# aclike/dynamic_multiview_3d

Hardware: AMD Instinct MI355X
Metric: train images/sec, appearance-flow encoder-decoder 128x128x3 (fwd+bwd+Adam) (higher is better)
Workload: dtype bf16x3; 1 GPU; appflow_offset: AppearanceFlowModel 128x128x3, batch 64 per GPU, Adam lr 1e-4, random-init weights (reference initialisers); global_batch=64, parallelism=dp1

## Files before the change

### dynamic_multiview_3d_amd/_lib.py

```python
import ctypes as C
import os

HERE = os.path.dirname(os.path.abspath(__file__))
LIB_PATH = os.environ.get("MV3D_LIB") or os.path.join(HERE, "libmv3d_hip.so")

ACT_NONE, ACT_LRELU, ACT_RELU, ACT_TANH = 0, 1, 2, 3
ACT_BY_NAME = {None: ACT_NONE, 'none': ACT_NONE, 'lrelu': ACT_LRELU, 'relu': ACT_RELU, 'tanh': ACT_TANH}
F32 = 0


class ConvGeom(C.Structure):
    _fields_ = [(n, C.c_int32) for n in
                ("N", "H", "W", "C", "Ho", "Wo", "K", "kh", "kw", "sh", "sw", "img_ld", "feat_ld", "dtype")]


class Epilogue(C.Structure):
    _fields_ = [("bias", C.c_void_p), ("act", C.c_int32), ("leak", C.c_float), ("gmask_act", C.c_int32),
                ("gmask_leak", C.c_float), ("gmask_ref", C.c_void_p), ("gmask_ld", C.c_int32)]


class FcChainLayer(C.Structure):
    _fields_ = [("M", C.c_void_p), ("bias", C.c_void_p), ("y", C.c_void_p), ("y_ld", C.c_int32), ("out", C.c_int32),
                ("act", C.c_int32), ("leak", C.c_float)]


class FcChain(C.Structure):
    _fields_ = [("B", C.c_int32), ("nlayers", C.c_int32), ("in_", C.c_int32), ("x_ld", C.c_int32), ("x", C.c_void_p),
                ("l", FcChainLayer * 4)]


class Mv3dError(RuntimeError):
    pass


_vp, _i, _i64, _f, _sz = C.c_void_p, C.c_int, C.c_int64, C.c_float, C.c_size_t
_G, _E = C.POINTER(ConvGeom), C.POINTER(Epilogue)

STATUS_FUNCS = {
    "mv3d_conv2d_fwd": [_G, _vp, _vp, _vp, _E, _vp, _sz, _vp],
    "mv3d_conv2d_dgrad": [_G, _vp, _vp, _vp, _E, _vp, _sz, _vp],
    "mv3d_conv2d_wgrad": [_G, _vp, _vp, _vp, _vp, _vp, _sz, _vp],
    "mv3d_deconv2d_fwd": [_G, _vp, _vp, _vp, _E, _vp, _sz, _vp],
    "mv3d_deconv2d_dgrad": [_G, _vp, _vp, _vp, _E, _vp, _sz, _vp],
    "mv3d_deconv2d_wgrad": [_G, _vp, _vp, _vp, _vp, _sz, _vp],
    "mv3d_fc_fwd": [_i, _i, _i, _vp, _i, _vp, _vp, _i, _E, _vp, _sz, _vp],
    "mv3d_fc_dgrad": [_i, _i, _i, _vp, _i, _vp, _vp, _i, _E, _vp, _sz, _vp],
    "mv3d_fc_wgrad": [_i, _i, _i, _vp, _i, _vp, _i, _vp, _vp, _vp, _sz, _vp],
    "mv3d_fc_wgrad_dgrad": [_i, _i, _i, _vp, _i, _vp, _i, _vp, _vp, _vp, _vp, _i, _E, _vp, _sz, _vp],
    "mv3d_fc_chain_fwd": [C.POINTER(FcChain), _vp],
    "mv3d_act_fwd": [_i64, _i, _vp, _i, _vp, _i, _i, _f, _vp],
    "mv3d_act_bwd": [_i64, _i, _vp, _i, _vp, _i, _vp, _i, _i, _f, _vp],
    "mv3d_copy2d": [_i64, _i, _vp, _i64, _i64, _vp, _i64, _i, _vp],
    "mv3d_group_sum": [_i64, _i, _i, _vp, _i64, _vp, _i64, _vp],
    "mv3d_warp_resample_fwd": [_i, _i, _i, _i, _i, _i, _vp, _vp, _i, _vp, _vp, _vp],
    "mv3d_warp_resample_bwd": [_i, _i, _i, _i, _i, _i, _vp, _vp, _i, _vp, _vp, _i, _vp],
    "mv3d_warp_resample_loss": [_i, _i, _i, _i, _i, _i, _vp, _vp, _i, _vp, _i, _i, _f, _vp, _vp, _vp, _i, _vp, _vp],
    "mv3d_resampler_fwd": [_i, _i, _i, _i, _i, _vp, _i, _vp, _i, _vp, _i, _vp],
    "mv3d_resampler_bwd": [_i, _i, _i, _i, _i, _vp, _i, _vp, _i, _vp, _i, _vp, _i, _vp, _i, _vp, _sz, _vp],
    "mv3d_image_metrics": [_i, _i, _i, _i, _vp, _i, _vp, _i, _f, _vp, _vp, _sz, _vp],
    "mv3d_ssim_loss": [_i, _i, _i, _i, _vp, _i, _vp, _i, _f, _f, _vp, _vp, _i, _i, _vp, _sz, _vp],
    "mv3d_flow_smoothness": [_i, _i, _i, _vp, _i, _vp, _i, _i, _f, _f, _f, _vp, _vp, _i, _i, _vp, _sz, _vp],
    "mv3d_pixel_loss": [_i64, _i, _vp, _vp, _vp, _i, _f, _vp, _vp, _vp],
    "mv3d_loss_overwrite_next": [],
    "mv3d_pixel_loss_strided": [_i64, _i, _vp, _i, _vp, _i, _f, _vp, _i, _i, _f, _vp, _vp, _i, _vp],
    "mv3d_tfrecord_open": [C.c_char_p, _i, C.POINTER(_vp)],
    "mv3d_tfrecord_read": [_vp, _i, _i, _i, C.POINTER(C.c_char_p), C.POINTER(C.c_int), C.POINTER(C.c_size_t), C.POINTER(_vp), C.POINTER(C.c_int)],
    "mv3d_u8_to_unit_f32": [_i64, _vp, _vp, _vp],
    "mv3d_u8_process_image": [_vp, _i, _i, _i, _i, _vp, _i, _i, _vp],
    "mv3d_fill": [_vp, _i64, _f, _vp],
    "mv3d_adam_step": [_i64, _vp, _vp, _vp, _vp, _f, _f, _f, _f, _f, _f, _f, _vp],
    "mv3d_adam_step_dev": [_i64, _vp, _vp, _vp, _vp, _vp, _i, C.POINTER(_i64), C.POINTER(_i64), _vp],
    "mv3d_adam_advance": [_vp, _vp],
    "mv3d_fc_wgrad_adam": [_i, _i, _i, _vp, _i, _vp, _i, _vp, _vp, _vp, _vp, _vp, _vp],
    "mv3d_sgd_step": [_i64, _vp, _vp, _vp, _f, _f, _i, _f, _vp],
    "mv3d_sgd_step_dev": [_i64, _vp, _vp, _vp, _vp, _i, C.POINTER(_i64), C.POINTER(_i64), _vp],
    "mv3d_fc_wgrad_sgd": [_i, _i, _i, _vp, _i, _vp, _i, _vp, _vp, _vp, _vp, _vp],
    "mv3d_grad_finalize_begin": [],
    "mv3d_grad_finalize_add": [_vp, _i64],
    "mv3d_grad_finalize_commit": [_vp, _sz, _vp, _vp, _vp, _vp, _vp, _vp],
    "mv3d_grad_finalize_commit_sgd": [_vp, _sz, _vp, _vp, _vp, _vp, _vp],
    "mv3d_grad_finalize_abort": [],
    "mv3d_comm_unique_id": [_vp],
    "mv3d_comm_init": [C.POINTER(_vp), _i, _i, _vp],
    "mv3d_comm_destroy": [_vp],
    "mv3d_comm_allreduce_sum": [_vp, _vp, _i64, _vp],
    "mv3d_comm_reduce_scatter_sum": [_vp, _vp, _vp, _i64, _vp],
    "mv3d_comm_allgather": [_vp, _vp, _vp, _i64, _vp],
    "mv3d_ipc_export": [_vp, _vp, C.POINTER(_i64)],
    "mv3d_ipc_open": [_vp, C.POINTER(_vp)],
    "mv3d_ipc_close": [_vp],
    "mv3d_mesh_reduce_sum": [C.POINTER(_vp), _i, _vp, _i64, _vp],
    "mv3d_mesh_copy": [_vp, _vp, _i64, _vp],
    "mv3d_filter_cache_bind": [_G, _i, _vp, _vp, _sz],
    "mv3d_filter_cache_commit": [_vp, _sz, _vp],
    "mv3d_filter_cache_refresh": [_vp],
    "mv3d_filter_cache_clear": [],
    "mv3d_plan_begin": [_vp],
    "mv3d_plan_end": [],
    "mv3d_plan_run": [_vp, _vp],
    "mv3d_plan_run_range": [_vp, _i, _i, _vp],
    "mv3d_plan_run_range_multi": [_vp, _i, _i, _vp, C.POINTER(_vp), _i, _i],
    "mv3d_plan_side": [_i],
    "mv3d_plan_profile": [_vp, _i],
    "mv3d_plan_profile_collect": [_vp],
    "mv3d_plan_profile_select": [_vp, C.c_char_p],
    "mv3d_plan_profile_reset": [_vp],
    "mv3d_plan_op_info": [_vp, _i, C.POINTER(C.c_char_p), C.POINTER(C.c_double), C.POINTER(C.c_double),
                          C.POINTER(C.c_double), C.POINTER(C.c_int)],
}
OTHER_FUNCS = {
    "mv3d_version": (C.c_char_p, []),
    "mv3d_last_error": (C.c_char_p, []),
    "mv3d_conv_workspace_bytes": (_sz, [_G]),
    "mv3d_conv_wgrad_workspace_bytes": (_sz, [_G]),
    "mv3d_fc_workspace_bytes": (_sz, [_i, _i, _i]),
    "mv3d_resampler_bwd_workspace_bytes": (_sz, [_i, _i, _i, _i, _i]),
    "mv3d_image_metrics_workspace_bytes": (_sz, [_i, _i, _i, _i]),
    "mv3d_ssim_loss_workspace_bytes": (_sz, [_i, _i, _i, _i]),
    "mv3d_flow_smoothness_workspace_bytes": (_sz, [_i, _i, _i]),
    "mv3d_crc32c": (C.c_uint32, [_vp, _sz]),
    "mv3d_set_diagnostics": (C.c_int, [_i]),
    "mv3d_set_wgrad_cus": (C.c_int, [_i]),
    "mv3d_tfrecord_close": (None, [_vp]),
    "mv3d_filter_prepared_bytes": (_sz, [_G, _i]),
    "mv3d_filter_cache_table_bytes": (_sz, []),
    "mv3d_grad_finalize_table_bytes": (_sz, []),
    "mv3d_plan_create": (_vp, []),
    "mv3d_plan_destroy": (None, [_vp]),
    "mv3d_plan_size": (_i, [_vp]),
    "mv3d_comm_available": (_i, []),
    "mv3d_fc_wgrad_adam_supported": (_i, [_i, _i, _i, _i, _i]),
    "mv3d_debug_cconv_stamps": (_i, [_vp, _sz]),
    "mv3d_debug_cwgrad_stamps": (_i, [_vp, _sz]),
    "mv3d_debug_band_stamps": (_i, [_vp, _sz]),
}
EXPORTS = sorted(list(STATUS_FUNCS) + list(OTHER_FUNCS))

_lib = None


class _Checked:

    def __init__(self, name, fn, dll):
        self.name, self.fn, self.dll = name, fn, dll

    def __call__(self, *args):
        rc = self.fn(*args)
        if rc != 0:
            raise Mv3dError("%s failed (%d): %s" % (self.name, rc, self.dll.mv3d_last_error().decode()))
        return rc


class _Lib:
    def __init__(self, path):
        if not os.path.exists(path):
            raise Mv3dError("%s not found: build it with `python -m dynamic_multiview_3d_amd.build` "
                            "(hipcc --offload-arch=gfx950); there is no fallback path" % path)
        import torch
        self.dll = C.CDLL(path)
        for name, (res, args) in OTHER_FUNCS.items():
            fn = getattr(self.dll, name)
            fn.restype, fn.argtypes = res, args
            if name[5:] != 'last_error':
                setattr(self, name[5:], fn)
        for name, args in STATUS_FUNCS.items():
            fn = getattr(self.dll, name)
            fn.restype, fn.argtypes = C.c_int, args
            setattr(self, name[5:], _Checked(name, fn, self.dll))
            setattr(self, "raw_" + name[5:], fn)

    def last_error(self):
        return self.dll.mv3d_last_error().decode()


def lib():
    global _lib
    if _lib is None:
        _lib = _Lib(LIB_PATH)
    return _lib


def plan_ops(plan):
    l = lib()
    out = []
    for i in range(l.plan_size(plan)):
        name, fl, by, ms, runs = C.c_char_p(), C.c_double(), C.c_double(), C.c_double(), C.c_int()
        l.plan_op_info(plan, i, C.byref(name), C.byref(fl), C.byref(by), C.byref(ms), C.byref(runs))
        out.append((name.value.decode(), fl.value, by.value, ms.value, runs.value))
    return out


def epilogue(bias=None, act=ACT_NONE, leak=0.2, gmask_act=ACT_NONE, gmask_leak=0.2, gmask_ref=None, gmask_ld=0):
    return Epilogue(bias, act, leak, gmask_act, gmask_leak, gmask_ref, gmask_ld)


def conv_geom(N, H, W, Cc, K, kh, kw, sh, sw, img_ld=None, feat_ld=None):
    Ho, Wo = -(-H // sh), -(-W // sw)
    return ConvGeom(N, H, W, Cc, Ho, Wo, K, kh, kw, sh, sw, Cc if img_ld is None else img_ld,
                    K if feat_ld is None else feat_ld, F32)
```

### dynamic_multiview_3d_amd/build.py

```python
import os
import shutil
import subprocess
import sys

HERE = os.path.dirname(os.path.abspath(__file__))
CSRC = os.path.join(HERE, "csrc")
LIB = os.path.join(HERE, "libmv3d_hip.so")

UNITS = {
    "core.hip": [],
    "conv.hip": [],
    "hconv.hip": [],
    "bconv.hip": [],
    "cconv.hip": (["-DCC_TAP_STAMPS"] if os.environ.get("MV3D_CC_TAP_STAMPS") else []),
    "sconv.hip": [],
    "thin.hip": [],
    "wgrad_tile.hip": [],
    "fc.hip": [],
    "elem.hip": ["-ffp-contract=off"],
    "resampler.hip": ["-ffp-contract=off"],
    "process_image.hip": ["-ffp-contract=off"],
    "metrics.hip": ["-ffp-contract=off"],
    "ssim_loss.hip": ["-ffp-contract=off"],
    "flow_smooth.hip": ["-ffp-contract=off"],
    "comm.hip": [],
    "tfrecord.hip": ["-msse4.2"],
}
COMMON = ["-O3", "-std=c++17", "--offload-arch=gfx950", "-fPIC", "-Wall", "-Wno-unused-function"]


def _hipcc():
    exe = shutil.which("hipcc") or "/opt/rocm/bin/hipcc"
    if not os.path.exists(exe):
        raise RuntimeError("hipcc not found: libmv3d_hip.so cannot be built")
    return exe


def _stale(target, deps):
    if not os.path.exists(target):
        return True
    t = os.path.getmtime(target)
    return any(os.path.getmtime(d) > t for d in deps)


def build(force=False, verbose=False):
    hipcc = _hipcc()
    objdir = os.path.join(HERE, "build")
    os.makedirs(objdir, exist_ok=True)
    headers = [os.path.join(CSRC, "common.h"), os.path.join(CSRC, "conv_common.h"), os.path.join(HERE, "..", "include", "mv3d_hip.h")]
    objs = []
    for src, extra in UNITS.items():
        s = os.path.join(CSRC, src)
        o = os.path.join(objdir, src.replace(".hip", ".o"))
        objs.append(o)
        if force or _stale(o, [s] + headers):
            cmd = [hipcc] + COMMON + extra + ["-c", s, "-o", o]
            if verbose:
                print(" ".join(cmd), flush=True)
            subprocess.run(cmd, check=True)
    if force or _stale(LIB, objs):
        cmd = [hipcc, "-shared", "-fPIC", "--offload-arch=gfx950", "-o", LIB] + objs + ["-ldl"]
        if verbose:
            print(" ".join(cmd), flush=True)
        subprocess.run(cmd, check=True)
    return LIB


if __name__ == "__main__":
    print(build(force="--force" in sys.argv, verbose=True))
```

### dynamic_multiview_3d_amd/csrc/bconv.hip

```cpp
#include "conv_common.h"
#include <algorithm>
#include <mutex>
#include <string.h>
#include <vector>

namespace mv3d {

typedef __bf16 bf16x8 __attribute__((ext_vector_type(8)));
typedef __bf16 bf16x4 __attribute__((ext_vector_type(4)));

constexpr int BC_PIXB = 144;

__device__ __forceinline__ void split4(const float4& v, uint2& hi, uint2& lo) {
    bf16x4 h, l;
    h[0] = (__bf16)v.x; h[1] = (__bf16)v.y; h[2] = (__bf16)v.z; h[3] = (__bf16)v.w;
    l[0] = (__bf16)(v.x - (float)h[0]); l[1] = (__bf16)(v.y - (float)h[1]);
    l[2] = (__bf16)(v.z - (float)h[2]); l[3] = (__bf16)(v.w - (float)h[3]);
    hi = __builtin_bit_cast(uint2, h);
    lo = __builtin_bit_cast(uint2, l);
}


template <int NTHR>
__device__ __forceinline__ void bconv_stage_halo(const IgemmParams& p, const HconvExtra& x, unsigned char* halo, int cc, int n,
                                                 int ih0, int iw0, int tid) {
    constexpr int PS = NTHR / 8;
    const int c4 = tid & 7;
    const int halo_pix = x.HR * x.HC;
    const int ch = cc * 32 + c4 * 4;
    const bool ch_ok = ch < p.Ka && !(x.dbg & 1);
    const int dq = PS / x.HC, dr = PS - dq * x.HC;
    int pix = tid >> 3;
    int hrv = (int)(((unsigned)pix * (unsigned)x.inv_hc) >> 20), hc = pix - hrv * x.HC;
    for (; pix < halo_pix;) {
        float4 v[8];
        int lofs[8];
#pragma unroll
        for (int u = 0; u < 8; ++u) {
            const int g = x.G > 1 ? (int)(((unsigned)hrv * (unsigned)x.inv_hri) >> 20) : 0;
            const int hr = hrv - g * x.HRi;
            const int ih = ih0 + hr, iw = iw0 + hc;
            const bool ok = ch_ok && pix < halo_pix && n + g < p.N && (unsigned)ih < (unsigned)p.Ha && (unsigned)iw < (unsigned)p.Wa;
            const float* src = ok ? p.A + (int64_t)(((n + g) * p.Ha + ih) * p.Wa + iw) * p.a_ld + ch : p.A;
            const float4 t4 = *reinterpret_cast<const float4*>(src);
            v[u] = ok ? t4 : make_float4(0.f, 0.f, 0.f, 0.f);
            lofs[u] = pix < halo_pix ? hrv * x.row_bytes + hc * BC_PIXB + c4 * 8 : -1;
            pix += PS; hc += dr; hrv += dq;
            if (hc >= x.HC) { hc -= x.HC; ++hrv; }
        }
#pragma unroll
        for (int u = 0; u < 8; ++u) {
            if (lofs[u] >= 0) {
                uint2 hi, lo;
                split4(v[u], hi, lo);
                *reinterpret_cast<uint2*>(halo + lofs[u]) = hi;
                *reinterpret_cast<uint2*>(halo + lofs[u] + 64) = lo;
            }
        }
    }
}

template <int MT, int NT>
__device__ __forceinline__ void bconv_store_tile(const IgemmParams& p, const HconvExtra& x, const f32x16 (&acc)[MT][NT], int wave, int lane,
                                                 int n, int oh0, int ow0, int n0, int phh, int phw, int zks) {
    const int li = lane & 31, lh = lane >> 5;
    const int Hp = p.Hp[0], Wp = p.Wp[0];
    const int64_t npix_total = (int64_t)p.N * p.Hc * p.Wc;
    const bool interior = n + x.G <= p.N && oh0 + x.TH <= Hp && ow0 + x.TW <= Wp && n0 + 32 * NT <= p.Cc && !(x.dbg & 16);
#pragma unroll
    for (int m = 0; m < MT; ++m)
#pragma unroll
        for (int y = 0; y < NT; ++y) {
            const int col = n0 + y * 32 + li;
            const float bias = (p.bias && col < p.Cc) ? p.bias[col] : 0.f;
#pragma unroll
            for (int grp = 0; grp < 4; ++grp) {
                const int q = (wave * MT + m) * 32 + 8 * grp + 4 * lh;
                const int g = q >> x.img_shift, qr = q & ((1 << x.img_shift) - 1);
                const int ohp = oh0 + (qr >> x.tw_shift), owp = ow0 + (qr & (x.TW - 1));
                const int64_t pix0 = (int64_t)((n + g) * p.Hc + ohp * p.so_h + phh) * p.Wc + owp * p.so_w + phw;
#pragma unroll
                for (int j = 0; j < 4; ++j) {
                    const float a = acc[m][y][4 * grp + j];
                    const int64_t pix = pix0 + j * p.so_w;
                    if (interior || (n + g < p.N && ohp < Hp && owp + j < Wp && col < p.Cc && !(x.dbg & 16))) {
                        if (x.ksplit > 1) p.Part[((int64_t)zks * npix_total + pix) * p.Cc + col] = a;
                        else {
                            float v = act_apply(a + bias, p.act, p.leak);
                            if (p.gact != MV3D_ACT_NONE) v *= act_grad_from_out(p.gref[pix * p.g_ld + col], p.gact, p.gleak);
                            p.Out[pix * p.c_ld + col] = v;
                        }
                    }
                }
            }
        }
}

__global__ __launch_bounds__(256) void bconv_split_filter_kernel(const IgemmParams p, uint4* __restrict__ Wf, int ntaps, int chunks, int ntiles) {
    const int64_t gid = (int64_t)blockIdx.x * 256 + threadIdx.x;
    const int lane = (int)(gid & 63);
    int64_t r = gid >> 6;
    const int s = (int)(r & 1); r >>= 1;
    const int nt = (int)(r % ntiles); r /= ntiles;
    const int cc = (int)(r % chunks); r /= chunks;
    const int t = (int)r;
    if (t >= ntaps) return;
    const int li = lane & 31, lh = lane >> 5;
    const int col = nt * 32 + li;
    const int ch0 = cc * 32 + s * 16 + lh * 8;
    const float* wt = p.Wt + (int64_t)p.taps[t].widx * p.w_tap_stride;
    float v[8];
#pragma unroll
    for (int j = 0; j < 8; ++j) {
        const int ch = ch0 + j;
        v[j] = (col < p.Cc && ch < p.Ka) ? wt[(int64_t)ch * p.w_ks + (int64_t)col * p.w_ns] : 0.f;
    }
    uint2 h0, l0, h1, l1;
    split4(make_float4(v[0], v[1], v[2], v[3]), h0, l0);
    split4(make_float4(v[4], v[5], v[6], v[7]), h1, l1);
    uint4* dst = Wf + ((((int64_t)t * chunks + cc) * ntiles + nt) * 4 + s * 2) * 64 + lane;
    dst[0] = make_uint4(h0.x, h0.y, h1.x, h1.y);
    dst[64] = make_uint4(l0.x, l0.y, l1.x, l1.y);
}

template <int MT, int NT>
struct BFrags {
    uint4 a[MT][2][2];
    uint4 b[NT][2][2];
};

template <int NPH, int MT, int NT, int WAVES>
__global__ __launch_bounds__(WAVES * 64) void bconv_kernel(const IgemmParams p, const HconvExtra x, const uint4* __restrict__ Wf, int ntiles) {
    extern __shared__ __attribute__((aligned(16))) unsigned char halo[];
    constexpr int NTHR = WAVES * 64;
    const int tid = threadIdx.x;
    const int lane = tid & 63, wave = tid >> 6;
    const int li = lane & 31, lh = lane >> 5;

    int b = blockIdx.x;
    const int tw_i = b % x.tiles_w; b /= x.tiles_w;
    const int th_i = b % x.tiles_h;
    const int n = (b / x.tiles_h) * x.G;
    const int oh0 = th_i * x.TH, ow0 = tw_i * x.TW;
    const int n0 = blockIdx.y * 32 * NT;
    const int zks = (int)blockIdx.z % x.ksplit;

    int lane_base[MT];
#pragma unroll
    for (int m = 0; m < MT; ++m) {
        const int pidx = (wave * MT + m) * 32 + li;
        const int g = pidx >> x.img_shift, pr = pidx & ((1 << x.img_shift) - 1);
        const int tr = pr >> x.tw_shift, tc = pr & (x.TW - 1);
        lane_base[m] = (g * x.HRi + tr * p.sa_h) * x.row_bytes + tc * p.sa_w * BC_PIXB + lh * 16;
    }

    f32x16 acc[NPH][MT][NT];
#pragma unroll
    for (int a = 0; a < NPH; ++a)
#pragma unroll
        for (int m = 0; m < MT; ++m)
#pragma unroll
            for (int y = 0; y < NT; ++y)
#pragma unroll
                for (int r = 0; r < 16; ++r) acc[a][m][y][r] = 0.f;

    const int ph_z = x.phase_split ? (int)blockIdx.z / x.ksplit : 0;
    const int tap_lo = x.phase_split ? p.tap_begin[ph_z] : 0;
    const int ntaps_here = x.phase_split ? p.tap_begin[ph_z + 1] - tap_lo : x.ntaps_total;
    const int tap_hi = tap_lo + ntaps_here;
    const int cc_begin = (x.chunks * zks) / x.ksplit, cc_end = (x.chunks * (zks + 1)) / x.ksplit;
    const int total_seq = (cc_end - cc_begin) * ntaps_here;

    const uint4* wf_lane = Wf + (int64_t)(blockIdx.y * NT) * 256 + lane;
// ... 296 lines not shown
        pg.x = std::min<int>((int)grid.x, cap);
    }
    return dispatch(stream, OpInfo{name, flops, bytes}, [=](hipStream_t s) {
        bconvu_kernel<NTAPS, U, MT, NT, WAVES><<<pg, WAVES * 64, lds, s>>>(p, xp, wf, ntiles);
        return launched(who);
    });
}

static int launch_bconv_cfg(const IgemmParams& p, const HconvExtra& x, int nph_fused, int MT, int NT, int WAVES, dim3 grid, size_t lds,
                            const uint4* wf, int ntiles, void* stream, const char* name, const char* who, double flops, double bytes) {
#define MV3D_BC(NPH_, MT_, NT_, W_) launch_bconv_t<NPH_, MT_, NT_, W_>(p, x, grid, lds, wf, ntiles, stream, name, who, flops, bytes)
    const int ntaps_all = p.tap_begin[p.so_h * p.so_w];
    if (WAVES == 8) return launch_cconv(p, x, wf, ntiles, stream, who, flops, bytes);
    if (nph_fused == 1 && !x.phase_split && p.so_h == 1 && p.so_w == 1 && (ntaps_all == 25 || ntaps_all == 9) && !(disabled_paths() & 8192)) {
#define MV3D_BCU(MT_, NT_, W_) (ntaps_all == 25 ? launch_bconvu_t<25, 5, MT_, NT_, W_>(p, x, grid, lds, wf, ntiles, stream, name, who, flops, bytes) \
                                                : launch_bconvu_t<9, 3, MT_, NT_, W_>(p, x, grid, lds, wf, ntiles, stream, name, who, flops, bytes))
        if (MT == 2 && NT == 1 && WAVES == 4) return MV3D_BCU(2, 1, 4);
        if (MT == 2 && NT == 2 && WAVES == 4) return MV3D_BCU(2, 2, 4);
        if (MT == 1 && NT == 2 && WAVES == 4) return MV3D_BCU(1, 2, 4);
        if (MT == 1 && NT == 1 && WAVES == 4) return MV3D_BCU(1, 1, 4);
        if (MT == 1 && NT == 1 && WAVES == 2) return MV3D_BCU(1, 1, 2);
        if (MT == 1 && NT == 2 && WAVES == 2) return MV3D_BCU(1, 2, 2);
#undef MV3D_BCU
    }
    if (nph_fused == 4) {
        if (MT == 1 && NT == 1 && WAVES == 4) return MV3D_BC(4, 1, 1, 4);
        if (MT == 1 && NT == 1 && WAVES == 2) return MV3D_BC(4, 1, 1, 2);
    } else {
        if (MT == 2 && NT == 1 && WAVES == 4) return MV3D_BC(1, 2, 1, 4);
        if (MT == 2 && NT == 2 && WAVES == 4) return MV3D_BC(1, 2, 2, 4);
        if (MT == 1 && NT == 2 && WAVES == 4) return MV3D_BC(1, 1, 2, 4);
        if (MT == 1 && NT == 1 && WAVES == 4) return MV3D_BC(1, 1, 1, 4);
        if (MT == 1 && NT == 1 && WAVES == 2) return MV3D_BC(1, 1, 1, 2);
        if (MT == 1 && NT == 2 && WAVES == 2) return MV3D_BC(1, 1, 2, 2);
    }
#undef MV3D_BC
    return fail(MV3D_E_UNSUPPORTED, "%s: no split-bf16 kernel for nph=%d MT=%d NT=%d waves=%d", who, nph_fused, MT, NT, WAVES);
}

const void* bconv_cache_lookup(const IgemmParams& p, int* ntiles_out);

int launch_bconv(const IgemmParams& p, const HconvExtra& x, int nph_fused, int MT, int NT, int WAVES, dim3 grid,
                 void* wfrag, void* stream, const char* name, const char* who, double flops, double bytes) {
    const int nph = p.so_h * p.so_w;
    const int ntaps = p.tap_begin[nph];
    const int chunks = x.chunks, ntiles = cdiv(p.Cc, 32 * NT) * NT;
    uint4* wf = reinterpret_cast<uint4*>(wfrag);
    int cached_tiles = 0;
    const void* cached = bconv_cache_lookup(p, &cached_tiles);
    if (cached && cached_tiles >= ntiles) {
        wf = reinterpret_cast<uint4*>(const_cast<void*>(cached));
        const size_t lds0 = (size_t)bconv_lds_bytes(x);
        return launch_bconv_cfg(p, x, nph_fused, MT, NT, WAVES, grid, lds0, wf, cached_tiles, stream, name, who, flops, bytes);
    }
    {
        const int64_t threads = (int64_t)ntaps * chunks * ntiles * 2 * 64;
        const int blocks = (int)cdiv64(threads, 256);
        const IgemmParams pc = p;
        int rc = dispatch(stream, OpInfo{"bconv_split_filter", 0.0, 2.0 * (double)ntaps * p.Ka * p.Cc * 4.0}, [=](hipStream_t s) {
            bconv_split_filter_kernel<<<blocks, 256, 0, s>>>(pc, wf, ntaps, chunks, ntiles);
            return launched("bconv_split_filter_kernel");
        });
        if (rc != MV3D_OK) return rc;
    }
    return launch_bconv_cfg(p, x, nph_fused, MT, NT, WAVES, grid, (size_t)bconv_lds_bytes(x), wf, ntiles, stream, name, who, flops, bytes);
}


const uint4* bconv_get_filter(const IgemmParams& p, void* ws, size_t ws_bytes, void* stream, int* ntiles_out, int* rc) {
    const int nph = p.so_h * p.so_w;
    const int ntaps = p.tap_begin[nph];
    const int chunks = cdiv(p.Ka, 32), ntiles = cdiv(p.Cc, 32);
    int cached_tiles = 0;
    const void* cached = bconv_cache_lookup(p, &cached_tiles);
    if (cached && cached_tiles >= ntiles) { *ntiles_out = cached_tiles; *rc = MV3D_OK; return reinterpret_cast<const uint4*>(cached); }
    const size_t need = bconv_filter_bytes(p, 1);
    if (!ws || ws_bytes < need || (reinterpret_cast<uintptr_t>(ws) & 15)) { *rc = 1; return nullptr; }
    uint4* wf = reinterpret_cast<uint4*>(ws);
    const int64_t threads = (int64_t)ntaps * chunks * ntiles * 2 * 64;
    const int blocks = (int)cdiv64(threads, 256);
    const IgemmParams pc = p;
    *rc = dispatch(stream, OpInfo{"bconv_split_filter", 0.0, 2.0 * (double)ntaps * p.Ka * p.Cc * 4.0}, [=](hipStream_t s) {
        bconv_split_filter_kernel<<<blocks, 256, 0, s>>>(pc, wf, ntaps, chunks, ntiles);
        return launched("bconv_split_filter_kernel");
    });
    if (*rc != MV3D_OK) return nullptr;
    *ntiles_out = ntiles;
    return wf;
}

struct SplitJob {
    const float* Wt; uint4* Wf;
    int ntaps, chunks, ntiles, Ka, Cc, w_tap_stride, w_ks, w_ns;
    int first_block, nblocks;
    int16_t widx[36];
};

static std::mutex g_cache_mu;
static std::vector<SplitJob> g_jobs;
static const SplitJob* g_table_dev = nullptr;
static int g_table_jobs = 0, g_total_blocks = 0;

__global__ __launch_bounds__(256) void bconv_split_all_kernel(const SplitJob* __restrict__ jobs, int njobs) {
    const int* block_job = reinterpret_cast<const int*>(jobs + njobs);
    const SplitJob& jb = jobs[block_job[blockIdx.x]];
    const int64_t gid = (int64_t)(blockIdx.x - jb.first_block) * 256 + threadIdx.x;
    const int lane = (int)(gid & 63);
    int64_t r = gid >> 6;
    const int s = (int)(r & 1); r >>= 1;
    const int nt = (int)(r % jb.ntiles); r /= jb.ntiles;
    const int cc = (int)(r % jb.chunks); r /= jb.chunks;
    const int t = (int)r;
    if (t >= jb.ntaps) return;
    const int li = lane & 31, lh = lane >> 5;
    const int col = nt * 32 + li;
    const int ch0 = cc * 32 + s * 16 + lh * 8;
    const float* wt = jb.Wt + (int64_t)jb.widx[t] * jb.w_tap_stride;
    float v[8];
    if (jb.w_ks == 1 && (jb.w_ns & 3) == 0 && ch0 + 8 <= jb.Ka && col < jb.Cc && ((reinterpret_cast<uintptr_t>(wt) & 15) == 0)) {
        const float4* src = reinterpret_cast<const float4*>(wt + (int64_t)col * jb.w_ns + ch0);
        const float4 u0 = src[0], u1 = src[1];
        v[0] = u0.x; v[1] = u0.y; v[2] = u0.z; v[3] = u0.w; v[4] = u1.x; v[5] = u1.y; v[6] = u1.z; v[7] = u1.w;
    } else {
#pragma unroll
        for (int e = 0; e < 8; ++e) {
            const int ch = ch0 + e;
            v[e] = (col < jb.Cc && ch < jb.Ka) ? wt[(int64_t)ch * jb.w_ks + (int64_t)col * jb.w_ns] : 0.f;
        }
    }
    uint2 h0, l0, h1, l1;
    split4(make_float4(v[0], v[1], v[2], v[3]), h0, l0);
    split4(make_float4(v[4], v[5], v[6], v[7]), h1, l1);
    uint4* dst = jb.Wf + ((((int64_t)t * jb.chunks + cc) * jb.ntiles + nt) * 4 + s * 2) * 64 + lane;
    dst[0] = make_uint4(h0.x, h0.y, h1.x, h1.y);
    dst[64] = make_uint4(l0.x, l0.y, l1.x, l1.y);
}

static bool job_matches(const SplitJob& j, const IgemmParams& p, int ntaps) {
    if (j.Wt != p.Wt || j.ntaps != ntaps || j.Ka != p.Ka || j.Cc != p.Cc || j.w_ks != p.w_ks || j.w_ns != p.w_ns ||
        j.w_tap_stride != p.w_tap_stride) return false;
    for (int t = 0; t < ntaps; ++t) if (j.widx[t] != p.taps[t].widx) return false;
    return true;
}

const void* bconv_cache_lookup(const IgemmParams& p, int* ntiles_out) {
    const int ntaps = p.tap_begin[p.so_h * p.so_w];
    std::lock_guard<std::mutex> lk(g_cache_mu);
    if (!g_table_dev) return nullptr;
    for (int i = 0; i < g_table_jobs && i < (int)g_jobs.size(); ++i)
        if (job_matches(g_jobs[i], p, ntaps)) { *ntiles_out = g_jobs[i].ntiles; return g_jobs[i].Wf; }
    return nullptr;
}

size_t bconv_prepared_bytes(const IgemmParams& p) {
    if (p.fold || p.Ka % 16 != 0 || p.Cc < 16) return 0;
    const int ntaps = p.tap_begin[p.so_h * p.so_w];
    if (ntaps < 2 || ntaps > 36) return 0;
    return bconv_filter_bytes(p, 2);
}

int bconv_cache_bind(const IgemmParams& p, void* prepared, size_t bytes) {
    const size_t need = bconv_prepared_bytes(p);
    if (need == 0) return 1;
    if (!prepared || bytes < need || (reinterpret_cast<uintptr_t>(prepared) & 15))
        return fail(MV3D_E_INVAL, "mv3d_filter_cache_bind: prepared buffer null, misaligned or %zu < %zu bytes", bytes, need);
    const int ntaps = p.tap_begin[p.so_h * p.so_w];
    SplitJob j = {};
    j.Wt = p.Wt; j.Wf = reinterpret_cast<uint4*>(prepared);
    j.ntaps = ntaps; j.chunks = cdiv(p.Ka, 32); j.ntiles = cdiv(p.Cc, 64) * 2; j.Ka = p.Ka; j.Cc = p.Cc;
    j.w_tap_stride = p.w_tap_stride; j.w_ks = p.w_ks; j.w_ns = p.w_ns;
    for (int t = 0; t < ntaps; ++t) j.widx[t] = p.taps[t].widx;
    j.nblocks = (int)cdiv64((int64_t)ntaps * j.chunks * j.ntiles * 2 * 64, 256);
    std::lock_guard<std::mutex> lk(g_cache_mu);
    for (auto& e : g_jobs)
        if (job_matches(e, p, ntaps)) { e.Wf = j.Wf; g_table_dev = nullptr; return MV3D_OK; }
    g_jobs.push_back(j);
    g_table_dev = nullptr;
    return MV3D_OK;
}

}

using namespace mv3d;

extern "C" {

static size_t cache_table_bytes_locked() {
    size_t blocks = 0;
    for (const auto& j : g_jobs) blocks += (size_t)j.nblocks;
    return g_jobs.size() * sizeof(SplitJob) + blocks * sizeof(int);
}

size_t mv3d_filter_cache_table_bytes(void) {
    std::lock_guard<std::mutex> lk(g_cache_mu);
    return cache_table_bytes_locked();
}

int mv3d_filter_cache_commit(void* table_dev, size_t table_bytes, void* stream) {
    std::lock_guard<std::mutex> lk(g_cache_mu);
    const size_t need = cache_table_bytes_locked();
    if (g_jobs.empty()) { g_table_dev = nullptr; g_table_jobs = 0; g_total_blocks = 0; return MV3D_OK; }
    if (!table_dev || table_bytes < need) return fail(MV3D_E_INVAL, "mv3d_filter_cache_commit: table %zu < %zu bytes", table_bytes, need);
    int first = 0;
    for (auto& j : g_jobs) { j.first_block = first; first += j.nblocks; }
    std::vector<unsigned char> host(need);
    memcpy(host.data(), g_jobs.data(), g_jobs.size() * sizeof(SplitJob));
    int* bj = reinterpret_cast<int*>(host.data() + g_jobs.size() * sizeof(SplitJob));
    for (size_t i = 0; i < g_jobs.size(); ++i)
        for (int b = 0; b < g_jobs[i].nblocks; ++b) bj[g_jobs[i].first_block + b] = (int)i;
    hipError_t e = hipMemcpyAsync(table_dev, host.data(), need, hipMemcpyHostToDevice, reinterpret_cast<hipStream_t>(stream));
    if (e == hipSuccess) e = hipStreamSynchronize(reinterpret_cast<hipStream_t>(stream));
    if (e != hipSuccess) return fail(MV3D_E_HIP, "mv3d_filter_cache_commit: %s", hipGetErrorString(e));
    g_table_dev = reinterpret_cast<const SplitJob*>(table_dev);
    g_table_jobs = (int)g_jobs.size();
    g_total_blocks = first;
    return MV3D_OK;
}

int mv3d_filter_cache_refresh(void* stream) {
    const SplitJob* table; int njobs, blocks; double bytes = 0.0;
    {
        std::lock_guard<std::mutex> lk(g_cache_mu);
        table = g_table_dev; njobs = g_table_jobs; blocks = g_total_blocks;
        for (int i = 0; i < njobs; ++i) bytes += 8.0 * g_jobs[i].ntaps * (double)g_jobs[i].Ka * g_jobs[i].Cc;
    }
    if (!table || njobs == 0) return MV3D_OK;
    return dispatch(stream, OpInfo{"bconv_split_all", 0.0, bytes}, [=](hipStream_t s) {
        bconv_split_all_kernel<<<blocks, 256, 0, s>>>(table, njobs);
        return launched("bconv_split_all_kernel");
    });
}

int mv3d_filter_cache_clear(void) {
    std::lock_guard<std::mutex> lk(g_cache_mu);
    g_jobs.clear(); g_table_dev = nullptr; g_table_jobs = 0; g_total_blocks = 0;
    return MV3D_OK;
}

}
```

### dynamic_multiview_3d_amd/csrc/common.h

```cpp
#pragma once
#include <hip/hip_runtime.h>
#include <stdint.h>
#include <stdlib.h>
#include <functional>
#include "../../include/mv3d_hip.h"

namespace mv3d {

int fail(int code, const char* fmt, ...) __attribute__((format(printf, 2, 3)));
struct OpInfo {
    const char* name;
    double flops;
    double bytes;
};

const char* intern_label(const char* fmt, ...) __attribute__((format(printf, 1, 2)));

bool recording();
bool take_loss_overwrite();
void record(std::function<int(hipStream_t)> fn, const OpInfo& info);

enum OptKind { OPT_NONE = 0, OPT_ADAM = 1, OPT_MOMENTUM = 2, OPT_GD = 3 };

__device__ __forceinline__ void momentum_elem(float g, float& p, float& a, float lr, float mu, bool nesterov) {
#pragma clang fp contract(off)
    a = a * mu + g;
    if (nesterov) p = p - (g * lr + (a * mu) * lr);
    else p = p - a * lr;
}
__device__ __forceinline__ void gd_elem(float g, float& p, float lr) {
#pragma clang fp contract(off)
    p = p - g * lr;
}

template <class F>
inline int dispatch(void* stream, const OpInfo& info, F fn) {
    if (recording()) { record(std::function<int(hipStream_t)>(fn), info); return MV3D_OK; }
    return fn(reinterpret_cast<hipStream_t>(stream));
}

inline int launched(const char* what) {
    hipError_t e = hipGetLastError();
    if (e != hipSuccess) return fail(MV3D_E_HIP, "%s: %s", what, hipGetErrorString(e));
    return MV3D_OK;
}

struct FinSegHost { const float* part; int nslab; int64_t count; float* out; };
bool finalize_collecting();
void finalize_push(const float* part, int nslab, int64_t count, float* out);
void finalize_open();
}
#include <vector>
namespace mv3d {
const std::vector<FinSegHost>* finalize_peek();
void finalize_take(std::vector<FinSegHost>* out);

int disabled_paths();

static inline int cdiv(int a, int b) { return (a + b - 1) / b; }
static inline int64_t cdiv64(int64_t a, int64_t b) { return (a + b - 1) / b; }

static inline void same_pad(int size, int k, int s, int* out, int* before) {
    int o = (size + s - 1) / s;
    int total = (o - 1) * s + k - size;
    if (total < 0) total = 0;
    *out = o;
    *before = total / 2;
}

__device__ __forceinline__ float act_apply(float x, int act, float leak) {
    if (act == MV3D_ACT_LRELU) {
        float f1 = 0.5f * (1.0f + leak), f2 = 0.5f * (1.0f - leak);
        return __fadd_rn(__fmul_rn(f1, x), __fmul_rn(f2, fabsf(x)));
    }
    if (act == MV3D_ACT_RELU) {
        float y = __fadd_rn(__fmul_rn(0.5f, x), __fmul_rn(0.5f, fabsf(x)));
        return x < 0.0f ? -0.0f : y;
    }
    if (act == MV3D_ACT_TANH) return tanhf(x);
    return x;
}

__device__ __forceinline__ float act_grad_from_out(float y, int act, float leak) {
    if (act == MV3D_ACT_LRELU) {
        float f1 = 0.5f * (1.0f + leak), f2 = 0.5f * (1.0f - leak);
        float s = (y > 0.0f) ? 1.0f : ((y < 0.0f) ? -1.0f : 0.0f);
        return f1 + f2 * s;
    }
    if (act == MV3D_ACT_RELU) {
        if (y > 0.0f) return 1.0f;
        return (__float_as_uint(y) >> 31) ? 0.0f : 0.5f;
    }
    if (act == MV3D_ACT_TANH) return 1.0f - y * y;
    return 1.0f;
}

typedef float f32x16 __attribute__((ext_vector_type(16)));
typedef float f32x4 __attribute__((ext_vector_type(4)));

}
```

### dynamic_multiview_3d_amd/csrc/core.hip

```cpp
#include "common.h"
#include <atomic>
#include <cstdlib>
#include <stdarg.h>
#include <stdio.h>
#include <string.h>
#include <vector>
#include <mutex>
#include <set>
#include <string>

struct PlanOp {
    std::function<int(hipStream_t)> fn;
    mv3d::OpInfo info;
    double total_ms;
    int runs;
    bool selected = true;
    int side = 0;
};

struct mv3d_plan {
    std::vector<PlanOp> ops;
    bool profile = false;
    std::vector<hipEvent_t> pool;
    size_t used = 0;
    hipEvent_t fork[MV3D_MAX_SIDE] = {}, join[MV3D_MAX_SIDE] = {};
    bool pass_open = false;
};

namespace mv3d {

static std::atomic<int> g_disabled{-1};
int disabled_paths() {
    int v = g_disabled.load(std::memory_order_relaxed);
    if (v < 0) {
        const char* e = getenv("MV3D_DISABLE");
        v = e ? atoi(e) : 0;
        g_disabled.store(v, std::memory_order_relaxed);
    }
    return v;
}

static thread_local char g_err[512] = "";
static thread_local mv3d_plan* g_rec = nullptr;
static thread_local int g_side = 0;

int fail(int code, const char* fmt, ...) {
    va_list ap;
    va_start(ap, fmt);
    vsnprintf(g_err, sizeof(g_err), fmt, ap);
    va_end(ap);
    return code;
}
const char* intern_label(const char* fmt, ...) {
    char buf[128];
    va_list ap;
    va_start(ap, fmt);
    vsnprintf(buf, sizeof(buf), fmt, ap);
    va_end(ap);
    static std::mutex mu;
    static std::set<std::string>* labels = new std::set<std::string>();
    std::lock_guard<std::mutex> lk(mu);
    return labels->insert(buf).first->c_str();
}
static thread_local std::vector<FinSegHost>* g_fin = nullptr;
bool finalize_collecting() { return g_fin != nullptr; }
void finalize_open() { if (!g_fin) g_fin = new std::vector<FinSegHost>(); }
void finalize_push(const float* part, int nslab, int64_t count, float* out) { if (g_fin) g_fin->push_back(FinSegHost{part, nslab, count, out}); }
const std::vector<FinSegHost>* finalize_peek() { return g_fin; }
void finalize_take(std::vector<FinSegHost>* out) {
    if (!g_fin) return;
    if (out) out->swap(*g_fin);
    delete g_fin;
    g_fin = nullptr;
}
bool recording() { return g_rec != nullptr; }
void record(std::function<int(hipStream_t)> fn, const OpInfo& info) { g_rec->ops.push_back(PlanOp{std::move(fn), info, 0.0, 0, true, g_side}); }
}

extern "C" {

const char* mv3d_version(void) { return "mv3d_hip 0.3 (gfx950, split-bf16 / fp32 MFMA)"; }
const char* mv3d_last_error(void) { return mv3d::g_err; }

mv3d_plan* mv3d_plan_create(void) { return new mv3d_plan(); }
void mv3d_plan_destroy(mv3d_plan* p) {
    if (!p) return;
    if (mv3d::g_rec == p) mv3d::g_rec = nullptr;
    for (hipEvent_t e : p->pool) (void)hipEventDestroy(e);
    for (int k = 0; k < MV3D_MAX_SIDE; ++k) {
        if (p->fork[k]) (void)hipEventDestroy(p->fork[k]);
        if (p->join[k]) (void)hipEventDestroy(p->join[k]);
    }
    delete p;
}
int mv3d_plan_begin(mv3d_plan* p) {
    if (!p) return mv3d::fail(MV3D_E_INVAL, "mv3d_plan_begin: null plan");
    if (mv3d::g_rec) return mv3d::fail(MV3D_E_INVAL, "mv3d_plan_begin: a plan is already recording on this thread");
    p->ops.clear();
    p->used = 0;
    mv3d::g_rec = p;
    mv3d::g_side = 0;
    return MV3D_OK;
}
int mv3d_plan_side(int side) {
    if (side < 0 || side > MV3D_MAX_SIDE) return mv3d::fail(MV3D_E_INVAL, "mv3d_plan_side: side %d not in [0, %d]", side, MV3D_MAX_SIDE);
    mv3d::g_side = side;
    return MV3D_OK;
}
int mv3d_plan_end(void) {
    if (!mv3d::g_rec) return mv3d::fail(MV3D_E_INVAL, "mv3d_plan_end: nothing is recording");
    mv3d::g_rec = nullptr;
    return MV3D_OK;
}
int mv3d_plan_size(const mv3d_plan* p) { return p ? (int)p->ops.size() : 0; }

int mv3d_plan_run_range(mv3d_plan* p, int begin, int end, void* stream) {
    return mv3d_plan_run_range_multi(p, begin, end, stream, nullptr, 0, 0);
}

int mv3d_plan_run_range_multi(mv3d_plan* p, int begin, int end, void* stream, void* const* side_streams, int nside, int flags) {
    if (!p) return mv3d::fail(MV3D_E_INVAL, "mv3d_plan_run_range: null plan");
    if (mv3d::g_rec) return mv3d::fail(MV3D_E_INVAL, "mv3d_plan_run_range: cannot run while recording");
    const int n = (int)p->ops.size();
    if (begin < 0 || end > n || begin > end) return mv3d::fail(MV3D_E_INVAL, "mv3d_plan_run_range: bad range [%d, %d) of %d", begin, end, n);
    if (nside < 0 || nside > MV3D_MAX_SIDE || (nside > 0 && !side_streams)) return mv3d::fail(MV3D_E_INVAL, "mv3d_plan_run_range_multi: bad side stream list");
    hipStream_t s = reinterpret_cast<hipStream_t>(stream);
    for (int k = 0; k < nside; ++k)
        if (!p->fork[k]) {
            if (hipEventCreateWithFlags(&p->fork[k], hipEventDisableTiming) != hipSuccess ||
                hipEventCreateWithFlags(&p->join[k], hipEventDisableTiming) != hipSuccess)
                return mv3d::fail(MV3D_E_HIP, "mv3d_plan_run_range_multi: hipEventCreate failed");
        }
    int prev_side = 0;
    bool used[MV3D_MAX_SIDE] = {};
    auto stream_of = [&](int i) -> hipStream_t {
        const int tag = p->ops[i].side;
        const int sd = (nside > 0 && tag > 0) ? 1 + (tag - 1) % nside : 0;
        hipStream_t so = sd ? reinterpret_cast<hipStream_t>(side_streams[sd - 1]) : s;
        if (sd && so == s) { prev_side = 0; return s; }
        if (sd && sd != prev_side) {
            (void)hipEventRecord(p->fork[sd - 1], s);
            (void)hipStreamWaitEvent(so, p->fork[sd - 1], 0);
            used[sd - 1] = true;
        }
        prev_side = sd;
        return so;
    };
    auto join = [&]() {
        if (flags & MV3D_RUN_NO_JOIN) return;
        for (int k = 0; k < nside; ++k)
            if (used[k]) {
                (void)hipEventRecord(p->join[k], reinterpret_cast<hipStream_t>(side_streams[k]));
                (void)hipStreamWaitEvent(s, p->join[k], 0);
            }
    };
    if (!p->profile) {
        for (int i = begin; i < end; ++i) {
            int rc = p->ops[i].fn(stream_of(i));
            if (rc != MV3D_OK) return rc;
        }
        join();
        return MV3D_OK;
    }
    const size_t need = p->used + 2 * (size_t)n;
    while (p->pool.size() < need) {
        hipEvent_t e;
        if (hipEventCreate(&e) != hipSuccess) return mv3d::fail(MV3D_E_HIP, "mv3d_plan_run: hipEventCreate failed");
        p->pool.push_back(e);
    }
    if (!p->pass_open) {
        for (int i = 0; i < begin; ++i)
            if (p->ops[i].selected) { (void)hipEventRecord(p->pool[p->used + 2 * i], s); (void)hipEventRecord(p->pool[p->used + 2 * i + 1], s); }
        p->pass_open = true;
    }
    for (int i = begin; i < end; ++i) {
        const bool sel = p->ops[i].selected;
        hipStream_t so = stream_of(i);
        if (sel) (void)hipEventRecord(p->pool[p->used + 2 * i], so);
        int rc = p->ops[i].fn(so);
        if (sel) (void)hipEventRecord(p->pool[p->used + 2 * i + 1], so);
        if (rc != MV3D_OK) return rc;
    }
    join();
    if (end == n) { p->used = need; p->pass_open = false; }
    return MV3D_OK;
}

int mv3d_plan_run(mv3d_plan* p, void* stream) {
    if (!p) return mv3d::fail(MV3D_E_INVAL, "mv3d_plan_run: null plan");
    return mv3d_plan_run_range(p, 0, (int)p->ops.size(), stream);
}

int mv3d_plan_profile(mv3d_plan* p, int enable) {
    if (!p) return mv3d::fail(MV3D_E_INVAL, "mv3d_plan_profile: null plan");
    p->profile = enable != 0;
    return MV3D_OK;
}

int mv3d_plan_profile_collect(mv3d_plan* p) {
    if (!p) return mv3d::fail(MV3D_E_INVAL, "mv3d_plan_profile_collect: null plan");
    const size_t n = p->ops.size();
    if (n == 0 || p->used == 0) return MV3D_OK;
    size_t last = n;
    for (size_t i = 0; i < n; ++i) if (p->ops[i].selected) last = i;
    if (last == n) { p->used = 0; return MV3D_OK; }
    if (hipEventSynchronize(p->pool[p->used - 2 * n + 2 * last + 1]) != hipSuccess)
        return mv3d::fail(MV3D_E_HIP, "mv3d_plan_profile_collect: hipEventSynchronize failed");
    for (size_t base = 0; base + 2 * n <= p->used; base += 2 * n)
        for (size_t i = 0; i < n; ++i) {
            if (!p->ops[i].selected) continue;
            float ms = 0.f;
            if (hipEventElapsedTime(&ms, p->pool[base + 2 * i], p->pool[base + 2 * i + 1]) == hipSuccess) {
                p->ops[i].total_ms += ms;
                p->ops[i].runs += 1;
            }
        }
    p->used = 0;
    (void)hipGetLastError();
    return MV3D_OK;
}

static bool label_matches(const char* label, const char* pats) {
    const size_t ll = strlen(label);
    for (const char* p = pats; *p;) {
        const char* e = strchr(p, '|');
        size_t n = e ? (size_t)(e - p) : strlen(p);
// ... 67 lines not shown
```

### dynamic_multiview_3d_amd/csrc/elem.hip

```cpp
#include "common.h"
#include "reduce_common.h"
#include <vector>
#include <algorithm>
#include <cstdlib>
#include <atomic>

namespace mv3d {

constexpr int LOSS_ROWS = 32, LOSS_MAXB = 1024;
__device__ unsigned g_loss_part[LOSS_ROWS][LOSS_MAXB];
__device__ unsigned g_loss_ticket[LOSS_ROWS];

static thread_local bool g_loss_overwrite = false;
bool take_loss_overwrite() {
    const bool v = g_loss_overwrite;
    g_loss_overwrite = false;
    return v;
}
static int next_loss_row() {
    static std::atomic<unsigned> n{0};
    const int flag = take_loss_overwrite() ? 256 : 0;
    return (int)(n.fetch_add(1) % LOSS_ROWS) | flag;
}

__device__ __forceinline__ void loss_combine(float term, float* loss, int row_flag) {
    const int row = row_flag & 255;
    __shared__ unsigned s_last;
    __shared__ float s_w[4];
    if (threadIdx.x == 0) {
        (void)__hip_atomic_exchange(&g_loss_part[row][blockIdx.x], __float_as_uint(term), __ATOMIC_RELAXED, __HIP_MEMORY_SCOPE_AGENT);
        asm volatile("s_waitcnt vmcnt(0)" ::: "memory");
        const unsigned t = __hip_atomic_fetch_add(&g_loss_ticket[row], 1u, __ATOMIC_RELAXED, __HIP_MEMORY_SCOPE_AGENT);
        s_last = t == gridDim.x - 1;
    }
    __syncthreads();
    if (!s_last) return;
    float sum = 0.f;
    for (unsigned i = threadIdx.x; i < gridDim.x; i += 256)
        sum += __uint_as_float(__hip_atomic_fetch_or(&g_loss_part[row][i], 0u, __ATOMIC_RELAXED, __HIP_MEMORY_SCOPE_AGENT));
    for (int off = 32; off > 0; off >>= 1) sum += __shfl_down(sum, off);
    if ((threadIdx.x & 63) == 0) s_w[threadIdx.x >> 6] = sum;
    __syncthreads();
    if (threadIdx.x == 0) {
        const float total = (s_w[0] + s_w[1]) + (s_w[2] + s_w[3]);
        if (row_flag & 256) *loss = total; else atomicAdd(loss, total);
        __hip_atomic_store(&g_loss_ticket[row], 0u, __ATOMIC_RELAXED, __HIP_MEMORY_SCOPE_AGENT);
    }
}

struct ResampleParams {
    const float* src; const float* flow; const float* dgen;
    float* warp; float* gen; float* dflow;
    int N, H, W, Hs, Ws, C, flow_ld, dflow_ld;
};

__device__ __forceinline__ float tap(const float* img, int Ws, int Hs, int C, int y, int x, int c) {
    const bool ok = (unsigned)x < (unsigned)Ws && (unsigned)y < (unsigned)Hs;
    const int xc = min(max(x, 0), Ws - 1), yc = min(max(y, 0), Hs - 1);
    const float v = img[((int64_t)yc * Ws + xc) * C + c];
    return ok ? v : 0.f;
}

template <bool BWD>
__global__ __launch_bounds__(256) void resample_kernel(const ResampleParams p) {
    const int tj = threadIdx.x & 31, ti = threadIdx.x >> 5;
    const int j = blockIdx.x * 32 + tj, i = blockIdx.y * 8 + ti, n = blockIdx.z;
    if (i >= p.H || j >= p.W) return;
    const int64_t pix = ((int64_t)n * p.H + i) * p.W + j;
    const float* fl = p.flow + pix * p.flow_ld;
    const float x = fl[0] + (float)i;
    const float y = fl[1] + (float)j;
    if (!BWD && p.warp) { p.warp[pix * 2] = x; p.warp[pix * 2 + 1] = y; }
    const bool valid = x > -1.0f && y > -1.0f && x < (float)p.Ws && y < (float)p.Hs;
    const float fxf = floorf(x), fyf = floorf(y);
    const int fx = (int)fxf, fy = (int)fyf, cx = fx + 1, cy = fy + 1;
    const float dx = (fxf + 1.0f) - x, dy = (fyf + 1.0f) - y;
    const float* img = p.src + (int64_t)n * p.Hs * p.Ws * p.C;
    if (!BWD) {
        float* out = p.gen + pix * p.C;
        for (int c = 0; c < p.C; ++c) {
            float v = 0.f;
            if (valid) {
                const float iff = tap(img, p.Ws, p.Hs, p.C, fy, fx, c), icc = tap(img, p.Ws, p.Hs, p.C, cy, cx, c);
                const float ifc = tap(img, p.Ws, p.Hs, p.C, cy, fx, c), icf = tap(img, p.Ws, p.Hs, p.C, fy, cx, c);
                v = ((dx * dy * iff + (1.0f - dx) * (1.0f - dy) * icc) + dx * (1.0f - dy) * ifc) + (1.0f - dx) * dy * icf;
            }
            out[c] = v;
        }
    } else {
        float gx = 0.f, gy = 0.f;
        if (valid) {
            const float* g = p.dgen + pix * p.C;
            for (int c = 0; c < p.C; ++c) {
                const float iff = tap(img, p.Ws, p.Hs, p.C, fy, fx, c), icc = tap(img, p.Ws, p.Hs, p.C, cy, cx, c);
                const float ifc = tap(img, p.Ws, p.Hs, p.C, cy, fx, c), icf = tap(img, p.Ws, p.Hs, p.C, fy, cx, c);
                gx += g[c] * (dy * (icf - iff) + (1.0f - dy) * (icc - ifc));
                gy += g[c] * (dx * (ifc - iff) + (1.0f - dx) * (icc - icf));
            }
        }
        float* d = p.dflow + pix * p.dflow_ld;
        d[0] = gx; d[1] = gy;
    }
}

struct ResampleTileParams {
    const float* src; const float* flow; const float* aux;
    float* warp; float* gen; float* dflow; float* loss; int loss_row;
    int N, H, W, Hs, Ws, flow_ld, aux_ld, dflow_ld, kind;
    float weight;
    int tiles_i, tiles_j, n_tiles;
};

template <int MODE, int C>
__global__ __launch_bounds__(256) void resample_tile_kernel(const ResampleTileParams p) {
    constexpr int P = 33;
    __shared__ float s_xy[2][32 * P];
    __shared__ float s_c[C][32 * P];
    const int lo = threadIdx.x & 31, hi = threadIdx.x >> 5;
    const float inv_pix = 1.0f / (float)((int64_t)p.N * p.H * p.W);
    const float gscale = (p.kind == 2 ? 2.0f : 1.0f) * p.weight / (float)((int64_t)p.N * p.H * p.W);
    float sum = 0.f;
    for (int tile = blockIdx.x; tile < p.n_tiles; tile += gridDim.x) {
        int b = tile;
        const int tj = b % p.tiles_j; b /= p.tiles_j;
        const int ti = b % p.tiles_i;
        const int n = b / p.tiles_i;
        const int i0 = ti * 32, j0 = tj * 32;
        const float* img = p.src + (int64_t)n * p.Hs * p.Ws * C;
        {
            float fx_[4], fy_[4], av[4][C];
#pragma unroll
            for (int k = 0; k < 4; ++k) {
                const int i = min(i0 + hi + 8 * k, p.H - 1), j = min(j0 + lo, p.W - 1);
                const int64_t pix = ((int64_t)n * p.H + i) * p.W + j;
                const float* fl = p.flow + pix * p.flow_ld;
                fx_[k] = fl[0]; fy_[k] = fl[1];
                if (MODE != 0) {
#pragma unroll
                    for (int c = 0; c < C; ++c) av[k][c] = p.aux[pix * p.aux_ld + c];
                }
            }
#pragma unroll
            for (int k = 0; k < 4; ++k) {
                const int r = hi + 8 * k, i = i0 + r, j = j0 + lo;
                const float x = fx_[k] + (float)min(i, p.H - 1), y = fy_[k] + (float)min(j, p.W - 1);
                s_xy[0][r * P + lo] = x; s_xy[1][r * P + lo] = y;
                if (MODE != 0) {
#pragma unroll
                    for (int c = 0; c < C; ++c) s_c[c][r * P + lo] = av[k][c];
                }
                if (MODE != 1 && p.warp && i < p.H && j < p.W) {
                    const int64_t pix = ((int64_t)n * p.H + i) * p.W + j;
                    p.warp[pix * 2] = x; p.warp[pix * 2 + 1] = y;
                }
// ... 115 lines not shown
        else { sum += fabsf(d); g = ((d > 0.f) ? 1.f : ((d < 0.f) ? -1.f : 0.f)) * m * gscale; }
        if (p.grad) p.grad[pix * p.grad_ld + c] = g;
    }
    for (int off = 32; off > 0; off >>= 1) sum += __shfl_down(sum, off);
    __shared__ float s_part[4];
    if ((threadIdx.x & 63) == 0) s_part[threadIdx.x >> 6] = sum;
    __syncthreads();
    loss_combine((s_part[0] + s_part[1] + s_part[2] + s_part[3]) * (p.weight / (float)p.pixels), p.loss, p.loss_row);
}

__global__ __launch_bounds__(256) void pixel_loss_dense_kernel(int64_t total4, int64_t pixels, const float4* __restrict__ a,
                                                              const float4* __restrict__ b, int kind, float weight, float* loss,
                                                              float4* __restrict__ grad, int loss_row) {
    const float gscale = (kind == 2 ? 2.0f : 1.0f) * weight / (float)pixels;
    float sum = 0.f;
    for (int64_t i = (int64_t)blockIdx.x * 256 + threadIdx.x; i < total4; i += (int64_t)gridDim.x * 256) {
        const float4 x = a[i], y = b[i];
        const float d[4] = {x.x - y.x, x.y - y.y, x.z - y.z, x.w - y.w};
        float g[4];
#pragma unroll
        for (int e = 0; e < 4; ++e) {
            if (kind == 2) { sum += d[e] * d[e]; g[e] = d[e] * gscale; }
            else { sum += fabsf(d[e]); g[e] = ((d[e] > 0.f) ? 1.f : ((d[e] < 0.f) ? -1.f : 0.f)) * gscale; }
        }
        if (grad) grad[i] = make_float4(g[0], g[1], g[2], g[3]);
    }
    for (int off = 32; off > 0; off >>= 1) sum += __shfl_down(sum, off);
    __shared__ float s_part[4];
    if ((threadIdx.x & 63) == 0) s_part[threadIdx.x >> 6] = sum;
    __syncthreads();
    loss_combine((s_part[0] + s_part[1] + s_part[2] + s_part[3]) * (weight / (float)pixels), loss, loss_row);
}

__global__ __launch_bounds__(256) void u8_to_unit_f32_kernel(int64_t count, const unsigned char* __restrict__ src, float* __restrict__ dst) {
    const int64_t nvec = count >> 2;
    for (int64_t i = (int64_t)blockIdx.x * 256 + threadIdx.x; i < nvec; i += (int64_t)gridDim.x * 256) {
        const uchar4 b = reinterpret_cast<const uchar4*>(src)[i];
        reinterpret_cast<float4*>(dst)[i] = make_float4((float)b.x / 255.0f, (float)b.y / 255.0f, (float)b.z / 255.0f, (float)b.w / 255.0f);
    }
    if (blockIdx.x == 0 && threadIdx.x < (count & 3)) { const int64_t i = (nvec << 2) + threadIdx.x; dst[i] = (float)src[i] / 255.0f; }
}

__global__ __launch_bounds__(256) void fill_kernel(float* dst, int64_t count, float v) {
    for (int64_t i = (int64_t)blockIdx.x * 256 + threadIdx.x; i < count; i += (int64_t)gridDim.x * 256) dst[i] = v;
}

__global__ __launch_bounds__(256) void adam_kernel(int64_t count, float* __restrict__ p, const float* __restrict__ g,
                                                  float* __restrict__ m, float* __restrict__ v, float alpha,
                                                  float omb1, float omb2, float eps, float gscale) {
    const int64_t nvec = count >> 2;
    for (int64_t i = (int64_t)blockIdx.x * 256 + threadIdx.x; i < nvec; i += (int64_t)gridDim.x * 256) {
        float4 pp = reinterpret_cast<float4*>(p)[i], gg = reinterpret_cast<const float4*>(g)[i];
        float4 mm = reinterpret_cast<float4*>(m)[i], vv = reinterpret_cast<float4*>(v)[i];
        float* pe = &pp.x; float* ge = &gg.x; float* me = &mm.x; float* ve = &vv.x;
#pragma unroll
        for (int k = 0; k < 4; ++k) {
            const float gk = ge[k] * gscale;
            me[k] += (gk - me[k]) * omb1;
            ve[k] += (gk * gk - ve[k]) * omb2;
            pe[k] -= (me[k] * alpha) / (sqrtf(ve[k]) + eps);
        }
        reinterpret_cast<float4*>(p)[i] = pp;
        reinterpret_cast<float4*>(m)[i] = mm;
        reinterpret_cast<float4*>(v)[i] = vv;
    }
    if (blockIdx.x == 0 && threadIdx.x < (count & 3)) {
        const int64_t i = (nvec << 2) + threadIdx.x;
        const float gk = g[i] * gscale;
        m[i] += (gk - m[i]) * omb1;
        v[i] += (gk * gk - v[i]) * omb2;
        p[i] -= (m[i] * alpha) / (sqrtf(v[i]) + eps);
    }
}

struct AdamSkips { int n; int64_t lo[8], hi[8]; };
__global__ __launch_bounds__(256) void adam_dev_kernel(int64_t count, float* __restrict__ p, const float* __restrict__ g,
                                                      float* __restrict__ m, float* __restrict__ v, const float* __restrict__ st, const AdamSkips sk) {
    const float lr = st[0], b1 = st[1], b2 = st[2], eps = st[3], b1p = st[4], b2p = st[5], gscale = st[6];
    const float alpha = lr * sqrtf(1.0f - b2p) / (1.0f - b1p);
    const float omb1 = 1.0f - b1, omb2 = 1.0f - b2;
    int64_t kept = count >> 2;
    for (int r = 0; r < sk.n; ++r) kept -= (sk.hi[r] - sk.lo[r]) >> 2;
    for (int64_t j = (int64_t)blockIdx.x * 256 + threadIdx.x; j < kept; j += (int64_t)gridDim.x * 256) {
        int64_t i = j;
        for (int r = 0; r < sk.n; ++r)
            if (i >= (sk.lo[r] >> 2)) i += (sk.hi[r] - sk.lo[r]) >> 2;
        float4 pp = reinterpret_cast<float4*>(p)[i], gg = reinterpret_cast<const float4*>(g)[i];
        float4 mm = reinterpret_cast<float4*>(m)[i], vv = reinterpret_cast<float4*>(v)[i];
        float* pe = &pp.x; float* ge = &gg.x; float* me = &mm.x; float* ve = &vv.x;
#pragma unroll
        for (int k = 0; k < 4; ++k) {
            const float gk = ge[k] * gscale;
            me[k] += (gk - me[k]) * omb1;
            ve[k] += (gk * gk - ve[k]) * omb2;
            pe[k] -= (me[k] * alpha) / (sqrtf(ve[k]) + eps);
        }
        reinterpret_cast<float4*>(p)[i] = pp;
        reinterpret_cast<float4*>(m)[i] = mm;
        reinterpret_cast<float4*>(v)[i] = vv;
    }
}
__global__ void adam_advance_kernel(float* st) {
    if (threadIdx.x == 0 && blockIdx.x == 0) { st[4] = st[4] * st[1]; st[5] = st[5] * st[2]; }
}

template <bool MOM>
__device__ __forceinline__ void sgd4(float* p, const float* g, float* a, int64_t i, float lr, float mu, bool nesterov, float gscale) {
    float4 pp = reinterpret_cast<float4*>(p)[i], gg = reinterpret_cast<const float4*>(g)[i];
    float4 aa = MOM ? reinterpret_cast<float4*>(a)[i] : make_float4(0.f, 0.f, 0.f, 0.f);
    float* pe = &pp.x; float* ge = &gg.x; float* ae = &aa.x;
#pragma unroll
    for (int k = 0; k < 4; ++k) {
        const float gk = ge[k] * gscale;
        if (MOM) momentum_elem(gk, pe[k], ae[k], lr, mu, nesterov);
        else gd_elem(gk, pe[k], lr);
    }
    reinterpret_cast<float4*>(p)[i] = pp;
    if (MOM) reinterpret_cast<float4*>(a)[i] = aa;
}

template <bool MOM>
__global__ __launch_bounds__(256) void sgd_kernel(int64_t count, float* __restrict__ p, const float* __restrict__ g,
                                                 float* __restrict__ a, float lr, float mu, int nesterov, float gscale) {
    const int64_t nvec = count >> 2;
    for (int64_t i = (int64_t)blockIdx.x * 256 + threadIdx.x; i < nvec; i += (int64_t)gridDim.x * 256)
        sgd4<MOM>(p, g, a, i, lr, mu, nesterov != 0, gscale);
    if (blockIdx.x == 0 && threadIdx.x < (count & 3)) {
        const int64_t i = (nvec << 2) + threadIdx.x;
        const float gk = g[i] * gscale;
        if (MOM) { float pv = p[i], av = a[i]; momentum_elem(gk, pv, av, lr, mu, nesterov != 0); p[i] = pv; a[i] = av; }
        else { float pv = p[i]; gd_elem(gk, pv, lr); p[i] = pv; }
    }
}

template <bool MOM>
__global__ __launch_bounds__(256) void sgd_dev_kernel(int64_t count, float* __restrict__ p, const float* __restrict__ g,
                                                     float* __restrict__ a, const float* __restrict__ st, const AdamSkips sk) {
    const float lr = st[MV3D_SGD_LR], mu = st[MV3D_SGD_MOMENTUM], gscale = st[MV3D_SGD_GSCALE];
    const bool nesterov = st[MV3D_SGD_NESTEROV] != 0.f;
    int64_t kept = count >> 2;
    for (int r = 0; r < sk.n; ++r) kept -= (sk.hi[r] - sk.lo[r]) >> 2;
    for (int64_t j = (int64_t)blockIdx.x * 256 + threadIdx.x; j < kept; j += (int64_t)gridDim.x * 256) {
        int64_t i = j;
        for (int r = 0; r < sk.n; ++r)
            if (i >= (sk.lo[r] >> 2)) i += (sk.hi[r] - sk.lo[r]) >> 2;
        sgd4<MOM>(p, g, a, i, lr, mu, nesterov, gscale);
    }
}

struct FinSeg {
    const float* part; float* out;
    int64_t off;
    int64_t count;
    int nslab, vec, blk0, pad;
};

template <int OPT>
__global__ __launch_bounds__(256) void grad_finalize_kernel(const FinSeg* __restrict__ segs, const int* __restrict__ seg_of_blk,
                                                           const float* __restrict__ G, float* __restrict__ P, float* __restrict__ M,
                                                           float* __restrict__ V, const float* __restrict__ st) {
    constexpr bool ADAM = OPT == OPT_ADAM, SGD = OPT == OPT_MOMENTUM || OPT == OPT_GD;
    __shared__ float s_sum[4][16][17];
    const FinSeg sg = segs[seg_of_blk[blockIdx.x]];
    const int blk = (int)blockIdx.x - sg.blk0;
    float alpha = 0.f, omb1 = 0.f, omb2 = 0.f, eps = 0.f, gscale = 1.f;
    if (ADAM) {
        const float lr = st[0], b1 = st[1], b2 = st[2], b1p = st[4], b2p = st[5];
        eps = st[3]; gscale = st[6];
        alpha = lr * sqrtf(1.0f - b2p) / (1.0f - b1p);
        omb1 = 1.0f - b1; omb2 = 1.0f - b2;
    }
    float lr = 0.f, mu = 0.f;
    bool nesterov = false;
    if (SGD) {
        lr = st[MV3D_SGD_LR]; mu = st[MV3D_SGD_MOMENTUM]; nesterov = st[MV3D_SGD_NESTEROV] != 0.f; gscale = st[MV3D_SGD_GSCALE];
    }
    auto adam1 = [&](int64_t i, float g) {
        const float gk = g * gscale;
        float m = M[i], v = V[i], pp = P[i];
        m += (gk - m) * omb1;
        v += (gk * gk - v) * omb2;
        pp -= (m * alpha) / (sqrtf(v) + eps);
        P[i] = pp; M[i] = m; V[i] = v;
    };
    auto sgd1 = [&](int64_t i, float g) {
        const float gk = g * gscale;
        float pp = P[i];
        if (OPT == OPT_MOMENTUM) { float a = M[i]; momentum_elem(gk, pp, a, lr, mu, nesterov); M[i] = a; }
        else gd_elem(gk, pp, lr);
        P[i] = pp;
    };
    if (sg.nslab == 0) {
        if (!ADAM && !SGD) return;
        const int64_t i4 = (int64_t)blk * 256 + threadIdx.x;
        if (i4 * 4 >= sg.count) return;
        const int64_t i = (sg.off >> 2) + i4;
        if constexpr (SGD) {
            sgd4<OPT == OPT_MOMENTUM>(P, G, M, i, lr, mu, nesterov, gscale);
            return;
        }
        float4 pp = reinterpret_cast<float4*>(P)[i], gg = reinterpret_cast<const float4*>(G)[i];
        float4 mm = reinterpret_cast<float4*>(M)[i], vv = reinterpret_cast<float4*>(V)[i];
        float* pe = &pp.x; float* ge = &gg.x; float* me = &mm.x; float* ve = &vv.x;
#pragma unroll
        for (int k = 0; k < 4; ++k) {
            const float gk = ge[k] * gscale;
            me[k] += (gk - me[k]) * omb1;
            ve[k] += (gk * gk - ve[k]) * omb2;
            pe[k] -= (me[k] * alpha) / (sqrtf(ve[k]) + eps);
        }
        reinterpret_cast<float4*>(P)[i] = pp;
        reinterpret_cast<float4*>(M)[i] = mm;
        reinterpret_cast<float4*>(V)[i] = vv;
        return;
    }
    auto fin = [&](int64_t i, float t) {
        if (ADAM) adam1(sg.off + i, t);
        else if (SGD) sgd1(sg.off + i, t);
        else sg.out[i] = t;
    };
    if (sg.vec) reduce_slabs_body<4>(sg.part, sg.nslab, sg.count, blk, s_sum, fin);
    else reduce_slabs_body<1>(sg.part, sg.nslab, sg.count, blk, s_sum, fin);
}

__global__ __launch_bounds__(256) void act_fwd_kernel(int64_t rows, int ch, const float* x, int x_ld, float* y, int y_ld,
                                                     int act, float leak) {
    const int64_t total = rows * ch;
    for (int64_t i = (int64_t)blockIdx.x * 256 + threadIdx.x; i < total; i += (int64_t)gridDim.x * 256) {
        const int64_t r = i / ch; const int c = (int)(i - r * ch);
        y[r * y_ld + c] = act_apply(x[r * x_ld + c], act, leak);
    }
}
__global__ __launch_bounds__(256) void act_bwd_kernel(int64_t rows, int ch, const float* dy, int dy_ld, const float* ref,
                                                     int ref_ld, float* dx, int dx_ld, int act, float leak) {
    const int64_t total = rows * ch;
    for (int64_t i = (int64_t)blockIdx.x * 256 + threadIdx.x; i < total; i += (int64_t)gridDim.x * 256) {
        const int64_t r = i / ch; const int c = (int)(i - r * ch);
        dx[r * dx_ld + c] = dy[r * dy_ld + c] * act_grad_from_out(ref[r * ref_ld + c], act, leak);
    }
}
__global__ __launch_bounds__(256) void copy2d_kernel(int64_t rows, int ch, const float* src, int64_t src_ld, int64_t src_row_div,
                                                    float* dst, int64_t dst_ld, int accumulate) {
    const int64_t total = rows * ch;
    for (int64_t i = (int64_t)blockIdx.x * 256 + threadIdx.x; i < total; i += (int64_t)gridDim.x * 256) {
        const int64_t r = i / ch; const int c = (int)(i - r * ch);
        const float v = src[(r / src_row_div) * src_ld + c];
        float* d = dst + r * dst_ld + c;
        *d = accumulate ? (*d + v) : v;
    }
}
__global__ __launch_bounds__(256) void group_sum_kernel(int64_t groups, int group, int ch, const float* src, int64_t src_ld,
                                                       float* dst, int64_t dst_ld) {
    const int64_t total = groups * ch;
    for (int64_t i = (int64_t)blockIdx.x * 256 + threadIdx.x; i < total; i += (int64_t)gridDim.x * 256) {
        const int64_t gidx = i / ch; const int c = (int)(i - gidx * ch);
        float s = 0.f;
        for (int r = 0; r < group; ++r) s += src[(gidx * group + r) * src_ld + c];
        dst[gidx * dst_ld + c] = s;
    }
}

static inline int grid_for(int64_t total) { return (int)std::min<int64_t>(cdiv64(total, 256), 8192); }

}

using namespace mv3d;

extern "C" {

int mv3d_warp_resample_fwd(int N, int H, int W, int Hs, int Ws, int C, const void* src, const void* flow, int flow_ld,
                           void* warp_out, void* gen, void* stream) {
    if (N <= 0 || H <= 0 || W <= 0 || Hs <= 0 || Ws <= 0 || C <= 0 || flow_ld < 2) return fail(MV3D_E_INVAL, "mv3d_warp_resample_fwd: bad shape");
    if (!src || !flow || !gen) return fail(MV3D_E_INVAL, "mv3d_warp_resample_fwd: null pointer");
    if (N > 65535) return fail(MV3D_E_UNSUPPORTED, "mv3d_warp_resample_fwd: batch > 65535");
    if (C <= 4 && !(disabled_paths() & 65536)) {
        ResampleTileParams t = {};
        t.src = (const float*)src; t.flow = (const float*)flow; t.warp = (float*)warp_out; t.gen = (float*)gen;
        t.N = N; t.H = H; t.W = W; t.Hs = Hs; t.Ws = Ws; t.flow_ld = flow_ld;
        const int blocks = resample_tile_blocks(t);
        return dispatch(stream, OpInfo{"resample_fwd", 0.0, (double)N * H * W * (8.0 + 8.0 * C)}, [=](hipStream_t s) {
            launch_resample_tile<0>(t, C, blocks, s);
            return launched("resample_tile_kernel<fwd>");
        });
    }
    ResampleParams p = {(const float*)src, (const float*)flow, nullptr, (float*)warp_out, (float*)gen, nullptr, N, H, W, Hs, Ws, C, flow_ld, 0};
    dim3 grid(cdiv(W, 32), cdiv(H, 8), N);
    return dispatch(stream, OpInfo{"resample_fwd", 0.0, (double)N * H * W * (8.0 + 8.0 * C)}, [=](hipStream_t s) {
        resample_kernel<false><<<grid, 256, 0, s>>>(p);
        return launched("resample_kernel<fwd>");
    });
}

int mv3d_warp_resample_bwd(int N, int H, int W, int Hs, int Ws, int C, const void* src, const void* flow, int flow_ld,
                           const void* dgen, void* dflow, int dflow_ld, void* stream) {
    if (N <= 0 || H <= 0 || W <= 0 || Hs <= 0 || Ws <= 0 || C <= 0 || flow_ld < 2 || dflow_ld < 2) return fail(MV3D_E_INVAL, "mv3d_warp_resample_bwd: bad shape");
    if (!src || !flow || !dgen || !dflow) return fail(MV3D_E_INVAL, "mv3d_warp_resample_bwd: null pointer");
    if (N > 65535) return fail(MV3D_E_UNSUPPORTED, "mv3d_warp_resample_bwd: batch > 65535");
    if (C <= 4 && !(disabled_paths() & 65536)) {
        ResampleTileParams t = {};
        t.src = (const float*)src; t.flow = (const float*)flow; t.aux = (const float*)dgen; t.aux_ld = C; t.dflow = (float*)dflow;
        t.N = N; t.H = H; t.W = W; t.Hs = Hs; t.Ws = Ws; t.flow_ld = flow_ld; t.dflow_ld = dflow_ld;
        const int blocks = resample_tile_blocks(t);
        return dispatch(stream, OpInfo{"resample_bwd", 0.0, (double)N * H * W * (16.0 + 8.0 * C)}, [=](hipStream_t s) {
            launch_resample_tile<1>(t, C, blocks, s);
            return launched("resample_tile_kernel<bwd>");
        });
    }
    ResampleParams p = {(const float*)src, (const float*)flow, (const float*)dgen, nullptr, nullptr, (float*)dflow, N, H, W, Hs, Ws, C, flow_ld, dflow_ld};
    dim3 grid(cdiv(W, 32), cdiv(H, 8), N);
    return dispatch(stream, OpInfo{"resample_bwd", 0.0, (double)N * H * W * (16.0 + 8.0 * C)}, [=](hipStream_t s) {
        resample_kernel<true><<<grid, 256, 0, s>>>(p);
        return launched("resample_kernel<bwd>");
    });
}

int mv3d_warp_resample_loss(int N, int H, int W, int Hs, int Ws, int C, const void* src, const void* flow, int flow_ld,
                            const void* target, int target_ld, int kind, float weight, void* warp_out, void* gen,
                            void* dflow, int dflow_ld, void* loss_accum, void* stream) {
    if (N <= 0 || H <= 0 || W <= 0 || Hs <= 0 || Ws <= 0 || C <= 0 || flow_ld < 2 || target_ld < C || (dflow && dflow_ld < 2))
        return fail(MV3D_E_INVAL, "mv3d_warp_resample_loss: bad shape");
    if (kind != 1 && kind != 2) return fail(MV3D_E_INVAL, "mv3d_warp_resample_loss: kind must be 1 (l1) or 2 (euclidean)");
    if (!src || !flow || !target || !gen || !loss_accum) return fail(MV3D_E_INVAL, "mv3d_warp_resample_loss: null pointer");
    if (C > 4) return fail(MV3D_E_UNSUPPORTED, "mv3d_warp_resample_loss: more than 4 channels");
    ResampleTileParams t = {};
    t.src = (const float*)src; t.flow = (const float*)flow; t.aux = (const float*)target; t.aux_ld = target_ld;
    t.warp = (float*)warp_out; t.gen = (float*)gen; t.dflow = (float*)dflow; t.loss = (float*)loss_accum;
    t.N = N; t.H = H; t.W = W; t.Hs = Hs; t.Ws = Ws; t.flow_ld = flow_ld; t.dflow_ld = dflow_ld; t.kind = kind; t.weight = weight;
    t.loss_row = next_loss_row();
    static const int max_blocks = getenv("MV3D_RL_BLOCKS") ? atoi(getenv("MV3D_RL_BLOCKS")) : 512;
    const int blocks = std::min(resample_tile_blocks(t), max_blocks);
    return dispatch(stream, OpInfo{"resample_loss", 0.0, (double)N * H * W * (8.0 + 8.0 + 8.0 + 12.0 * C)}, [=](hipStream_t s) {
        launch_resample_tile<2>(t, C, blocks, s);
        return launched("resample_tile_kernel<fused>");
    });
}

int mv3d_pixel_loss_strided(int64_t pixels, int ch, const void* a, int a_ld, const void* b, int b_ld, float b_scale,
                            const void* mask, int mask_ld, int kind, float weight, void* loss_accum, void* grad, int grad_ld,
                            void* stream) {
    if (pixels <= 0 || ch <= 0 || (kind != 1 && kind != 2)) return fail(MV3D_E_INVAL, "mv3d_pixel_loss: bad arguments");
    if (!a || !b || !loss_accum) return fail(MV3D_E_INVAL, "mv3d_pixel_loss: null pointer");
    if (a_ld < ch || b_ld < ch || (grad && grad_ld < ch) || (mask && mask_ld < 1)) return fail(MV3D_E_INVAL, "mv3d_pixel_loss: pixel stride smaller than the channel count");
    PixelLossParams p = {pixels, ch, (const float*)a, a_ld, (const float*)b, b_ld, b_scale, (const float*)mask, mask_ld, kind, weight,
                         (float*)loss_accum, (float*)grad, grad_ld, next_loss_row()};
    const int64_t total = pixels * ch;
    const bool dense = a_ld == ch && b_ld == ch && (!grad || grad_ld == ch) && !mask && b_scale == 1.0f && (total & 3) == 0 &&
                       ((((uintptr_t)a) | ((uintptr_t)b) | ((uintptr_t)grad)) & 15) == 0;
    if (dense) {
        const int64_t total4 = total >> 2;
        const int blocks4 = (int)std::min<int64_t>(cdiv64(total4, 256 * 2), 256);
        return dispatch(stream, OpInfo{"pixel_loss", 0.0, (double)total * (grad ? 12.0 : 8.0)}, [=](hipStream_t s) {
            pixel_loss_dense_kernel<<<blocks4, 256, 0, s>>>(total4, pixels, (const float4*)a, (const float4*)b, kind, weight,
                                                           (float*)loss_accum, (float4*)grad, p.loss_row);
            return launched("pixel_loss_dense_kernel");
        });
    }
    const int blocks = (int)std::min<int64_t>(cdiv64(total, 256 * 8), 256);
    return dispatch(stream, OpInfo{"pixel_loss", 0.0, (double)total * (grad ? 12.0 : 8.0)}, [=](hipStream_t s) {
        pixel_loss_kernel<<<blocks, 256, 0, s>>>(p);
        return launched("pixel_loss_kernel");
    });
}

int mv3d_pixel_loss(int64_t pixels, int ch, const void* a, const void* b, const void* mask, int kind, float weight,
                    void* loss_accum, void* grad, void* stream) {
    return mv3d_pixel_loss_strided(pixels, ch, a, ch, b, ch, 1.0f, mask, 1, kind, weight, loss_accum, grad, ch, stream);
}

int mv3d_fill(void* dst, int64_t count, float value, void* stream) {
    if (!dst || count < 0) return fail(MV3D_E_INVAL, "mv3d_fill: bad arguments");
    if (count == 0) return MV3D_OK;
    return dispatch(stream, OpInfo{"fill", 0.0, 4.0 * count}, [=](hipStream_t s) {
        fill_kernel<<<grid_for(count), 256, 0, s>>>((float*)dst, count, value);
        return launched("fill_kernel");
    });
}

int mv3d_u8_to_unit_f32(int64_t count, const void* src, void* dst, void* stream) {
    if (count <= 0 || !src || !dst) return fail(MV3D_E_INVAL, "mv3d_u8_to_unit_f32: bad arguments");
    if (((uintptr_t)src & 3) || ((uintptr_t)dst & 15)) return fail(MV3D_E_INVAL, "mv3d_u8_to_unit_f32: src must be 4-byte and dst 16-byte aligned");
    return dispatch(stream, OpInfo{"u8_to_unit_f32", 0.0, 5.0 * count}, [=](hipStream_t s) {
        u8_to_unit_f32_kernel<<<grid_for(count / 4 + 1), 256, 0, s>>>(count, (const unsigned char*)src, (float*)dst);
        return launched("u8_to_unit_f32_kernel");
    });
}

static int parse_skips(const char* who, int64_t count, int nskip, const int64_t* skip_lo, const int64_t* skip_hi, AdamSkips& sk,
                       int64_t& skipped) {
    if (nskip < 0 || nskip > 8 || (nskip > 0 && (!skip_lo || !skip_hi))) return fail(MV3D_E_INVAL, "%s: at most 8 skipped ranges", who);
    sk = {};
    sk.n = nskip;
    skipped = 0;
    for (int r = 0; r < nskip; ++r) {
        if ((skip_lo[r] & 3) || (skip_hi[r] & 3) || skip_lo[r] < 0 || skip_hi[r] > count || skip_lo[r] > skip_hi[r])
            return fail(MV3D_E_INVAL, "%s: skipped range %d is not a multiple-of-4 sub-range", who, r);
        if (r > 0 && skip_lo[r] < skip_hi[r - 1]) return fail(MV3D_E_INVAL, "%s: skipped ranges must be sorted and disjoint", who);
        sk.lo[r] = skip_lo[r]; sk.hi[r] = skip_hi[r];
        skipped += skip_hi[r] - skip_lo[r];
    }
    return MV3D_OK;
}

int mv3d_adam_step(int64_t count, void* p, const void* g, void* m, void* v, float lr, float beta1, float beta2,
                   float eps, float beta1_power, float beta2_power, float grad_scale, void* stream) {
    if (count <= 0 || !p || !g || !m || !v) return fail(MV3D_E_INVAL, "mv3d_adam_step: bad arguments");
    if (((uintptr_t)p | (uintptr_t)g | (uintptr_t)m | (uintptr_t)v) & 15) return fail(MV3D_E_INVAL, "mv3d_adam_step: buffers must be 16-byte aligned");
    const float alpha = lr * sqrtf(1.0f - beta2_power) / (1.0f - beta1_power);
    const float omb1 = 1.0f - beta1, omb2 = 1.0f - beta2;
    const int blocks = (int)std::min<int64_t>(cdiv64(count / 4 + 1, 256), 4096);
    return dispatch(stream, OpInfo{"adam", 0.0, 28.0 * count}, [=](hipStream_t s) {
        adam_kernel<<<blocks, 256, 0, s>>>(count, (float*)p, (const float*)g, (float*)m, (float*)v, alpha, omb1, omb2, eps, grad_scale);
        return launched("adam_kernel");
    });
}

int mv3d_adam_step_dev(int64_t count, void* p, const void* g, void* m, void* v, const void* state, int nskip, const int64_t* skip_lo,
                       const int64_t* skip_hi, void* stream) {
    if (count <= 0 || (count & 3) || !p || !g || !m || !v || !state) return fail(MV3D_E_INVAL, "mv3d_adam_step_dev: bad arguments (count must be a multiple of 4)");
    if (((uintptr_t)p | (uintptr_t)g | (uintptr_t)m | (uintptr_t)v) & 15) return fail(MV3D_E_INVAL, "mv3d_adam_step_dev: buffers must be 16-byte aligned");
    AdamSkips sk;
    int64_t skipped;
    if (int rc = parse_skips("mv3d_adam_step_dev", count, nskip, skip_lo, skip_hi, sk, skipped)) return rc;
    const int blocks = (int)std::min<int64_t>(cdiv64((count - skipped) / 4 + 1, 256), 4096);
    return dispatch(stream, OpInfo{"adam", 0.0, 28.0 * (count - skipped)}, [=](hipStream_t s) {
        adam_dev_kernel<<<blocks, 256, 0, s>>>(count, (float*)p, (const float*)g, (float*)m, (float*)v, (const float*)state, sk);
        return launched("adam_dev_kernel");
    });
}

int mv3d_adam_advance(void* state, void* stream) {
    if (!state) return fail(MV3D_E_INVAL, "mv3d_adam_advance: null state");
    return dispatch(stream, OpInfo{"adam_advance", 0.0, 16.0}, [=](hipStream_t s) {
        adam_advance_kernel<<<1, 64, 0, s>>>((float*)state);
        return launched("adam_advance_kernel");
    });
}

int mv3d_sgd_step(int64_t count, void* p, const void* g, void* accum, float lr, float momentum, int use_nesterov, float grad_scale,
                  void* stream) {
    if (count <= 0 || !p || !g) return fail(MV3D_E_INVAL, "mv3d_sgd_step: bad arguments");
    if (((uintptr_t)p | (uintptr_t)g | (uintptr_t)accum) & 15) return fail(MV3D_E_INVAL, "mv3d_sgd_step: buffers must be 16-byte aligned");
    if (!accum && (momentum != 0.0f || use_nesterov))
        return fail(MV3D_E_INVAL, "mv3d_sgd_step: momentum / use_nesterov need the accumulator (accum == NULL is gradient descent)");
    const bool mom = accum != nullptr;
    const int nest = use_nesterov ? 1 : 0;
    const int blocks = (int)std::min<int64_t>(cdiv64(count / 4 + 1, 256), 4096);
    return dispatch(stream, OpInfo{mom ? "momentum" : "sgd", 0.0, (mom ? 20.0 : 12.0) * count}, [=](hipStream_t s) {
        if (mom) sgd_kernel<true><<<blocks, 256, 0, s>>>(count, (float*)p, (const float*)g, (float*)accum, lr, momentum, nest, grad_scale);
        else sgd_kernel<false><<<blocks, 256, 0, s>>>(count, (float*)p, (const float*)g, nullptr, lr, 0.0f, 0, grad_scale);
        return launched("sgd_kernel");
    });
}

int mv3d_sgd_step_dev(int64_t count, void* p, const void* g, void* accum, const void* sgd_state, int nskip, const int64_t* skip_lo,
                      const int64_t* skip_hi, void* stream) {
    if (count <= 0 || (count & 3) || !p || !g || !sgd_state) return fail(MV3D_E_INVAL, "mv3d_sgd_step_dev: bad arguments (count must be a multiple of 4)");
    if (((uintptr_t)p | (uintptr_t)g | (uintptr_t)accum) & 15) return fail(MV3D_E_INVAL, "mv3d_sgd_step_dev: buffers must be 16-byte aligned");
    AdamSkips sk;
    int64_t skipped;
    if (int rc = parse_skips("mv3d_sgd_step_dev", count, nskip, skip_lo, skip_hi, sk, skipped)) return rc;
    const bool mom = accum != nullptr;
    const int blocks = (int)std::min<int64_t>(cdiv64((count - skipped) / 4 + 1, 256), 4096);
    return dispatch(stream, OpInfo{mom ? "momentum" : "sgd", 0.0, (mom ? 20.0 : 12.0) * (count - skipped)}, [=](hipStream_t s) {
        if (mom) sgd_dev_kernel<true><<<blocks, 256, 0, s>>>(count, (float*)p, (const float*)g, (float*)accum, (const float*)sgd_state, sk);
        else sgd_dev_kernel<false><<<blocks, 256, 0, s>>>(count, (float*)p, (const float*)g, nullptr, (const float*)sgd_state, sk);
        return launched("sgd_dev_kernel");
    });
}

int mv3d_act_fwd(int64_t rows, int ch, const void* x, int x_ld, void* y, int y_ld, int act, float leak, void* stream) {
    if (rows <= 0 || ch <= 0 || !x || !y || x_ld < ch || y_ld < ch) return fail(MV3D_E_INVAL, "mv3d_act_fwd: bad arguments");
    return dispatch(stream, OpInfo{"act_fwd", 0.0, 8.0 * rows * ch}, [=](hipStream_t s) {
        act_fwd_kernel<<<grid_for(rows * ch), 256, 0, s>>>(rows, ch, (const float*)x, x_ld, (float*)y, y_ld, act, leak);
        return launched("act_fwd_kernel");
    });
}

int mv3d_act_bwd(int64_t rows, int ch, const void* dy, int dy_ld, const void* ref, int ref_ld, void* dx, int dx_ld,
                 int act, float leak, void* stream) {
    if (rows <= 0 || ch <= 0 || !dy || !ref || !dx || dy_ld < ch || ref_ld < ch || dx_ld < ch) return fail(MV3D_E_INVAL, "mv3d_act_bwd: bad arguments");
    return dispatch(stream, OpInfo{"act_bwd", 0.0, 12.0 * rows * ch}, [=](hipStream_t s) {
        act_bwd_kernel<<<grid_for(rows * ch), 256, 0, s>>>(rows, ch, (const float*)dy, dy_ld, (const float*)ref, ref_ld, (float*)dx, dx_ld, act, leak);
        return launched("act_bwd_kernel");
    });
}

int mv3d_copy2d(int64_t rows, int ch, const void* src, int64_t src_ld, int64_t src_row_div, void* dst, int64_t dst_ld,
                int accumulate, void* stream) {
    if (rows <= 0 || ch <= 0 || !src || !dst || src_row_div < 1) return fail(MV3D_E_INVAL, "mv3d_copy2d: bad arguments");
    return dispatch(stream, OpInfo{"copy2d", 0.0, 8.0 * rows * ch}, [=](hipStream_t s) {
        copy2d_kernel<<<grid_for(rows * ch), 256, 0, s>>>(rows, ch, (const float*)src, src_ld, src_row_div, (float*)dst, dst_ld, accumulate);
        return launched("copy2d_kernel");
    });
}

int mv3d_group_sum(int64_t groups, int group, int ch, const void* src, int64_t src_ld, void* dst, int64_t dst_ld, void* stream) {
    if (groups <= 0 || group <= 0 || ch <= 0 || !src || !dst) return fail(MV3D_E_INVAL, "mv3d_group_sum: bad arguments");
    return dispatch(stream, OpInfo{"group_sum", 0.0, 4.0 * groups * ch * (group + 1)}, [=](hipStream_t s) {
        group_sum_kernel<<<grid_for(groups * ch), 256, 0, s>>>(groups, group, ch, (const float*)src, src_ld, (float*)dst, dst_ld);
        return launched("group_sum_kernel");
    });
}

int mv3d_loss_overwrite_next(void) { g_loss_overwrite = true; return MV3D_OK; }

int mv3d_grad_finalize_begin(void) {
    if (finalize_collecting()) return fail(MV3D_E_INVAL, "mv3d_grad_finalize_begin: a collection is already open on this thread");
    finalize_open();
    return MV3D_OK;
}
int mv3d_grad_finalize_add(void* grad, int64_t count) {
    if (!finalize_collecting()) return fail(MV3D_E_INVAL, "mv3d_grad_finalize_add: no open collection");
    if (!grad || count <= 0 || ((uintptr_t)grad & 15)) return fail(MV3D_E_INVAL, "mv3d_grad_finalize_add: bad range (16-byte aligned, count > 0)");
    finalize_push(nullptr, 0, count, (float*)grad);
    return MV3D_OK;
}
int mv3d_grad_finalize_abort(void) { finalize_take(nullptr); return MV3D_OK; }

static int fin_blocks(const FinSegHost& h) {
    if (h.nslab == 0) return (int)cdiv64(cdiv64(h.count, 4), 256);
    const bool vec = h.count % 4 == 0 && ((uintptr_t)h.part & 15) == 0;
    return (int)cdiv64(h.count, vec ? 64 : 16);
}
size_t mv3d_grad_finalize_table_bytes(void) {
    const std::vector<FinSegHost>* v = finalize_peek();
    if (!v) return 0;
    size_t blocks = 0;
    for (const FinSegHost& h : *v) blocks += fin_blocks(h);
    return ((v->size() * sizeof(FinSeg) + 255) & ~(size_t)255) + blocks * sizeof(int);
}
static int grad_finalize_launch(std::vector<FinSegHost>& segs, size_t need, void* table, size_t table_bytes, void* grads, void* params,
                                void* slot1, void* slot2, const void* state, int opt, void* stream) {
    const bool upd = opt != OPT_NONE;
    std::vector<FinSegHost> keep;
    for (size_t a = 0; a < segs.size(); ++a) {
        const FinSegHost& h = segs[a];
        bool dup = false;
        for (size_t b = 0; b < segs.size(); ++b) {
            if (b == a || segs[b].out != h.out) continue;
            if (h.nslab == 0 && (segs[b].nslab > 0 || b < a)) dup = true;
            if (h.nslab > 0 && segs[b].nslab > 0 && b < a) return fail(MV3D_E_INVAL, "mv3d_grad_finalize_commit: two filter gradients write the same range");
        }
        if (!dup && (upd || h.nslab > 0)) keep.push_back(h);
    }
    if (keep.empty()) return MV3D_OK;
    const bool dry = !table && recording();
    if (!dry && (!table || table_bytes < need || ((uintptr_t)table & 15))) return fail(MV3D_E_WORKSPACE, "mv3d_grad_finalize_commit: table %zu < %zu bytes", table_bytes, need);
    std::vector<FinSeg> dev(keep.size());
    std::vector<int> seg_of;
    double bytes = 0.0;
    for (size_t j = 0; j < keep.size(); ++j) {
        const FinSegHost& h = keep[j];
        FinSeg& d = dev[j];
        d.part = h.part; d.out = h.out; d.count = h.count; d.nslab = h.nslab; d.pad = 0;
        d.vec = h.nslab > 0 && h.count % 4 == 0 && ((uintptr_t)h.part & 15) == 0;
        d.off = 0;
        if (upd) {
            const int64_t off = h.out - (float*)grads;
            if (off < 0 || (h.nslab == 0 && (off & 3))) return fail(MV3D_E_INVAL, "mv3d_grad_finalize_commit: segment %zu is not inside the flat gradient buffer", j);
            d.off = off;
        }
        d.blk0 = (int)seg_of.size();
        const int nb = fin_blocks(h);
        seg_of.insert(seg_of.end(), nb, (int)j);
        bytes += 4.0 * h.count * (h.nslab + (opt == OPT_ADAM ? 6 : opt == OPT_MOMENTUM ? 4 : opt == OPT_GD ? 2 : 1));
    }
    const size_t seg_bytes = (dev.size() * sizeof(FinSeg) + 255) & ~(size_t)255;
    if (!dry && (hipMemcpy(table, dev.data(), dev.size() * sizeof(FinSeg), hipMemcpyHostToDevice) != hipSuccess ||
                 hipMemcpy((char*)table + seg_bytes, seg_of.data(), seg_of.size() * sizeof(int), hipMemcpyHostToDevice) != hipSuccess))
        return fail(MV3D_E_HIP, "mv3d_grad_finalize_commit: table upload failed");
    const FinSeg* dsegs = (const FinSeg*)table;
    const int* dmap = (const int*)((char*)table + seg_bytes);
    const int blocks = (int)seg_of.size();
    const char* label = opt == OPT_ADAM ? "grad_finalize_adam" : opt == OPT_MOMENTUM ? "grad_finalize_momentum" : opt == OPT_GD ? "grad_finalize_sgd" : "grad_finalize";
    return dispatch(stream, OpInfo{label, 0.0, bytes}, [=](hipStream_t s) {
        const float* G = (const float*)grads; float* P = (float*)params; const float* st = (const float*)state;
        if (opt == OPT_ADAM) grad_finalize_kernel<OPT_ADAM><<<blocks, 256, 0, s>>>(dsegs, dmap, G, P, (float*)slot1, (float*)slot2, st);
        else if (opt == OPT_MOMENTUM) grad_finalize_kernel<OPT_MOMENTUM><<<blocks, 256, 0, s>>>(dsegs, dmap, G, P, (float*)slot1, nullptr, st);
        else if (opt == OPT_GD) grad_finalize_kernel<OPT_GD><<<blocks, 256, 0, s>>>(dsegs, dmap, G, P, nullptr, nullptr, st);
        else grad_finalize_kernel<OPT_NONE><<<blocks, 256, 0, s>>>(dsegs, dmap, nullptr, nullptr, nullptr, nullptr, nullptr);
        return launched("grad_finalize_kernel");
    });
}

int mv3d_grad_finalize_commit(void* table, size_t table_bytes, void* grads, void* params, void* adam_m, void* adam_v,
                              const void* adam_state, void* stream) {
    if (!finalize_collecting()) return fail(MV3D_E_INVAL, "mv3d_grad_finalize_commit: no open collection");
    const size_t need = mv3d_grad_finalize_table_bytes();
    std::vector<FinSegHost> segs;
    finalize_take(&segs);
    const bool adam = adam_state != nullptr;
    if (adam && (!grads || !params || !adam_m || !adam_v || (((uintptr_t)grads | (uintptr_t)params | (uintptr_t)adam_m | (uintptr_t)adam_v) & 15)))
        return fail(MV3D_E_INVAL, "mv3d_grad_finalize_commit: the optimiser needs the four flat buffers (16-byte aligned)");
    return grad_finalize_launch(segs, need, table, table_bytes, grads, params, adam_m, adam_v, adam_state, adam ? OPT_ADAM : OPT_NONE, stream);
}

int mv3d_grad_finalize_commit_sgd(void* table, size_t table_bytes, void* grads, void* params, void* accum, const void* sgd_state,
                                  void* stream) {
    if (!finalize_collecting()) return fail(MV3D_E_INVAL, "mv3d_grad_finalize_commit_sgd: no open collection");
    const size_t need = mv3d_grad_finalize_table_bytes();
    std::vector<FinSegHost> segs;
    finalize_take(&segs);
    if (!grads || !params || !sgd_state || (((uintptr_t)grads | (uintptr_t)params | (uintptr_t)accum) & 15))
        return fail(MV3D_E_INVAL, "mv3d_grad_finalize_commit_sgd: the optimiser needs the flat gradient, parameter (and momentum) buffers, 16-byte aligned, and the state");
    return grad_finalize_launch(segs, need, table, table_bytes, grads, params, accum, nullptr, sgd_state, accum ? OPT_MOMENTUM : OPT_GD, stream);
}

}
```

### dynamic_multiview_3d_amd/csrc/reduce_common.h

```cpp
#pragma once
#include "common.h"

namespace mv3d {

template <int VEC, class FIN>
__device__ __forceinline__ void reduce_slabs_body(const float* __restrict__ part, int nslab, int64_t count,
                                                  int blk, float (*s_sum)[16][17], FIN fin) {
    const int e = threadIdx.x & 15, sl = threadIdx.x >> 4;
    const int64_t i = ((int64_t)blk * 16 + e) * VEC;
    float acc[8][VEC];
#pragma unroll
    for (int u = 0; u < 8; ++u)
#pragma unroll
        for (int v = 0; v < VEC; ++v) acc[u][v] = 0.f;
    if (i < count) {
        const float* p = part + (int64_t)sl * count + i;
        const int64_t step = 16 * count;
        int k = sl;
        for (; k + 112 < nslab; k += 128, p += 8 * step) {
#pragma unroll
            for (int u = 0; u < 8; ++u) {
                if constexpr (VEC == 4) {
                    const float4 t = *reinterpret_cast<const float4*>(p + u * step);
                    acc[u][0] += t.x; acc[u][1] += t.y; acc[u][2] += t.z; acc[u][3] += t.w;
                } else {
                    acc[u][0] += p[u * step];
                }
            }
        }
        for (; k < nslab; k += 16, p += step) {
            if constexpr (VEC == 4) {
                const float4 t = *reinterpret_cast<const float4*>(p);
                acc[0][0] += t.x; acc[0][1] += t.y; acc[0][2] += t.z; acc[0][3] += t.w;
            } else {
                acc[0][0] += p[0];
            }
        }
    }
#pragma unroll
    for (int v = 0; v < VEC; ++v)
        s_sum[v][sl][e] = ((acc[0][v] + acc[1][v]) + (acc[2][v] + acc[3][v])) + ((acc[4][v] + acc[5][v]) + (acc[6][v] + acc[7][v]));
    __syncthreads();
    if (sl < VEC && i < count) {
        float t = 0.f;
#pragma unroll
        for (int j = 0; j < 16; ++j) t += s_sum[sl][j][e];
        fin(i + sl, t);
    }
}

}
```

### dynamic_multiview_3d_amd/graph.py

```python
import ctypes as C
import os
import math
from collections import OrderedDict

import numpy as np
import torch

from . import _lib
from ._lib import ACT_NONE, ACT_LRELU, ACT_RELU, ACT_TANH

_current = []


def current_graph():
    if not _current:
        raise RuntimeError("no Graph is active: build models inside `with Graph(...) as g:`")
    return _current[-1]


class Storage:

    def __init__(self, rows, ch, alias_of=None):
        self.rows, self.ch = rows, ch
        self.parent, self.ch_off = None, 0
        self.alias_of = alias_of
        self.has_alias = False
        self.data = None
        self.grad = None
        self.needs_grad = False
        self.external = False
        if alias_of is not None:
            alias_of.has_alias = True

    def resolve(self):
        s, off = self, 0
        while s.parent is not None:
            off += s.ch_off
            s = s.parent
        return s, off

    def can_be_adopted(self):
        return self.parent is None and self.alias_of is None and not self.has_alias and not self.external


class Tensor:
    def __init__(self, graph, shape, storage=None, ch_off=0, producer=None, act=ACT_NONE, leak=0.2,
                 requires_grad=False, name=None):
        self.graph = graph
        self.shape = tuple(int(s) for s in shape)
        self.C = self.shape[-1]
        self.rows = int(np.prod(self.shape[:-1])) if len(self.shape) > 1 else 1
        self.storage = storage if storage is not None else Storage(self.rows, self.C)
        self.ch_off = ch_off
        self.producer = producer
        self.act, self.leak = act, leak
        self.requires_grad = requires_grad
        self.name = name
        self.fused_into = None
        self.grad_consumers = 0
        self.grad_written = False
        self.grad_masked = False
        if requires_grad:
            self.storage.needs_grad = True

    def get_shape(self):
        return list(self.shape)

    def _root(self):
        s = self.storage
        if s.alias_of is not None:
            root, off = s.alias_of.resolve()
            assert off == 0 and root.ch == s.alias_of.ch
            return root, 0, s.ch
        root, off = s.resolve()
        return root, off, root.ch

    @property
    def ld(self):
        return self._root()[2]

    @property
    def ptr(self):
        root, off, _ = self._root()
        return root.data.data_ptr() + 4 * (off + self.ch_off)

    @property
    def grad_ptr(self):
        root, off, _ = self._root()
        return root.grad.data_ptr() + 4 * (off + self.ch_off)

    def _view(self, buf):
        root, off, ld = self._root()
        v = buf.view(-1, ld)[:, off + self.ch_off: off + self.ch_off + self.C]
        return v.reshape(self.shape) if v.is_contiguous() else v.unflatten(0, self.shape[:-1])

    def value(self):
        return self._view(self._root()[0].data)

    def grad_value(self):
        return self._view(self._root()[0].grad)

    def numpy(self):
        return self.value().detach().cpu().numpy().copy()

    def set(self, array):
        t = torch.as_tensor(np.ascontiguousarray(array, dtype=np.float32)) if not torch.is_tensor(array) else array
        self.value().copy_(t.reshape(self.shape), non_blocking=True)


class Variable:
    def __init__(self, name, shape, init):
        self.name, self.shape, self.init = name, tuple(shape), init
        self.size = int(np.prod(shape))
        self.offset = None
        self.graph = None
        self.has_grad = False

    @property
    def ptr(self):
        return self.graph.params.data_ptr() + 4 * self.offset

    @property
    def grad_ptr(self):
        return self.graph.grads.data_ptr() + 4 * self.offset

    def value(self):
        self.graph._settle()
        return self.graph.params[self.offset:self.offset + self.size].view(self.shape)

    def grad_value(self):
        self.graph._settle()
        return self.graph.grads[self.offset:self.offset + self.size].view(self.shape)


class ScalarExpr:

    def __init__(self, terms=()):
        self.terms = list(terms)

    def __add__(self, o):
        if isinstance(o, (int, float)):
            if o != 0:
                raise NotImplementedError("adding a non-zero constant to a loss")
            return ScalarExpr(self.terms)
        return ScalarExpr(self.terms + o.terms)

    __radd__ = __add__

    def __mul__(self, c):
        return ScalarExpr([(w * float(c), t) for w, t in self.terms])

    __rmul__ = __mul__


LOSS_L1, LOSS_L2, LOSS_SSIM, LOSS_SMOOTH = 1, 2, 3, 4


class LossTerm:

    def __init__(self, a, b, kind, mask=None, b_scale=1.0, max_val=1.0, edge_alpha=0.0, eps=1e-3):
        self.a, self.b, self.kind, self.mask, self.b_scale = a, b, kind, mask, float(b_scale)
        self.max_val = float(max_val)
        self.edge_alpha, self.eps = float(edge_alpha), float(eps)
        self.ws = None


class Node:
    def forward(self, g):
        raise NotImplementedError

    def backward(self, g):
        pass


def _epi(bias=None, act=ACT_NONE, leak=0.2, mask_of=None):
    if mask_of is not None and mask_of.act != ACT_NONE:
        return _lib.epilogue(bias, act, leak, mask_of.act, mask_of.leak, mask_of.ptr, mask_of.ld)
    return _lib.epilogue(bias, act, leak)


def _ensure_premasked(g, t):
    if t.act != ACT_NONE and not t.grad_masked:
        g.lib.act_bwd(t.rows, t.C, t.grad_ptr, t.ld, t.ptr, t.ld, t.grad_ptr, t.ld, t.act, t.leak, g.stream)
        t.grad_masked = True


def _note_grad_written(x, masked):
    x.grad_written = True
    x.grad_masked = masked


class ConvNode(Node):

    def __init__(self, x, y, w, b, kh, kw, sh, sw, transposed):
        self.x, self.y, self.w, self.b = x, y, w, b
        self.k = (kh, kw, sh, sw)
        self.transposed = transposed
        self.act, self.leak = ACT_NONE, 0.2

    def geom(self):
        kh, kw, sh, sw = self.k
        img, feat = (self.y, self.x) if self.transposed else (self.x, self.y)
        n, h, w, c = img.shape
        return _lib.conv_geom(n, h, w, c, feat.shape[3], kh, kw, sh, sw, img.ld, feat.ld)

    def workspace_bytes(self, g):
        return g.lib.conv_workspace_bytes(C.byref(self.geom()))

    def wgrad_partial_bytes(self, g):
        return int(g.lib.conv_wgrad_workspace_bytes(C.byref(self.geom())))

    def forward(self, g):
        geom = self.geom()
        epi = _epi(self.b.ptr if self.b is not None else None, self.act, self.leak)
        fn = g.lib.deconv2d_fwd if self.transposed else g.lib.conv2d_fwd
        fn(C.byref(geom), self.x.ptr, self.w.ptr, self.y.ptr, C.byref(epi), g.ws_ptr, g.ws_bytes, g.stream)

    def backward(self, g):
        y, x = self.y, self.x
        if not y.grad_written:
            return
        _ensure_premasked(g, y)
        geom = self.geom()
        ws_side = g.begin_side()
        ws_len = g.ws_bytes
        if g._finalizing:
            ws_side, ws_len = g._part_arena.data_ptr() + self._part_off, self._part_bytes
        if self.transposed:
            g.lib.deconv2d_wgrad(C.byref(geom), x.ptr, y.grad_ptr, self.w.grad_ptr, ws_side, ws_len, g.stream)
        else:
            g.lib.conv2d_wgrad(C.byref(geom), x.ptr, y.grad_ptr, self.w.grad_ptr,
                               self.b.grad_ptr if self.b is not None else None, ws_side, ws_len, g.stream)
        g.end_side()
        self.w.has_grad = True
        if self.b is not None:
            self.b.has_grad = True
        if x.requires_grad:
            epi = _epi(mask_of=x)
            fn = g.lib.deconv2d_dgrad if self.transposed else g.lib.conv2d_dgrad
            fn(C.byref(geom), y.grad_ptr, self.w.ptr, x.grad_ptr, C.byref(epi), g.ws_ptr, g.ws_bytes, g.stream)
            _note_grad_written(x, x.act != ACT_NONE)


class LinearNode(Node):

    def __init__(self, x, y, m, b):
        self.x, self.y, self.m, self.b = x, y, m, b
        self.act, self.leak = ACT_NONE, 0.2

    def workspace_bytes(self, g):
        return g.lib.fc_workspace_bytes(self.x.shape[0], self.x.C, self.y.C)

    chain = None

    def forward(self, g):
        x, y = self.x, self.y
        if self.chain is not None:
            if self is not self.chain[-1]:
                return
            c = _lib.FcChain()
# ... 100 lines not shown
                    _ensure_premasked(g, o)
        for i in self.ins:
            if i.requires_grad:
                if want_mask and i.act == ACT_NONE:
                    raise RuntimeError("view of mixed activation / linear tensors cannot carry a masked gradient")
                _note_grad_written(i, want_mask)


class CopyConcatNode(Node):

    def __init__(self, ins, out):
        self.ins, self.out = ins, out

    def forward(self, g):
        off = 0
        for t in self.ins:
            g.lib.copy2d(t.rows, t.C, t.ptr, t.ld, 1, self.out.ptr + 4 * off, self.out.ld, 0, g.stream)
            off += t.C

    def backward(self, g):
        o = self.out
        if not o.grad_written:
            return
        off = 0
        for t in self.ins:
            if t.requires_grad:
                g.lib.copy2d(t.rows, t.C, o.grad_ptr + 4 * off, o.ld, 1, t.grad_ptr, t.ld, 0, g.stream)
                _note_grad_written(t, o.grad_masked and t.act != ACT_NONE)
                if o.grad_masked and t.act == ACT_NONE:
                    raise RuntimeError("masked gradient reached a linear tensor through concat")
            off += t.C


class TileNode(Node):

    def __init__(self, x, y, reps):
        self.x, self.y, self.reps = x, y, reps

    def forward(self, g):
        x, y = self.x, self.y
        g.lib.copy2d(y.rows, y.C, x.ptr, x.ld, self.reps, y.ptr, y.ld, 0, g.stream)

    def backward(self, g):
        x, y = self.x, self.y
        if not y.grad_written or not x.requires_grad:
            return
        g.lib.group_sum(x.rows, self.reps, x.C, y.grad_ptr, y.ld, x.grad_ptr, x.ld, g.stream)
        _note_grad_written(x, y.grad_masked)


class ResampleNode(Node):

    def __init__(self, src, flow, warp, gen):
        self.src, self.flow, self.warp, self.gen = src, flow, warp, gen
        self.fused_loss = None

    def workspace_bytes(self, g):
        if not self.src.requires_grad:
            return 0
        n, h, w, _ = self.flow.shape
        _, hs, ws, c = self.src.shape
        return g.lib.resampler_bwd_workspace_bytes(n, h * w, hs, ws, c)

    def forward(self, g):
        n, h, w, _ = self.flow.shape
        _, hs, ws, c = self.src.shape
        if self.fused_loss is not None:
            wgt, term = self.fused_loss
            want_grad = self.flow.requires_grad
            g.lib.warp_resample_loss(n, h, w, hs, ws, c, self.src.ptr, self.flow.ptr, self.flow.ld, term.b.ptr, term.b.ld,
                                     term.kind, float(wgt), self.warp.ptr, self.gen.ptr,
                                     self.flow.grad_ptr if want_grad else None, self.flow.ld, g.loss_buf.data_ptr(), g.stream)
            if want_grad:
                _note_grad_written(self.flow, False)
            return
        g.lib.warp_resample_fwd(n, h, w, hs, ws, c, self.src.ptr, self.flow.ptr, self.flow.ld,
                                self.warp.ptr, self.gen.ptr, g.stream)

    def backward(self, g):
        if self.fused_loss is not None or not self.gen.grad_written:
            return
        n, h, w, _ = self.flow.shape
        _, hs, ws, c = self.src.shape
        if self.flow.requires_grad:
            g.lib.warp_resample_bwd(n, h, w, hs, ws, c, self.src.ptr, self.flow.ptr, self.flow.ld,
                                    self.gen.grad_ptr, self.flow.grad_ptr, self.flow.ld, g.stream)
            _note_grad_written(self.flow, False)
        if self.src.requires_grad:
            g.lib.resampler_bwd(n, h * w, hs, ws, c, self.src.ptr, self.src.ld, self.warp.ptr, 2, self.gen.grad_ptr, self.gen.ld,
                                None, 0, self.src.grad_ptr, self.src.ld, g.ws_ptr, g.ws_bytes, g.stream)
            _note_grad_written(self.src, False)


class ResamplerNode(Node):

    def __init__(self, src, warp, out):
        self.src, self.warp, self.out = src, warp, out

    def _dims(self):
        n, hs, ws, c = self.src.shape
        return n, self.warp.rows // n, hs, ws, c

    def workspace_bytes(self, g):
        return g.lib.resampler_bwd_workspace_bytes(*self._dims()) if self.src.requires_grad else 0

    def forward(self, g):
        src, warp, out = self.src, self.warp, self.out
        g.lib.resampler_fwd(*self._dims(), src.ptr, src.ld, warp.ptr, warp.ld, out.ptr, out.ld, g.stream)

    def backward(self, g):
        src, warp, out = self.src, self.warp, self.out
        if not out.grad_written or not (warp.requires_grad or src.requires_grad):
            return
        g.lib.resampler_bwd(*self._dims(), src.ptr, src.ld, warp.ptr, warp.ld, out.grad_ptr, out.ld,
                            warp.grad_ptr if warp.requires_grad else None, warp.ld,
                            src.grad_ptr if src.requires_grad else None, src.ld, g.ws_ptr, g.ws_bytes, g.stream)
        for t in (warp, src):
            if t.requires_grad:
                _note_grad_written(t, False)


class Graph:

    ALIGN = 64

    def __init__(self, device=None, seed=1234):
        self.device = torch.device(device if device is not None else 'cuda')
        self.rng = np.random.default_rng(seed)
        self.nodes = []
        self.tensors = []
        self.inputs = OrderedDict()
        self.variables = OrderedDict()
        self._scope = []
        self.loss_expr = None
        self.lr = None
        self.finalized = False
        self.lib = None
        self.stream = None
        self.ws = None
        self.ws_ptr, self.ws_bytes = None, 0
        self.n_side = max(0, min(4, int(os.environ.get('MV3D_SIDE_STREAMS', '2'))))
        self.ws_side = []
        self.side_streams = None
        self.adam_stream = None
        self.adam_timing = None
        self.overlap_adam = os.environ.get('MV3D_OVERLAP_ADAM', '1') != '0'
        self.fuse_fc_adam = os.environ.get('MV3D_FUSE_FC_ADAM', '1') != '0'
        self._fusing = False
        self.fuse_finalize = os.environ.get('MV3D_FUSE_FINALIZE', '1') != '0'
        self.finalize_chunk_bytes = int(float(os.environ.get('MV3D_FINALIZE_CHUNK_MB', '48')) * 1e6)
        self._finalizing = False
        self._finalized_in_plan = False
        self._part_arena = self._fin_table = None
        self._fused_vars = []
        self.pipeline_fc = os.environ.get('MV3D_PIPELINE_FCADAM', '1') != '0'
        self.pipeline_dp = os.environ.get('MV3D_PIPELINE_DP', '1') != '0'
        self.pipeline_dp_min_idx = 8
        self._fused_nodes = []
        self._fwd_wait_idx = 0
        self._fc_event = None
        self._fc_pending = False
        self._pending_idx = 0
        self.plan_bwd_fused = None
        self.opt_state = None
        self.plan_fwd = self.plan_bwd = None
        self._smooth_deferred = []
        self.optimizer = 'adam'
        self.momentum, self.use_nesterov = 0.0, False
        self.adam_m = self.adam_v = self.accum = None
        self.beta1, self.beta2, self.eps = 0.9, 0.999, 1e-8
        self.beta1_power = np.float32(self.beta1)
        self.beta2_power = np.float32(self.beta2)
        self.world_size, self.dist_group = 1, None
        self.comm = None
        self.dp_mode = 'sharded'
        self.comm_stream = None
        self.bucket_elems = 16 * 1024 * 1024

    OPTIMIZERS = ('adam', 'momentum', 'sgd')

    @property
    def adam_state(self):
        return self.opt_state

    def __enter__(self):
        _current.append(self)
        return self

    def __exit__(self, *a):
        _current.pop()

    def scope_name(self, name):
        return '/'.join(self._scope + [name])

    def variable(self, name, shape, init):
        full = self.scope_name(name)
        if full in self.variables:
            raise ValueError("variable %s already exists" % full)
        v = Variable(full, shape, init)
        v.graph = self
        self.variables[full] = v
        return v

    def placeholder(self, shape, name):
        t = Tensor(self, shape, name=name)
        t.storage.external = True
        self.inputs[name] = t
        self.tensors.append(t)
        return t

    def new_tensor(self, shape, **kw):
        t = Tensor(self, shape, **kw)
        self.tensors.append(t)
        return t

    def add(self, node):
        self.nodes.append(node)
        return node

    def finalize(self):
        if self.finalized:
            return
        self.lib = _lib.lib()
        dev = self.device
        roots = []
        for t in self.tensors:
            s = t.storage
            base = s.alias_of if s.alias_of is not None else s
            root, _ = base.resolve()
            if s.needs_grad:
                root.needs_grad = True
            if root not in roots:
                roots.append(root)
        act_bytes = 0
        for r in roots:
            r.data = torch.zeros(r.rows * r.ch, dtype=torch.float32, device=dev)
            act_bytes += r.rows * r.ch * 4
            if r.needs_grad:
                r.grad = torch.zeros(r.rows * r.ch, dtype=torch.float32, device=dev)
                act_bytes += r.rows * r.ch * 4
        self.activation_bytes = act_bytes
        off = 0
        for v in self.variables.values():
            v.offset = off
            off += -(-v.size // self.ALIGN) * self.ALIGN
        self.flat_size = off
        host = np.zeros(off, dtype=np.float32)
        for v in self.variables.values():
            host[v.offset:v.offset + v.size] = v.init(self.rng, v.shape).reshape(-1)
        self.params = torch.from_numpy(host).to(dev)
        self.grads = torch.zeros(off, dtype=torch.float32, device=dev)
        if self.optimizer not in self.OPTIMIZERS:
            raise ValueError("unknown optimizer %r (have %s)" % (self.optimizer, ', '.join(self.OPTIMIZERS)))
        if self.optimizer == 'adam':
            self.adam_m = torch.zeros(off, dtype=torch.float32, device=dev)
            self.adam_v = torch.zeros(off, dtype=torch.float32, device=dev)
        elif self.optimizer == 'momentum':
            self.accum = torch.zeros(off, dtype=torch.float32, device=dev)
        self.opt_state = torch.zeros(16, dtype=torch.float32, device=dev)
        self.loss_buf = torch.zeros(4, dtype=torch.float32, device=dev)
        self.zero_buf = torch.zeros(1024, dtype=torch.float32, device=dev)
        self.zero_ptr = self.zero_buf.data_ptr()
        self.finalized = True
        need = 0
        for n in self.nodes:
            if hasattr(n, 'workspace_bytes'):
                need = max(need, int(n.workspace_bytes(self)))
        self.ws_bytes = need
        self.ws = torch.empty(max(need // 4, 4), dtype=torch.float32, device=dev)
        self.ws_ptr = self.ws.data_ptr()
        self.ws_side = [torch.empty(max(need // 4, 4), dtype=torch.float32, device=dev) for _ in range(self.n_side)]

    def _fuse_resample_losses(self):
        self.fused_terms = set()
        enabled = os.environ.get('MV3D_FUSE_RESAMPLE', '1') != '0'
        for n in self.nodes:
            if not isinstance(n, ResampleNode):
                continue
            n.fused_loss = None
            if not enabled or self.loss_expr is None or n.src.requires_grad:
                continue
            gen = n.gen
            uses = [(w, t) for w, t in self.loss_expr.terms if t.a is gen or t.b is gen or t.mask is gen]
            if len(uses) != 1:
                continue
            w, t = uses[0]
            if t.kind == LOSS_SSIM:
                continue
            if t.a is not gen or t.mask is not None or t.b_scale != 1.0 or t.b.requires_grad or t.b.rows != gen.rows or t.b.C != gen.C:
                continue
            if gen.C > 4 or gen.ld != gen.C or gen.storage.has_alias or gen.storage.alias_of is not None:
                continue
            read_elsewhere = False
            for m in self.nodes:
                if m is n:
                    continue
                for v in vars(m).values():
                    vs = v if isinstance(v, (list, tuple)) else (v,)
                    if any(x is gen for x in vs):
                        read_elsewhere = True
            if read_elsewhere:
                continue
            n.fused_loss = (w, t)
            self.fused_terms.add(id(t))

    def _find_fc_chains(self):
        for n in self.nodes:
            if isinstance(n, LinearNode):
                n.chain = None
        cur = self.lib.set_diagnostics(0)
        self.lib.set_diagnostics(cur)
        if os.environ.get('MV3D_FC_CHAINS', '1') == '0' or (cur & 4):
            return
        def tensors_of(node):
            for val in vars(node).values():
                for t in (val if isinstance(val, (list, tuple)) else (val,)):
                    if isinstance(t, Tensor):
                        yield t
        users = {}
        for n in self.nodes:
            for t in tensors_of(n):
                users.setdefault(id(t._root()[0]), set()).add(id(n))
        small = lambda n: isinstance(n, LinearNode) and n.x.C <= 64 and n.y.C <= 64 and n.b is not None
        nxt = {}
        for n in self.nodes:
            if not small(n):
                continue
            root = id(n.y._root()[0])
            if len(users.get(root, ())) != 2:
                continue
            for m in self.nodes:
                if m is not n and small(m) and id(m.x._root()[0]) == root and m.x.ptr == n.y.ptr and m.x.C == n.y.C and m.x.ld == n.y.ld:
                    nxt[id(n)] = m
        heads = [n for n in self.nodes if id(n) in nxt and not any(v is n for v in nxt.values())]
        for h in heads:
            chain = [h]
            while id(chain[-1]) in nxt and len(chain) < 4:
                chain.append(nxt[id(chain[-1])])
            if len(chain) >= 2:
                for n in chain:
                    n.chain = chain

    def _emit_losses(self, with_grad):
        if self.loss_expr is None:
            return
        written = set()
        order = lambda k: 2 if k == LOSS_SMOOTH else 1 if k == LOSS_SSIM else 0
        terms = sorted(self.loss_expr.terms, key=lambda wt: order(wt[1].kind))
        self._smooth_deferred = []
        for w, term in terms:
            if id(term) in self.fused_terms:
                continue
            a, b, m = term.a, term.b, term.mask
            if term.kind == LOSS_SMOOTH:
                both = with_grad and a.requires_grad and a.grad_written
                self._smooth_launch(w, term, value=True, grad=both, accumulate=both)
                if with_grad and a.requires_grad and not both:
                    self._smooth_deferred.append((w, term))
                continue
            if a.C != b.C or a.rows != b.rows:
                raise ValueError("loss operands of different shapes")
            grad = a.grad_ptr if (with_grad and a.requires_grad) else None
            if term.kind == LOSS_SSIM:
                n, h, wd, c = a.shape
                self.lib.ssim_loss(n, h, wd, c, a.ptr, a.ld, b.ptr, b.ld, term.max_val, float(w), self.loss_buf.data_ptr(), grad, a.ld,
                                   1 if grad in written else 0, term.ws.data_ptr(), term.ws.numel(), self.stream)
            else:
                self.lib.pixel_loss_strided(a.rows, a.C, a.ptr, a.ld, b.ptr, b.ld, term.b_scale,
                                            m.ptr if m is not None else None, m.ld if m is not None else 1,
                                            term.kind, float(w), self.loss_buf.data_ptr(), grad, a.ld, self.stream)
            if grad is not None:
                written.add(grad)
                _note_grad_written(a, False)

    def _smooth_launch(self, w, term, value, grad, accumulate):
        a, b = term.a, term.b
        if grad and accumulate and a.grad_masked:
            raise NotImplementedError("flow_smoothness_loss on a tensor whose gradient buffer already holds d/d(pre-activation)")
        n, h, wd, _ = a.shape
        self.lib.flow_smoothness(n, h, wd, a.ptr, a.ld, b.ptr if b is not None else None, b.C if b is not None else 0,
                                 b.ld if b is not None else 0, term.edge_alpha, term.eps, float(w),
                                 self.loss_buf.data_ptr() if value else None, a.grad_ptr if grad else None, a.ld,
                                 1 if (grad and accumulate) else 0, term.ws.data_ptr(), term.ws.numel(), self.stream)
        if grad:
            _note_grad_written(a, False)

    def _smooth_before(self, n, pending):
        for wt in [wt for wt in pending if wt[1].a.producer is n]:
            self._smooth_launch(wt[0], wt[1], value=False, grad=True, accumulate=wt[1].a.grad_written)
            pending.remove(wt)

    def _smooth_after(self, pending):
        for wt in [wt for wt in pending if wt[1].a.grad_written]:
            self._smooth_launch(wt[0], wt[1], value=False, grad=True, accumulate=True)
            pending.remove(wt)

    def _backward_node(self, n, pending):
        self._smooth_before(n, pending)
        n.backward(self)
        self._smooth_after(pending)

    @staticmethod
    def _smooth_all_placed(pending):
        if pending:
            raise RuntimeError("flow_smoothness_loss: the reverse pass has no place for the gradient of %d term(s): no node of "
                               "this graph produces the tensor" % len(pending))

    def compile(self, stream=None):
        self.finalize()
        self.stream = stream
        lib = self.lib
        for t in self.tensors:
            t.grad_written = t.grad_masked = False
        self._smooth_deferred = []
        self._bind_prepared_filters()
        self._fuse_resample_losses()
        for _, term in (self.loss_expr.terms if self.loss_expr is not None else ()):
            if term.kind == LOSS_SSIM and term.ws is None:
                nbytes = int(lib.ssim_loss_workspace_bytes(*term.a.shape))
                if not nbytes:
                    raise ValueError("ssim_loss: operands of shape %s are outside what mv3d_ssim_loss takes" % (term.a.shape,))
                term.ws = torch.empty(nbytes, dtype=torch.uint8, device=self.device)
            if term.kind == LOSS_SMOOTH and term.ws is None:
                nbytes = int(lib.flow_smoothness_workspace_bytes(*term.a.shape[:3]))
                if not nbytes:
                    raise ValueError("flow_smoothness_loss: a flow of shape %s is outside what mv3d_flow_smoothness takes" % (term.a.shape,))
                term.ws = torch.empty(nbytes, dtype=torch.uint8, device=self.device)
        self._find_fc_chains()
        self.plan_fwd = lib.plan_create()
        lib.plan_begin(self.plan_fwd)
        try:
            lib.filter_cache_refresh(None)
            if self.loss_expr is not None and self.loss_expr.terms:
                lib.loss_overwrite_next()
            else:
                lib.fill(self.loss_buf.data_ptr(), 1, 0.0, self.stream)
            self._fwd_first_op = {}
            for n in self.nodes:
                self._fwd_first_op[id(n)] = lib.plan_size(self.plan_fwd)
                n.forward(self)
            self._emit_losses(with_grad=True)
        finally:
            lib.plan_end()
        flags_after_forward = [(t.grad_written, t.grad_masked) for t in self.tensors]
        self.plan_bwd = lib.plan_create()
        lib.plan_begin(self.plan_bwd)
        self.grad_buckets = []
        try:
            done = set()
            order = list(self.variables.values())
            suffix = len(order)
            cut_hi = self.flat_size
            gate = 0
            pending = list(self._smooth_deferred)
            for n in reversed(self.nodes):
                self._backward_node(n, pending)
                if isinstance(n, LinearNode):
                    gate = lib.plan_size(self.plan_bwd)
                for v in (getattr(n, 'w', None), getattr(n, 'b', None), getattr(n, 'm', None)):
                    if isinstance(v, Variable):
                        done.add(v.name)
                while suffix > 0 and order[suffix - 1].name in done:
                    suffix -= 1
                lo = order[suffix].offset if suffix < len(order) else self.flat_size
                boundary = False
                if isinstance(n, ConvNode) and cut_hi > lo:
                    for prev in reversed(self.nodes[:self.nodes.index(n)]):
                        if any(isinstance(v, Variable) for v in vars(prev).values()):
                            boundary = isinstance(prev, LinearNode)
                            break
                if cut_hi - lo >= self.bucket_elems or boundary:
                    self.grad_buckets.append((lib.plan_size(self.plan_bwd), lo, cut_hi))
                    cut_hi = lo
            self._smooth_all_placed(pending)
        finally:
            lib.plan_end()
        nbwd = lib.plan_size(self.plan_bwd)
        if cut_hi > 0 or not self.grad_buckets:
            self.grad_buckets.append((nbwd, 0, cut_hi))
        else:
            end, lo, hi = self.grad_buckets[-1]
            self.grad_buckets[-1] = (nbwd, lo, hi)
        mode = os.environ.get('MV3D_ADAM_GATE', '0.9')
        if mode == 'none':
            gate = 0
        elif mode != 'fc':
            gate = int(float(mode) * nbwd)
        self.adam_gate = gate if 0 < gate < nbwd else 0
        if self.adam_gate and all(b[0] != self.adam_gate for b in self.grad_buckets):
            i = next(j for j, b in enumerate(self.grad_buckets) if b[0] > self.adam_gate)
            hi = self.grad_buckets[i][2]
            self.grad_buckets.insert(i, (self.adam_gate, hi, hi))
        self.n_launch_fwd = lib.plan_size(self.plan_fwd)
        self.n_launch_bwd = lib.plan_size(self.plan_bwd)
        self._bucket_first_use = [self._first_param_use(lo, hi) for _, lo, hi in self.grad_buckets]
        self.plan_bwd_fused = None
        self._fused_vars = []
        self._fused_nodes = []
        if self.fuse_fc_adam and self.lr is not None and any(isinstance(n, LinearNode) for n in self.nodes):
            for t, (gw, gm) in zip(self.tensors, flags_after_forward):
                t.grad_written, t.grad_masked = gw, gm
            plan = lib.plan_create()
            self._finalized_in_plan = False
            if self.fuse_finalize:
                off = 0
                for n in self.nodes:
                    if isinstance(n, ConvNode):
                        n._part_off, n._part_bytes = off, n.wgrad_partial_bytes(self)
                        off += -(-n._part_bytes // 256) * 256
                self._part_arena = torch.empty(max(off // 4, 4), dtype=torch.float32, device=self.device)
                lib.grad_finalize_begin()
                self._finalizing = True
                self._fin_pending, self._fin_vars, self._fin_done, self._fin_tables = 0, [], set(), []
            lib.plan_begin(plan)
            self._fusing = True
            pending = list(self._smooth_deferred)
            try:
                for n in reversed(self.nodes):
                    self._backward_node(n, pending)
                    if self._finalizing and isinstance(n, ConvNode) and n.w.has_grad:
                        self._fin_pending += n._part_bytes
                        self._fin_vars += [n.w] + ([n.b] if n.b is not None else [])
                        if self._fin_pending >= self.finalize_chunk_bytes:
                            self._finalize_commit()
                            lib.grad_finalize_begin()
                self._smooth_all_placed(pending)
                for n in self._fused_nodes:
                    n.record_fused_update(self)
                if self._finalizing and self._fused_vars:
                    fused = {id(v) for v in self._fused_vars} | {id(n.b) for n in self._fused_nodes}
                    for v in self.variables.values():
                        if v.has_grad and id(v) not in fused and id(v) not in self._fin_done:
                            lib.grad_finalize_add(v.grad_ptr, -(-v.size // 4) * 4)
                    self._finalize_commit()
                    self._finalizing = False
                    self._finalized_in_plan = True
            finally:
                self._fusing = False
                if self._finalizing:
                    lib.grad_finalize_abort()
                    self._finalizing = False
                lib.plan_end()
            if self._fused_vars:
                self.plan_bwd_fused = plan
                self.n_launch_bwd_fused = lib.plan_size(plan)
                def merged(ranges):
                    out = []
                    for lo, hi in sorted(ranges):
                        if out and lo <= out[-1][1]:
                            out[-1][1] = max(out[-1][1], hi)
                        else:
                            out.append([lo, hi])
                    return out
                pad4 = lambda v: (v.offset, v.offset + -(-v.size // 4) * 4)
                biases = merged(pad4(n.b) for n in self._fused_nodes)
                skips = merged([pad4(v) for v in self._fused_vars] + [tuple(b) for b in biases])
                assert len(skips) <= 8, "mv3d_adam_step_dev leaves at most 8 ranges untouched"
                self._skip_lo = (C.c_int64 * len(skips))(*[a for a, _ in skips])
                self._skip_hi = (C.c_int64 * len(skips))(*[b for _, b in skips])
                self._bias_span = (biases[0][0], biases[-1][1])
                gaps = [(biases[i][1] - biases[0][0], biases[i + 1][0] - biases[0][0]) for i in range(len(biases) - 1)]
                assert len(gaps) <= 8
                self._bias_skip = (len(gaps), (C.c_int64 * max(1, len(gaps)))(*[a for a, _ in gaps] or [0]),
                                   (C.c_int64 * max(1, len(gaps)))(*[b for _, b in gaps] or [0]))
                self._fwd_wait_idx = self._first_fc_hazard()
            else:
                lib.plan_destroy(plan)
        self.upload_optimizer_state()
        return self

    def _finalize_commit(self):
        lib = self.lib
        on_gpu = torch.device(self.device).type == 'cuda'
        tb = int(lib.grad_finalize_table_bytes())
        table = torch.empty(max(tb, 16), dtype=torch.uint8, device=self.device) if on_gpu else None
        self._fin_tables.append(table)
        self.begin_side()
        try:
            tp = table.data_ptr() if on_gpu else None
            if self.optimizer == 'adam':
                lib.grad_finalize_commit(tp, tb, self.grads.data_ptr(), self.params.data_ptr(),
                                         self.adam_m.data_ptr(), self.adam_v.data_ptr(), self.opt_state.data_ptr(), self.stream)
            else:
                lib.grad_finalize_commit_sgd(tp, tb, self.grads.data_ptr(), self.params.data_ptr(),
                                             self.accum.data_ptr() if self.accum is not None else None, self.opt_state.data_ptr(),
                                             self.stream)
        finally:
            self.end_side()
        self._fin_done |= {id(v) for v in self._fin_vars}
        self._fin_pending, self._fin_vars = 0, []

    def _bind_prepared_filters(self):
        lib = self.lib
        lib.filter_cache_clear()
        self._prepared = []
        if torch.device(self.device).type != 'cuda':
            return
        for n in self.nodes:
            if not isinstance(n, ConvNode):
                continue
            geom = n.geom()
            ops = [2 if n.transposed else 0]
            if n.x.requires_grad:
                ops.append(3 if n.transposed else 1)
            for op in ops:
                nbytes = int(lib.filter_prepared_bytes(C.byref(geom), op))
                if nbytes > 0:
                    buf = torch.empty(nbytes, dtype=torch.uint8, device=self.device)
                    self._prepared.append(buf)
                    lib.filter_cache_bind(C.byref(geom), op, n.w.ptr, buf.data_ptr(), nbytes)
        tb = int(lib.filter_cache_table_bytes())
        self._prepared_table = torch.empty(max(tb, 16), dtype=torch.uint8, device=self.device)
        lib.filter_cache_commit(self._prepared_table.data_ptr(), tb, None)

    def _stream_ptr(self):
        return torch.cuda.current_stream(self.device).cuda_stream

    def _first_param_use(self, lo, hi):
        first = self.n_launch_fwd
        for n in self.nodes:
            for name, val in vars(n).items():
                if isinstance(val, Variable) and val.offset is not None and lo <= val.offset < hi:
                    first = min(first, 0 if (isinstance(n, ConvNode) and name == 'w') else self._fwd_first_op[id(n)])
        return first

    def _first_fc_hazard(self):
        roots = set()
        for n in self._fused_nodes:
            root = n.x._root()[0]
            if root.external or n.x.storage.external:
                return None
            roots.add(id(root))
        def tensors_of(node):
            for val in vars(node).values():
                for t in (val if isinstance(val, (list, tuple)) else (val,)):
                    if isinstance(t, Tensor):
                        yield t
        fused = {id(n) for n in self._fused_nodes}
        idx = self.n_launch_fwd
        for n in self.nodes:
            if id(n) in fused or any(id(t._root()[0]) in roots for t in tensors_of(n)):
                idx = min(idx, self._fwd_first_op[id(n)])
        return idx

    def _settle(self):
        if self._fc_pending:
            torch.cuda.current_stream(self.device).wait_event(self._fc_event)
            self._fc_pending = False

    settle = _settle

    def run_forward(self):
        st = self._stream_ptr()
        if self._fc_pending and 0 < self._pending_idx < self.n_launch_fwd:
            self.lib.plan_run_range(self.plan_fwd, 0, self._pending_idx, st)
            self._settle()
            self.lib.plan_run_range(self.plan_fwd, self._pending_idx, self.n_launch_fwd, st)
            return
        self._settle()
        self.lib.plan_run(self.plan_fwd, st)

    def begin_side(self, cls=1):
        if self.n_side == 0:
            return self.ws_ptr
        k = (cls - 1) % self.n_side
        self.lib.plan_side(k + 1)
        return self.ws_side[k].data_ptr()

    def end_side(self):
        if self.n_side:
            self.lib.plan_side(0)

    def _side_ptrs(self):
        if self.n_side == 0 or torch.device(self.device).type != 'cuda':
            return None, 0
        if self.side_streams is None:
            self.side_streams = [torch.cuda.Stream(device=self.device) for _ in range(self.n_side)]
            self._side_arr = (C.c_void_p * self.n_side)(*[st.cuda_stream for st in self.side_streams])
        return self._side_arr, self.n_side

    def run_backward(self):
        self._settle()
        sides, ns = self._side_ptrs()
        self.lib.plan_run_range_multi(self.plan_bwd, 0, self.n_launch_bwd, self._stream_ptr(), sides, ns, 0)

    def allreduce_grads(self):
        self._settle()
        if self.world_size > 1:
            self.comm.allreduce_sum_(self.grads, 0, self.flat_size, self._stream_ptr())

    def upload_optimizer_state(self):
        if self.opt_state is None or self.lr is None:
            return
        if self.optimizer == 'adam':
            vals = [self.lr, self.beta1, self.beta2, self.eps, self.beta1_power, self.beta2_power]
        else:
            vals = [self.lr, self.momentum, 1.0 if self.use_nesterov else 0.0, 0.0, 0.0, 0.0]
        vals = np.array(vals + [1.0 / self.world_size, 0.0], np.float32)
        self._settle()
        self.opt_state.copy_(torch.from_numpy(np.concatenate([vals, vals])))

    upload_adam_state = upload_optimizer_state

    def _opt_range(self, lo, hi, stream, skips=None, state=None):
        off = lo * 4
        n, slo, shi = (0, None, None) if skips is None else skips
        state = self.opt_state.data_ptr() if state is None else state
        if self.optimizer == 'adam':
            self.lib.adam_step_dev(hi - lo, self.params.data_ptr() + off, self.grads.data_ptr() + off, self.adam_m.data_ptr() + off,
                                   self.adam_v.data_ptr() + off, state, n, slo, shi, stream)
        else:
            self.lib.sgd_step_dev(hi - lo, self.params.data_ptr() + off, self.grads.data_ptr() + off,
                                  self.accum.data_ptr() + off if self.accum is not None else None, state, n, slo, shi, stream)

    _adam_range = _opt_range

    def _adam_advance(self, stream=None, both=True):
        if self.optimizer != 'adam':
            return
        st = self._stream_ptr() if stream is None else stream
        self.lib.adam_advance(self.opt_state.data_ptr(), st)
        if both:
            self.lib.adam_advance(self.opt_state.data_ptr() + 32, st)
        self.beta1_power = np.float32(self.beta1_power * np.float32(self.beta1))
        self.beta2_power = np.float32(self.beta2_power * np.float32(self.beta2))

    def apply_optimizer(self):
        self._settle()
        self._opt_range(0, self.flat_size, self._stream_ptr())
        self._adam_advance()

    apply_adam = apply_optimizer

    def run_backward_fused(self):
        sides, ns = self._side_ptrs()
        st = self._stream_ptr()
        pipelined = self.pipeline_fc and ns >= 2 and self._fwd_wait_idx is not None
        self.lib.plan_run_range_multi(self.plan_bwd_fused, 0, self.n_launch_bwd_fused, st, sides, ns, 1 if pipelined else 0)
        fc_state = self.opt_state.data_ptr() + 32
        if pipelined:
            main = torch.cuda.current_stream(self.device)
            for k, q in enumerate(self.side_streams):
                if k != 1 % ns:
                    main.wait_stream(q)
            fcq = self.side_streams[1 % ns]
            fc_stream = fcq.cuda_stream
        else:
            fc_stream = st
        lo, hi = self._bias_span
        self._opt_range(lo, hi, fc_stream, self._bias_skip, state=fc_state)
        if self.optimizer == 'adam':
            self.lib.adam_advance(fc_state, fc_stream)
        if pipelined:
            if self._fc_event is None:
                self._fc_event = torch.cuda.Event()
            self._fc_event.record(fcq)
            self._fc_pending = True
            self._pending_idx = self._fwd_wait_idx
        if not self._finalized_in_plan:
            self._opt_range(0, self.flat_size, st, (len(self._skip_lo), self._skip_lo, self._skip_hi))
        self._adam_advance(st, both=False)

    def run_backward_with_adam(self):
        self._settle()
        main = torch.cuda.current_stream(self.device)
        sides, ns = self._side_ptrs()
        if self.adam_stream is None:
            self.adam_stream = torch.cuda.Stream(device=self.device)
        begin, pending = 0, []
        for end, lo, hi in self.grad_buckets:
            self.lib.plan_run_range_multi(self.plan_bwd, begin, end, main.cuda_stream, sides, ns, 1)
            begin = end
            if hi > lo:
                pending.append((lo, hi))
            if end < self.adam_gate or not pending:
                continue
            self.adam_stream.wait_stream(main)
            for st in (self.side_streams or []):
                self.adam_stream.wait_stream(st)
            for plo, phi in pending:
                if self.adam_timing is not None:
                    e0, e1 = torch.cuda.Event(enable_timing=True), torch.cuda.Event(enable_timing=True)
                    e0.record(self.adam_stream)
                self._opt_range(plo, phi, self.adam_stream.cuda_stream)
                if self.adam_timing is not None:
                    e1.record(self.adam_stream)
                    self.adam_timing.append((e0, e1))
            pending = []
        main.wait_stream(self.adam_stream)
        for st in (self.side_streams or []):
            main.wait_stream(st)
        self._adam_advance(main.cuda_stream)

    run_backward_with_optimizer = run_backward_with_adam

    def run_backward_overlapped(self, with_adam=False):
        self._settle()
        main = self._stream_ptr()
        sides, ns = self._side_ptrs()
        on_gpu = torch.device(self.device).type == 'cuda'
        if on_gpu and self.comm_stream is None:
            self.comm_stream = torch.cuda.Stream(device=self.device)
        cs = self.comm_stream.cuda_stream if on_gpu else None
        comm, W = self.comm, self.world_size
        begin = 0
        late = []
        for end, lo, hi in self.grad_buckets:
            self.lib.plan_run_range_multi(self.plan_bwd, begin, end, main, sides, ns, 1 if on_gpu else 0)
            begin = end
            if hi <= lo:
                continue
            if on_gpu:
                self.comm_stream.wait_stream(torch.cuda.current_stream(self.device))
                for q in (self.side_streams or []):
                    self.comm_stream.wait_stream(q)
                ctx = torch.cuda.stream(self.comm_stream)
                ctx.__enter__()
            if self.dp_mode == 'sharded' and with_adam:
                n = (hi - lo) // W
                assert n * W == hi - lo and n % 4 == 0, "bucket not divisible by 4 * world"
                comm.reduce_scatter_sum_(self.grads, lo, n, cs)
                a = lo + comm.rank * n
                self._opt_range(a, a + n, cs)
                self._slots_sharded = bool(self._slots())
                use = self._bucket_first_use[self.grad_buckets.index((end, lo, hi))]
                if self.pipeline_dp and use >= self.pipeline_dp_min_idx:
                    late.append((use, lo, n))
                else:
                    comm.allgather_(self.params, lo, n, cs)
            else:
                comm.allreduce_sum_(self.grads, lo, hi - lo, cs)
                if with_adam:
                    self._opt_range(lo, hi, cs)
            if on_gpu:
                ctx.__exit__(None, None, None)
        if on_gpu:
            cur = torch.cuda.current_stream(self.device)
            cur.wait_stream(self.comm_stream)
            for q in (self.side_streams or []):
                cur.wait_stream(q)
        if late:
            late.sort()
            if on_gpu:
                ctx = torch.cuda.stream(self.comm_stream)
                ctx.__enter__()
            for _, lo, n in late:
                comm.allgather_(self.params, lo, n, cs)
            if on_gpu:
                ctx.__exit__(None, None, None)
                if self._fc_event is None:
                    self._fc_event = torch.cuda.Event()
                self._fc_event.record(self.comm_stream)
                self._fc_pending = True
                self._pending_idx = late[0][0]
        if with_adam:
            self._adam_advance()

    def train_step(self):
        self.run_forward()
        if self.world_size > 1:
            self.run_backward_overlapped(with_adam=True)
        elif self.plan_bwd_fused is not None:
            self.run_backward_fused()
        elif self.overlap_adam and torch.device(self.device).type == 'cuda':
            self.run_backward_with_adam()
        else:
            self.run_backward()
            self.apply_optimizer()
        return self.loss_buf[0]

    def get_variables(self):
        self._settle()
        return OrderedDict((k, v.value().detach().cpu().numpy().copy()) for k, v in self.variables.items())

    def set_variables(self, values):
        self._settle()
        for k, a in values.items():
            self.variables[k].value().copy_(torch.as_tensor(np.asarray(a, dtype=np.float32)).reshape(self.variables[k].shape))

    def get_gradients(self):
        self._settle()
        return OrderedDict((k, v.grad_value().detach().cpu().numpy().copy()) for k, v in self.variables.items() if v.has_grad)

    def _slots(self):
        if self.optimizer == 'adam':
            return [('Adam', self.adam_m), ('Adam_1', self.adam_v)]
        if self.optimizer == 'momentum':
            return [('Momentum', self.accum)]
        return []

    def gather_optimizer_state(self):
        self._settle()
        if self.world_size <= 1 or not getattr(self, '_slots_sharded', False):
            return
        on_gpu = torch.device(self.device).type == 'cuda'
        if on_gpu:
            torch.cuda.synchronize(self.device)
        cs = self._stream_ptr() if on_gpu else None
        W = self.world_size
        for _, lo, hi in self.grad_buckets:
            if hi > lo:
                n = (hi - lo) // W
                for _, buf in self._slots():
                    self.comm.allgather_(buf, lo, n, cs)
        if on_gpu:
            torch.cuda.synchronize(self.device)
        self._slots_sharded = False

    def state_dict(self):
        self._settle()
        if self.world_size > 1 and getattr(self, '_slots_sharded', False):
            raise RuntimeError("sharded data-parallel step: this rank holds 1/%d of the optimiser slots; call "
                               "Graph.gather_optimizer_state() on EVERY rank before state_dict() / Saver.save()" % self.world_size)
        sd = OrderedDict()
        slots = self._slots()
        for k, v in self.variables.items():
            sd[k] = v.value().detach().cpu().clone()
            if v.has_grad:
                for name, buf in slots:
                    sd[k + '/' + name] = buf[v.offset:v.offset + v.size].view(v.shape).detach().cpu().clone()
        if self.optimizer == 'adam':
            sd['beta1_power'] = torch.tensor(float(self.beta1_power))
            sd['beta2_power'] = torch.tensor(float(self.beta2_power))
        return sd

    def load_state_dict(self, sd):
        self._settle()
        slots = self._slots()
        names = {n for n, _ in slots}
        missing = [k for k in self.variables if k not in sd]
        if self.optimizer == 'momentum':
            missing += [k + '/Momentum' for k, v in self.variables.items() if v.has_grad and k + '/Momentum' not in sd]
        scalars = {'beta1_power', 'beta2_power'} if self.optimizer == 'adam' else set()
        unexpected = [k for k in sd if k not in scalars and k not in self.variables and
                      not (k.rsplit('/', 1)[0] in self.variables and k.rsplit('/', 1)[-1] in names)]
        bad = [k for k, v in self.variables.items() if k in sd and tuple(sd[k].shape) != tuple(v.shape)]
        if missing or unexpected or bad or not scalars <= set(sd):
            raise KeyError("checkpoint does not match the model (%s optimizer): missing %s; unexpected %s; shape mismatch %s%s"
                           % (self.optimizer, missing[:8], unexpected[:8], [(k, tuple(sd[k].shape), self.variables[k].shape) for k in bad[:8]],
                              '' if scalars <= set(sd) else '; no beta1_power / beta2_power'))
        for k, v in self.variables.items():
            v.value().copy_(sd[k])
            for name, buf in slots:
                if k + '/' + name in sd:
                    buf[v.offset:v.offset + v.size].view(v.shape).copy_(sd[k + '/' + name])
        if self.optimizer == 'adam':
            self.beta1_power = np.float32(float(sd['beta1_power']))
            self.beta2_power = np.float32(float(sd['beta2_power']))
        self.upload_optimizer_state()


def truncated_normal_init(stddev):
    def init(rng, shape):
        out = rng.standard_normal(shape)
        bad = np.abs(out) > 2
        while bad.any():
            out[bad] = rng.standard_normal(int(bad.sum()))
            bad = np.abs(out) > 2
        return (out * stddev).astype(np.float32)
    return init


def random_normal_init(stddev):
    return lambda rng, shape: (rng.standard_normal(shape) * stddev).astype(np.float32)


def zeros_init():
    return lambda rng, shape: np.zeros(shape, np.float32)
```

### include/mv3d_hip.h

```cpp
#ifndef MV3D_HIP_H
#define MV3D_HIP_H
#include <stddef.h>
#include <stdint.h>

#ifdef __cplusplus
extern "C" {
#endif

enum { MV3D_OK = 0, MV3D_E_INVAL = -1, MV3D_E_HIP = -2, MV3D_E_WORKSPACE = -3, MV3D_E_UNSUPPORTED = -4 };
enum { MV3D_F32 = 0 };
enum { MV3D_ACT_NONE = 0, MV3D_ACT_LRELU = 1, MV3D_ACT_RELU = 2, MV3D_ACT_TANH = 3 };

typedef struct mv3d_conv_geom {
    int32_t N;
    int32_t H, W, C;
    int32_t Ho, Wo, K;
    int32_t kh, kw, sh, sw;
    int32_t img_ld, feat_ld;
    int32_t dtype;
} mv3d_conv_geom;

typedef struct mv3d_epilogue {
    const void* bias;
    int32_t act;
    float leak;
    int32_t gmask_act;
    float gmask_leak;
    const void* gmask_ref;
    int32_t gmask_ld;
} mv3d_epilogue;

const char* mv3d_version(void);
const char* mv3d_last_error(void);
int mv3d_set_diagnostics(int mask);
int mv3d_set_wgrad_cus(int cus);

typedef struct mv3d_tfrecord_reader mv3d_tfrecord_reader;
int mv3d_tfrecord_open(const char* path, int verify_crc, mv3d_tfrecord_reader** out);
int mv3d_tfrecord_read(mv3d_tfrecord_reader* r, int max_records, int first, int nfeat, const char* const* names, const int* kinds,
                       const size_t* sizes, void* const* dst, int* nread);
void mv3d_tfrecord_close(mv3d_tfrecord_reader* r);
int mv3d_u8_to_unit_f32(int64_t count, const void* src, void* dst, void* stream);

int mv3d_u8_process_image(const void* src, int n, int hs, int ws, int c, void* dst, int ho, int wo, void* stream);

uint32_t mv3d_crc32c(const void* data, size_t n);

int mv3d_conv2d_fwd(const mv3d_conv_geom* g, const void* x, const void* w, void* y,
                    const mv3d_epilogue* epi, void* workspace, size_t workspace_bytes, void* stream);
int mv3d_conv2d_dgrad(const mv3d_conv_geom* g, const void* dy, const void* w, void* dx,
                      const mv3d_epilogue* epi, void* workspace, size_t workspace_bytes, void* stream);
int mv3d_conv2d_wgrad(const mv3d_conv_geom* g, const void* x, const void* dy, void* dw, void* db,
                      void* workspace, size_t workspace_bytes, void* stream);

int mv3d_deconv2d_fwd(const mv3d_conv_geom* g, const void* x, const void* w, void* y,
                      const mv3d_epilogue* epi, void* workspace, size_t workspace_bytes, void* stream);
int mv3d_deconv2d_dgrad(const mv3d_conv_geom* g, const void* dy, const void* w, void* dx,
                        const mv3d_epilogue* epi, void* workspace, size_t workspace_bytes, void* stream);
int mv3d_deconv2d_wgrad(const mv3d_conv_geom* g, const void* x, const void* dy, void* dw,
                        void* workspace, size_t workspace_bytes, void* stream);
size_t mv3d_conv_workspace_bytes(const mv3d_conv_geom* g);
size_t mv3d_conv_wgrad_workspace_bytes(const mv3d_conv_geom* g);

enum { MV3D_FILTER_CONV_FWD = 0, MV3D_FILTER_CONV_DGRAD = 1, MV3D_FILTER_DECONV_FWD = 2, MV3D_FILTER_DECONV_DGRAD = 3 };
size_t mv3d_filter_prepared_bytes(const mv3d_conv_geom* g, int op);
int mv3d_filter_cache_bind(const mv3d_conv_geom* g, int op, const void* w, void* prepared, size_t prepared_bytes);
size_t mv3d_filter_cache_table_bytes(void);
int mv3d_filter_cache_commit(void* table_dev, size_t table_bytes, void* stream);
int mv3d_filter_cache_refresh(void* stream);
int mv3d_filter_cache_clear(void);

int mv3d_fc_fwd(int B, int in, int out, const void* x, int x_ld, const void* M, void* y, int y_ld,
                const mv3d_epilogue* epi, void* workspace, size_t workspace_bytes, void* stream);
int mv3d_fc_dgrad(int B, int in, int out, const void* dy, int dy_ld, const void* M, void* dx, int dx_ld,
                  const mv3d_epilogue* epi, void* workspace, size_t workspace_bytes, void* stream);
int mv3d_fc_wgrad(int B, int in, int out, const void* x, int x_ld, const void* dy, int dy_ld,
                  void* dM, void* db, void* workspace, size_t workspace_bytes, void* stream);
int mv3d_fc_wgrad_dgrad(int B, int in, int out, const void* x, int x_ld, const void* dy, int dy_ld, const void* M,
                        void* dM, void* db, void* dx, int dx_ld, const mv3d_epilogue* dx_epi,
                        void* workspace, size_t workspace_bytes, void* stream);
#define MV3D_FC_CHAIN_MAX 4
typedef struct mv3d_fc_chain_layer {
    const void* M;
    const void* bias;
    void* y;
    int32_t y_ld, out;
    int32_t act;
    float leak;
} mv3d_fc_chain_layer;
typedef struct mv3d_fc_chain {
    int32_t B, nlayers, in, x_ld;
    const void* x;
    mv3d_fc_chain_layer l[MV3D_FC_CHAIN_MAX];
} mv3d_fc_chain;
int mv3d_fc_chain_fwd(const mv3d_fc_chain* chain, void* stream);
size_t mv3d_fc_workspace_bytes(int B, int in, int out);

int mv3d_act_fwd(int64_t rows, int ch, const void* x, int x_ld, void* y, int y_ld, int act, float leak, void* stream);
int mv3d_act_bwd(int64_t rows, int ch, const void* dy, int dy_ld, const void* ref, int ref_ld,
                 void* dx, int dx_ld, int act, float leak, void* stream);
int mv3d_copy2d(int64_t rows, int ch, const void* src, int64_t src_ld, int64_t src_row_div,
                void* dst, int64_t dst_ld, int accumulate, void* stream);
int mv3d_group_sum(int64_t groups, int group, int ch, const void* src, int64_t src_ld, void* dst, int64_t dst_ld, void* stream);

int mv3d_warp_resample_fwd(int N, int H, int W, int Hs, int Ws, int C, const void* src, const void* flow, int flow_ld,
                           void* warp_out, void* gen, void* stream);
int mv3d_warp_resample_bwd(int N, int H, int W, int Hs, int Ws, int C, const void* src, const void* flow, int flow_ld,
                           const void* dgen, void* dflow, int dflow_ld, void* stream);
int mv3d_warp_resample_loss(int N, int H, int W, int Hs, int Ws, int C, const void* src, const void* flow, int flow_ld,
                            const void* target, int target_ld, int kind, float weight, void* warp_out, void* gen,
                            void* dflow, int dflow_ld, void* loss_accum, void* stream);

int mv3d_resampler_fwd(int N, int P, int Hs, int Ws, int C, const void* data, int data_ld,
                       const void* warp, int warp_ld, void* out, int out_ld, void* stream);
size_t mv3d_resampler_bwd_workspace_bytes(int N, int P, int Hs, int Ws, int C);
int mv3d_resampler_bwd(int N, int P, int Hs, int Ws, int C, const void* data, int data_ld,
                       const void* warp, int warp_ld, const void* dout, int dout_ld,
                       void* dwarp, int dwarp_ld, void* ddata, int ddata_ld,
                       void* workspace, size_t workspace_bytes, void* stream);

int mv3d_pixel_loss(int64_t pixels, int ch, const void* a, const void* b, const void* mask, int kind, float weight,
                    void* loss_accum, void* grad, void* stream);
int mv3d_pixel_loss_strided(int64_t pixels, int ch, const void* a, int a_ld, const void* b, int b_ld, float b_scale,
                            const void* mask, int mask_ld, int kind, float weight, void* loss_accum, void* grad, int grad_ld,
                            void* stream);
int mv3d_fill(void* dst, int64_t count, float value, void* stream);
int mv3d_loss_overwrite_next(void);

size_t mv3d_image_metrics_workspace_bytes(int N, int H, int W, int C);
int mv3d_image_metrics(int N, int H, int W, int C, const void* a, int a_ld, const void* b, int b_ld, float max_val, void* out,
                       void* workspace, size_t workspace_bytes, void* stream);

size_t mv3d_ssim_loss_workspace_bytes(int N, int H, int W, int C);
int mv3d_ssim_loss(int N, int H, int W, int C, const void* a, int a_ld, const void* b, int b_ld, float max_val, float weight,
                   void* loss_accum, void* grad, int grad_ld, int grad_accumulate, void* workspace, size_t workspace_bytes,
                   void* stream);

size_t mv3d_flow_smoothness_workspace_bytes(int N, int H, int W);
int mv3d_flow_smoothness(int N, int H, int W, const void* flow, int flow_ld, const void* guide, int guide_c, int guide_ld,
                         float edge_alpha, float eps, float weight, void* loss_accum, void* grad, int grad_ld, int grad_accumulate,
                         void* workspace, size_t workspace_bytes, void* stream);

int mv3d_adam_step(int64_t count, void* p, const void* g, void* m, void* v, float lr, float beta1, float beta2,
                   float eps, float beta1_power, float beta2_power, float grad_scale, void* stream);

enum { MV3D_ADAM_LR = 0, MV3D_ADAM_BETA1 = 1, MV3D_ADAM_BETA2 = 2, MV3D_ADAM_EPS = 3, MV3D_ADAM_BETA1_POWER = 4, MV3D_ADAM_BETA2_POWER = 5,
       MV3D_ADAM_GSCALE = 6, MV3D_ADAM_STATE_FLOATS = 8 };
int mv3d_adam_step_dev(int64_t count, void* p, const void* g, void* m, void* v, const void* adam_state, int nskip,
                       const int64_t* skip_lo, const int64_t* skip_hi, void* stream);
int mv3d_adam_advance(void* adam_state, void* stream);
int mv3d_fc_wgrad_adam(int B, int in, int out, const void* x, int x_ld, const void* dy, int dy_ld, void* M, void* adam_m, void* adam_v,
                       void* db, const void* adam_state, void* stream);
int mv3d_fc_wgrad_adam_supported(int B, int in, int out, int x_ld, int dy_ld);

int mv3d_sgd_step(int64_t count, void* p, const void* g, void* accum, float lr, float momentum, int use_nesterov,
                  float grad_scale, void* stream);
enum { MV3D_SGD_LR = 0, MV3D_SGD_MOMENTUM = 1, MV3D_SGD_NESTEROV = 2, MV3D_SGD_GSCALE = 6, MV3D_SGD_STATE_FLOATS = 8 };
int mv3d_sgd_step_dev(int64_t count, void* p, const void* g, void* accum, const void* sgd_state, int nskip,
                      const int64_t* skip_lo, const int64_t* skip_hi, void* stream);
int mv3d_fc_wgrad_sgd(int B, int in, int out, const void* x, int x_ld, const void* dy, int dy_ld, void* M, void* accum,
                      void* db, const void* sgd_state, void* stream);

int mv3d_grad_finalize_begin(void);
int mv3d_grad_finalize_add(void* grad, int64_t count);
size_t mv3d_grad_finalize_table_bytes(void);
int mv3d_grad_finalize_commit(void* table, size_t table_bytes, void* grads, void* params, void* adam_m, void* adam_v,
                              const void* adam_state, void* stream);
int mv3d_grad_finalize_commit_sgd(void* table, size_t table_bytes, void* grads, void* params, void* accum, const void* sgd_state,
                                  void* stream);
int mv3d_grad_finalize_abort(void);

typedef struct mv3d_comm mv3d_comm;
int mv3d_comm_available(void);
int mv3d_comm_unique_id(void* id128);
int mv3d_comm_init(mv3d_comm** out, int rank, int world, const void* id128);
int mv3d_comm_destroy(mv3d_comm* comm);
int mv3d_comm_allreduce_sum(mv3d_comm* comm, void* buf, int64_t count, void* stream);
int mv3d_comm_reduce_scatter_sum(mv3d_comm* comm, const void* send, void* recv, int64_t recv_count, void* stream);
int mv3d_comm_allgather(mv3d_comm* comm, const void* send, void* recv, int64_t send_count, void* stream);

#define MV3D_MESH_MAX_RANKS 8
int mv3d_ipc_export(const void* ptr, void* handle64, int64_t* offset);
int mv3d_ipc_open(const void* handle64, void** base);
int mv3d_ipc_close(void* base);
int mv3d_mesh_reduce_sum(const void* const* srcs, int nsrc, void* dst, int64_t count, void* stream);
int mv3d_mesh_copy(void* dst, const void* src, int64_t count, void* stream);

typedef struct mv3d_plan mv3d_plan;
mv3d_plan* mv3d_plan_create(void);
void mv3d_plan_destroy(mv3d_plan* p);
int mv3d_plan_begin(mv3d_plan* p);
int mv3d_plan_end(void);
int mv3d_plan_size(const mv3d_plan* p);
int mv3d_plan_run(mv3d_plan* p, void* stream);
int mv3d_plan_run_range(mv3d_plan* p, int begin, int end, void* stream);
#define MV3D_MAX_SIDE 4
int mv3d_plan_side(int side);
#define MV3D_RUN_NO_JOIN 1
int mv3d_plan_run_range_multi(mv3d_plan* p, int begin, int end, void* stream, void* const* side_streams, int nside, int flags);
int mv3d_plan_profile(mv3d_plan* p, int enable);
int mv3d_plan_profile_collect(mv3d_plan* p);
int mv3d_plan_profile_select(mv3d_plan* p, const char* name);
int mv3d_plan_profile_reset(mv3d_plan* p);
int mv3d_plan_op_info(const mv3d_plan* p, int i, const char** name, double* flops, double* bytes,
                      double* total_ms, int* runs);

int mv3d_debug_cconv_stamps(void* host_dst, size_t bytes);
int mv3d_debug_cwgrad_stamps(void* host_dst, size_t bytes);
int mv3d_debug_band_stamps(void* host_dst, size_t bytes);

#ifdef __cplusplus
}
#endif
#endif
```

Measured before the change: 38200 images/sec.

## Write prepared bf16 split filter planes directly from fused Adam finalize kernel

The gradient-finalize/Adam kernel gains a plane mode: for conv filters bound in the prepared-filter cache, each block updates an 8x32 tile of weights, stages it in shared memory, then splits it into hi/lo bf16 and writes it straight into the cached tiled layout for each orientation. A lean forward plan without the filter-cache refresh pass can then run when all prepared filters were updated this way, tracked by a dirty flag. This removes a separate re-read and re-split of the filters before each forward, at the cost of more complex finalize indexing, extra writes and fallback bookkeeping.

```diff
diff --git a/dynamic_multiview_3d_amd/_lib.py b/dynamic_multiview_3d_amd/_lib.py
--- a/dynamic_multiview_3d_amd/_lib.py
+++ b/dynamic_multiview_3d_amd/_lib.py
@@ -80,6 +80,7 @@
     "mv3d_grad_finalize_commit": [_vp, _sz, _vp, _vp, _vp, _vp, _vp, _vp],
     "mv3d_grad_finalize_commit_sgd": [_vp, _sz, _vp, _vp, _vp, _vp, _vp],
     "mv3d_grad_finalize_abort": [],
+    "mv3d_grad_finalize_keep_planes": [_vp, _vp],
     "mv3d_comm_unique_id": [_vp],
     "mv3d_comm_init": [C.POINTER(_vp), _i, _i, _vp],
     "mv3d_comm_destroy": [_vp],
diff --git a/dynamic_multiview_3d_amd/build.py b/dynamic_multiview_3d_amd/build.py
--- a/dynamic_multiview_3d_amd/build.py
+++ b/dynamic_multiview_3d_amd/build.py
@@ -47,7 +47,8 @@
     hipcc = _hipcc()
     objdir = os.path.join(HERE, "build")
     os.makedirs(objdir, exist_ok=True)
-    headers = [os.path.join(CSRC, "common.h"), os.path.join(CSRC, "conv_common.h"), os.path.join(HERE, "..", "include", "mv3d_hip.h")]
+    headers = [os.path.join(CSRC, "common.h"), os.path.join(CSRC, "conv_common.h"), os.path.join(CSRC, "reduce_common.h"),
+               os.path.join(CSRC, "split_bf16.h"), os.path.join(HERE, "..", "include", "mv3d_hip.h")]
     objs = []
     for src, extra in UNITS.items():
         s = os.path.join(CSRC, src)
diff --git a/dynamic_multiview_3d_amd/csrc/bconv.hip b/dynamic_multiview_3d_amd/csrc/bconv.hip
--- a/dynamic_multiview_3d_amd/csrc/bconv.hip
+++ b/dynamic_multiview_3d_amd/csrc/bconv.hip
@@ -1,4 +1,5 @@
 #include "conv_common.h"
+#include "split_bf16.h"
 #include <algorithm>
 #include <mutex>
 #include <string.h>
@@ -7,18 +8,8 @@
 namespace mv3d {
 
 typedef __bf16 bf16x8 __attribute__((ext_vector_type(8)));
-typedef __bf16 bf16x4 __attribute__((ext_vector_type(4)));
 
 constexpr int BC_PIXB = 144;
-
-__device__ __forceinline__ void split4(const float4& v, uint2& hi, uint2& lo) {
-    bf16x4 h, l;
-    h[0] = (__bf16)v.x; h[1] = (__bf16)v.y; h[2] = (__bf16)v.z; h[3] = (__bf16)v.w;
-    l[0] = (__bf16)(v.x - (float)h[0]); l[1] = (__bf16)(v.y - (float)h[1]);
-    l[2] = (__bf16)(v.z - (float)h[2]); l[3] = (__bf16)(v.w - (float)h[3]);
-    hi = __builtin_bit_cast(uint2, h);
-    lo = __builtin_bit_cast(uint2, l);
-}
 
 
 template <int NTHR>
@@ -621,6 +612,22 @@
     return nullptr;
 }
 
+int bconv_cache_jobs_of(const float* Wt, PlaneJob* out, int max_out) {
+    std::lock_guard<std::mutex> lk(g_cache_mu);
+    int n = 0;
+    for (const SplitJob& j : g_jobs) {
+        if (j.Wt != Wt) continue;
+        if (n < max_out) {
+            PlaneJob& o = out[n];
+            o.Wf = j.Wf; o.ntaps = j.ntaps; o.chunks = j.chunks; o.ntiles = j.ntiles; o.Ka = j.Ka; o.Cc = j.Cc;
+            o.w_tap_stride = j.w_tap_stride; o.w_ks = j.w_ks; o.w_ns = j.w_ns;
+            memcpy(o.widx, j.widx, sizeof(o.widx));
+        }
+        ++n;
+    }
+    return n;
+}
+
 size_t bconv_prepared_bytes(const IgemmParams& p) {
     if (p.fold || p.Ka % 16 != 0 || p.Cc < 16) return 0;
     const int ntaps = p.tap_begin[p.so_h * p.so_w];
diff --git a/dynamic_multiview_3d_amd/csrc/common.h b/dynamic_multiview_3d_amd/csrc/common.h
--- a/dynamic_multiview_3d_amd/csrc/common.h
+++ b/dynamic_multiview_3d_amd/csrc/common.h
@@ -54,6 +54,8 @@
 namespace mv3d {
 const std::vector<FinSegHost>* finalize_peek();
 void finalize_take(std::vector<FinSegHost>* out);
+void finalize_set_planes(const float* grads, const float* params);
+bool finalize_planes(const float** grads, const float** params);
 
 int disabled_paths();
 
diff --git a/dynamic_multiview_3d_amd/csrc/core.hip b/dynamic_multiview_3d_amd/csrc/core.hip
--- a/dynamic_multiview_3d_amd/csrc/core.hip
+++ b/dynamic_multiview_3d_amd/csrc/core.hip
@@ -63,8 +63,16 @@
     return labels->insert(buf).first->c_str();
 }
 static thread_local std::vector<FinSegHost>* g_fin = nullptr;
+static thread_local const float* g_fin_plane_grads = nullptr;
+static thread_local const float* g_fin_plane_params = nullptr;
 bool finalize_collecting() { return g_fin != nullptr; }
-void finalize_open() { if (!g_fin) g_fin = new std::vector<FinSegHost>(); }
+void finalize_open() { if (!g_fin) { g_fin = new std::vector<FinSegHost>(); g_fin_plane_grads = g_fin_plane_params = nullptr; } }
+void finalize_set_planes(const float* grads, const float* params) { g_fin_plane_grads = grads; g_fin_plane_params = params; }
+bool finalize_planes(const float** grads, const float** params) {
+    if (!g_fin || !g_fin_plane_params) return false;
+    *grads = g_fin_plane_grads; *params = g_fin_plane_params;
+    return true;
+}
 void finalize_push(const float* part, int nslab, int64_t count, float* out) { if (g_fin) g_fin->push_back(FinSegHost{part, nslab, count, out}); }
 const std::vector<FinSegHost>* finalize_peek() { return g_fin; }
 void finalize_take(std::vector<FinSegHost>* out) {
@@ -72,6 +80,7 @@
     if (out) out->swap(*g_fin);
     delete g_fin;
     g_fin = nullptr;
+    g_fin_plane_grads = g_fin_plane_params = nullptr;
 }
 bool recording() { return g_rec != nullptr; }
 void record(std::function<int(hipStream_t)> fn, const OpInfo& info) { g_rec->ops.push_back(PlanOp{std::move(fn), info, 0.0, 0, true, g_side}); }
diff --git a/dynamic_multiview_3d_amd/csrc/elem.hip b/dynamic_multiview_3d_amd/csrc/elem.hip
--- a/dynamic_multiview_3d_amd/csrc/elem.hip
+++ b/dynamic_multiview_3d_amd/csrc/elem.hip
@@ -1,5 +1,6 @@
 #include "common.h"
 #include "reduce_common.h"
+#include "split_bf16.h"
 #include <vector>
 #include <algorithm>
 #include <cstdlib>
@@ -421,15 +422,28 @@
     const float* part; float* out;
     int64_t off;
     int64_t count;
-    int nslab, vec, blk0, pad;
+    int nslab, vec, blk0;
+    int plane;
 };
 
-template <int OPT>
+struct FinPlaneJob {
+    uint4* Wf;
+    int chunks, ntiles, kcols, pad;
+    int16_t slot[36];
+};
+struct FinPlane {
+    int C, K, rtiles, ctiles, njobs, pad[3];
+    FinPlaneJob job[2];
+};
+
+template <int OPT, bool PLANES = false>
 __global__ __launch_bounds__(256) void grad_finalize_kernel(const FinSeg* __restrict__ segs, const int* __restrict__ seg_of_blk,
                                                            const float* __restrict__ G, float* __restrict__ P, float* __restrict__ M,
-                                                           float* __restrict__ V, const float* __restrict__ st) {
+                                                           float* __restrict__ V, const float* __restrict__ st,
+                                                           const FinPlane* __restrict__ planes) {
     constexpr bool ADAM = OPT == OPT_ADAM, SGD = OPT == OPT_MOMENTUM || OPT == OPT_GD;
-    __shared__ float s_sum[4][16][17];
+    __shared__ float s_sum[PLANES ? 4 : 1][4][16][17];
+    __shared__ float s_tile[PLANES ? 8 : 1][33];
     const FinSeg sg = segs[seg_of_blk[blockIdx.x]];
     const int blk = (int)blockIdx.x - sg.blk0;
     float alpha = 0.f, omb1 = 0.f, omb2 = 0.f, eps = 0.f, gscale = 1.f;
@@ -451,6 +465,7 @@
         v += (gk * gk - v) * omb2;
         pp -= (m * alpha) / (sqrtf(v) + eps);
         P[i] = pp; M[i] = m; V[i] = v;
+        return pp;
     };
     auto sgd1 = [&](int64_t i, float g) {
         const float gk = g * gscale;
@@ -458,7 +473,65 @@
         if (OPT == OPT_MOMENTUM) { float a = M[i]; momentum_elem(gk, pp, a, lr, mu, nesterov); M[i] = a; }
         else gd_elem(gk, pp, lr);
         P[i] = pp;
+        return pp;
     };
+    if constexpr (PLANES && (ADAM || SGD)) {
+        if (sg.plane) {
+            const FinPlane& pl = planes[sg.plane - 1];
+            const int tid = threadIdx.x, e = tid & 15, sl = tid >> 4;
+            const int ct = blk % pl.ctiles, rt = (blk / pl.ctiles) % pl.rtiles, tap = blk / (pl.ctiles * pl.rtiles);
+            const int r0 = rt * 8, c0 = ct * 32;
+            const int64_t tap_base = (int64_t)tap * pl.C * pl.K;
+            if (sg.nslab > 0) {
+#pragma unroll
+                for (int q = 0; q < 4; ++q) {
+                    const int row = r0 + 2 * q + (e >> 3), col = c0 + (e & 7) * 4;
+                    reduce_slabs_partial<4>(sg.part, sg.nslab, sg.count, tap_base + (int64_t)row * pl.K + col, row < pl.C && col < pl.K,
+                                            e, sl, s_sum[q]);
+                }
+                __syncthreads();
+            }
+            {
+                const int q = tid >> 6, v = sl & 3;
+                const int rl = 2 * q + (e >> 3), cl = (e & 7) * 4 + v;
+                float nv = 0.f;
+                if (r0 + rl < pl.C && c0 + cl < pl.K) {
+                    const int64_t i = sg.off + tap_base + (int64_t)(r0 + rl) * pl.K + (c0 + cl);
+                    const float t = sg.nslab > 0 ? reduce_slabs_total(s_sum[q], v, e) : G[i];
+                    if constexpr (ADAM) nv = adam1(i, t);
+                    else nv = sgd1(i, t);
+                }
+                s_tile[rl][cl] = nv;
+            }
+            __syncthreads();
+            const int j = tid >> 6, w = tid & 63;
+            if (j < pl.njobs && w < 32) {
+                const FinPlaneJob& jb = pl.job[j];
+                const int t = jb.slot[tap];
+                float x[8];
+                int cc, s, lh, nt, li;
+                if (!jb.kcols) {
+#pragma unroll
+                    for (int k = 0; k < 8; ++k) x[k] = s_tile[k][w];
+                    cc = r0 >> 5; s = (r0 >> 4) & 1; lh = (r0 >> 3) & 1; nt = ct; li = w;
+                } else {
+                    const int r = w & 7, gq = w >> 3;
+#pragma unroll
+                    for (int k = 0; k < 8; ++k) x[k] = s_tile[r][gq * 8 + k];
+                    cc = ct; s = gq >> 1; lh = gq & 1; nt = (r0 + r) >> 5; li = (r0 + r) & 31;
+                }
+                if (t >= 0 && cc < jb.chunks && nt < jb.ntiles) {
+                    uint2 h0, l0, h1, l1;
+                    split4(make_float4(x[0], x[1], x[2], x[3]), h0, l0);
+                    split4(make_float4(x[4], x[5], x[6], x[7]), h1, l1);
+                    uint4* dst = jb.Wf + ((((int64_t)t * jb.chunks + cc) * jb.ntiles + nt) * 4 + s * 2) * 64 + lh * 32 + li;
+                    dst[0] = make_uint4(h0.x, h0.y, h1.x, h1.y);
+                    dst[64] = make_uint4(l0.x, l0.y, l1.x, l1.y);
+                }
+            }
+            return;
+        }
+    }
     if (sg.nslab == 0) {
         if (!ADAM && !SGD) return;
         const int64_t i4 = (int64_t)blk * 256 + threadIdx.x;
@@ -488,8 +561,8 @@
         else if (SGD) sgd1(sg.off + i, t);
         else sg.out[i] = t;
     };
-    if (sg.vec) reduce_slabs_body<4>(sg.part, sg.nslab, sg.count, blk, s_sum, fin);
-    else reduce_slabs_body<1>(sg.part, sg.nslab, sg.count, blk, s_sum, fin);
+    if (sg.vec) reduce_slabs_body<4>(sg.part, sg.nslab, sg.count, blk, s_sum[0], fin);
+    else reduce_slabs_body<1>(sg.part, sg.nslab, sg.count, blk, s_sum[0], fin);
 }
 
 __global__ __launch_bounds__(256) void act_fwd_kernel(int64_t rows, int ch, const float* x, int x_ld, float* y, int y_ld,
@@ -786,20 +859,72 @@
 }
 int mv3d_grad_finalize_abort(void) { finalize_take(nullptr); return MV3D_OK; }
 
-static int fin_blocks(const FinSegHost& h) {
+static int fin_plane_of(const FinSegHost& h, const float* grads, const float* params, FinPlane* pl) {
+    PlaneJob jobs[2];
+    const int nj = bconv_cache_jobs_of(params + (h.out - grads), jobs, 2);
+    if (nj == 0) return 0;
+    if (nj > 2) return -1;
+    const PlaneJob& a = jobs[0];
+    const int K = a.w_ns == 1 ? a.w_ks : a.w_ns;
+    if (K < 1 || K % 4 != 0 || a.w_tap_stride % K != 0) return -1;
+    const int C = a.w_tap_stride / K;
+    const int64_t taps = h.count / ((int64_t)C * K);
+    if (taps < 1 || taps > 36 || h.count - taps * C * K < 0 || h.count - taps * C * K > 3) return -1;
+    if (h.nslab > 0 && (h.count % 4 != 0 || ((uintptr_t)h.part & 15))) return -1;
+    *pl = FinPlane{};
+    pl->C = C; pl->K = K; pl->njobs = nj;
+    int rows = 0, cols = 0;
+    for (int j = 0; j < nj; ++j) {
+        const PlaneJob& b = jobs[j];
+        FinPlaneJob& d = pl->job[j];
+        const bool kcols = b.w_ks == 1 && b.w_ns == K;
+        if (!kcols && !(b.w_ns == 1 && b.w_ks == K)) return -1;
+        if (b.w_tap_stride != C * K || b.ntaps != (int)taps || b.Ka != (kcols ? K : C) || b.Cc != (kcols ? C : K)) return -1;
+        d.Wf = reinterpret_cast<uint4*>(b.Wf); d.chunks = b.chunks; d.ntiles = b.ntiles; d.kcols = kcols ? 1 : 0;
+        for (int t = 0; t < 36; ++t) d.slot[t] = -1;
+        for (int t = 0; t < b.ntaps; ++t) {
+            if (b.widx[t] < 0 || b.widx[t] >= taps || d.slot[b.widx[t]] >= 0) return -1;
+            d.slot[b.widx[t]] = (int16_t)t;
+        }
+        rows = std::max(rows, 32 * (kcols ? b.ntiles : b.chunks));
+        cols = std::max(cols, 32 * (kcols ? b.chunks : b.ntiles));
+    }
+    pl->rtiles = rows / 8; pl->ctiles = cols / 32;
+    return 1;
+}
+static int fin_blocks(const FinSegHost& h, const FinPlane* pl = nullptr) {
+    if (pl) return (int)(h.count / ((int64_t)pl->C * pl->K)) * pl->rtiles * pl->ctiles;
     if (h.nslab == 0) return (int)cdiv64(cdiv64(h.count, 4), 256);
     const bool vec = h.count % 4 == 0 && ((uintptr_t)h.part & 15) == 0;
     return (int)cdiv64(h.count, vec ? 64 : 16);
 }
+static size_t fin_table_bytes(size_t nsegs, size_t blocks, size_t nplanes) {
+    size_t n = ((nsegs * sizeof(FinSeg) + 255) & ~(size_t)255) + blocks * sizeof(int);
+    if (nplanes) n = ((n + 15) & ~(size_t)15) + nplanes * sizeof(FinPlane);
+    return n;
+}
 size_t mv3d_grad_finalize_table_bytes(void) {
     const std::vector<FinSegHost>* v = finalize_peek();
     if (!v) return 0;
-    size_t blocks = 0;
-    for (const FinSegHost& h : *v) blocks += fin_blocks(h);
-    return ((v->size() * sizeof(FinSeg) + 255) & ~(size_t)255) + blocks * sizeof(int);
+    const float* grads = nullptr; const float* params = nullptr;
+    const bool planes = finalize_planes(&grads, &params);
+    size_t blocks = 0, nplanes = 0;
+    for (const FinSegHost& h : *v) {
+        FinPlane pl;
+        if (planes && fin_plane_of(h, grads, params, &pl) == 1) { blocks += fin_blocks(h, &pl); ++nplanes; }
+        else blocks += fin_blocks(h);
+    }
+    return fin_table_bytes(v->size(), blocks, nplanes);
+}
+int mv3d_grad_finalize_keep_planes(const void* grads, const void* params) {
+    if (!finalize_collecting()) return fail(MV3D_E_INVAL, "mv3d_grad_finalize_keep_planes: no open collection");
+    if (!grads || !params || (((uintptr_t)grads | (uintptr_t)params) & 15))
+        return fail(MV3D_E_INVAL, "mv3d_grad_finalize_keep_planes: the flat gradient and parameter buffers (16-byte aligned)");
+    finalize_set_planes((const float*)grads, (const float*)params);
+    return MV3D_OK;
 }
 static int grad_finalize_launch(std::vector<FinSegHost>& segs, size_t need, void* table, size_t table_bytes, void* grads, void* params,
-                                void* slot1, void* slot2, const void* state, int opt, void* stream) {
+                                void* slot1, void* slot2, const void* state, int opt, bool keep_planes, void* stream) {
     const bool upd = opt != OPT_NONE;
     std::vector<FinSegHost> keep;
     for (size_t a = 0; a < segs.size(); ++a) {
@@ -816,12 +941,13 @@
     const bool dry = !table && recording();
     if (!dry && (!table || table_bytes < need || ((uintptr_t)table & 15))) return fail(MV3D_E_WORKSPACE, "mv3d_grad_finalize_commit: table %zu < %zu bytes", table_bytes, need);
     std::vector<FinSeg> dev(keep.size());
+    std::vector<FinPlane> planes;
     std::vector<int> seg_of;
     double bytes = 0.0;
     for (size_t j = 0; j < keep.size(); ++j) {
         const FinSegHost& h = keep[j];
         FinSeg& d = dev[j];
-        d.part = h.part; d.out = h.out; d.count = h.count; d.nslab = h.nslab; d.pad = 0;
+        d.part = h.part; d.out = h.out; d.count = h.count; d.nslab = h.nslab; d.plane = 0;
         d.vec = h.nslab > 0 && h.count % 4 == 0 && ((uintptr_t)h.part & 15) == 0;
         d.off = 0;
         if (upd) {
@@ -829,50 +955,82 @@
             if (off < 0 || (h.nslab == 0 && (off & 3))) return fail(MV3D_E_INVAL, "mv3d_grad_finalize_commit: segment %zu is not inside the flat gradient buffer", j);
             d.off = off;
         }
+        FinPlane pl;
+        const int has = keep_planes ? fin_plane_of(h, (const float*)grads, (const float*)params, &pl) : 0;
+        if (has < 0)
+            return fail(MV3D_E_UNSUPPORTED, "mv3d_grad_finalize_commit: segment %zu is a bound conv filter whose prepared copies this launch cannot write "
+                                            "(K %% 4, misaligned partials, more than two orientations or a partial tap set)", j);
+        if (has) { planes.push_back(pl); d.plane = (int)planes.size(); }
         d.blk0 = (int)seg_of.size();
-        const int nb = fin_blocks(h);
+        const int nb = fin_blocks(h, has ? &pl : nullptr);
         seg_of.insert(seg_of.end(), nb, (int)j);
         bytes += 4.0 * h.count * (h.nslab + (opt == OPT_ADAM ? 6 : opt == OPT_MOMENTUM ? 4 : opt == OPT_GD ? 2 : 1));
+        if (has) bytes += 4.0 * h.count * pl.njobs;
     }
     const size_t seg_bytes = (dev.size() * sizeof(FinSeg) + 255) & ~(size_t)255;
+    const size_t plane_off = (seg_bytes + seg_of.size() * sizeof(int) + 15) & ~(size_t)15;
+    if (!dry && fin_table_bytes(dev.size(), seg_of.size(), planes.size()) > table_bytes)
+        return fail(MV3D_E_WORKSPACE, "mv3d_grad_finalize_commit: table %zu bytes too small", table_bytes);
     if (!dry && (hipMemcpy(table, dev.data(), dev.size() * sizeof(FinSeg), hipMemcpyHostToDevice) != hipSuccess ||
-                 hipMemcpy((char*)table + seg_bytes, seg_of.data(), seg_of.size() * sizeof(int), hipMemcpyHostToDevice) != hipSuccess))
+                 hipMemcpy((char*)table + seg_bytes, seg_of.data(), seg_of.size() * sizeof(int), hipMemcpyHostToDevice) != hipSuccess ||
+                 (!planes.empty() && hipMemcpy((char*)table + plane_off, planes.data(), planes.size() * sizeof(FinPlane), hipMemcpyHostToDevice) != hipSuccess)))
         return fail(MV3D_E_HIP, "mv3d_grad_finalize_commit: table upload failed");
     const FinSeg* dsegs = (const FinSeg*)table;
     const int* dmap = (const int*)((char*)table + seg_bytes);
+    const FinPlane* dplanes = planes.empty() ? nullptr : (const FinPlane*)((char*)table + plane_off);
     const int blocks = (int)seg_of.size();
     const char* label = opt == OPT_ADAM ? "grad_finalize_adam" : opt == OPT_MOMENTUM ? "grad_finalize_momentum" : opt == OPT_GD ? "grad_finalize_sgd" : "grad_finalize";
     return dispatch(stream, OpInfo{label, 0.0, bytes}, [=](hipStream_t s) {
         const float* G = (const float*)grads; float* P = (float*)params; const float* st = (const float*)state;
-        if (opt == OPT_ADAM) grad_finalize_kernel<OPT_ADAM><<<blocks, 256, 0, s>>>(dsegs, dmap, G, P, (float*)slot1, (float*)slot2, st);
-        else if (opt == OPT_MOMENTUM) grad_finalize_kernel<OPT_MOMENTUM><<<blocks, 256, 0, s>>>(dsegs, dmap, G, P, (float*)slot1, nullptr, st);
-        else if (opt == OPT_GD) grad_finalize_kernel<OPT_GD><<<blocks, 256, 0, s>>>(dsegs, dmap, G, P, nullptr, nullptr, st);
-        else grad_finalize_kernel<OPT_NONE><<<blocks, 256, 0, s>>>(dsegs, dmap, nullptr, nullptr, nullptr, nullptr, nullptr);
+        if (dplanes) {
+            if (opt == OPT_ADAM) grad_finalize_kernel<OPT_ADAM, true><<<blocks, 256, 0, s>>>(dsegs, dmap, G, P, (float*)slot1, (float*)slot2, st, dplanes);
+            else if (opt == OPT_MOMENTUM) grad_finalize_kernel<OPT_MOMENTUM, true><<<blocks, 256, 0, s>>>(dsegs, dmap, G, P, (float*)slot1, nullptr, st, dplanes);
+            else grad_finalize_kernel<OPT_GD, true><<<blocks, 256, 0, s>>>(dsegs, dmap, G, P, nullptr, nullptr, st, dplanes);
+        }
+        else if (opt == OPT_ADAM) grad_finalize_kernel<OPT_ADAM><<<blocks, 256, 0, s>>>(dsegs, dmap, G, P, (float*)slot1, (float*)slot2, st, dplanes);
+        else if (opt == OPT_MOMENTUM) grad_finalize_kernel<OPT_MOMENTUM><<<blocks, 256, 0, s>>>(dsegs, dmap, G, P, (float*)slot1, nullptr, st, dplanes);
+        else if (opt == OPT_GD) grad_finalize_kernel<OPT_GD><<<blocks, 256, 0, s>>>(dsegs, dmap, G, P, nullptr, nullptr, st, dplanes);
+        else grad_finalize_kernel<OPT_NONE><<<blocks, 256, 0, s>>>(dsegs, dmap, nullptr, nullptr, nullptr, nullptr, nullptr, nullptr);
         return launched("grad_finalize_kernel");
     });
+}
+
+static bool fin_keep_planes(const void* grads, const void* params, bool optimiser, int* rc) {
+    const float* g = nullptr; const float* p = nullptr;
+    *rc = MV3D_OK;
+    if (!finalize_planes(&g, &p)) return false;
+    if (!optimiser || g != grads || p != params)
+        *rc = fail(MV3D_E_INVAL, "mv3d_grad_finalize_commit: mv3d_grad_finalize_keep_planes needs an optimiser commit on the flat buffers it named");
+    return true;
 }
 
 int mv3d_grad_finalize_commit(void* table, size_t table_bytes, void* grads, void* params, void* adam_m, void* adam_v,
                               const void* adam_state, void* stream) {
     if (!finalize_collecting()) return fail(MV3D_E_INVAL, "mv3d_grad_finalize_commit: no open collection");
     const size_t need = mv3d_grad_finalize_table_bytes();
+    const bool adam = adam_state != nullptr;
+    int prc;
+    const bool keep_planes = fin_keep_planes(grads, params, adam, &prc);
     std::vector<FinSegHost> segs;
     finalize_take(&segs);
-    const bool adam = adam_state != nullptr;
+    if (prc != MV3D_OK) return prc;
     if (adam && (!grads || !params || !adam_m || !adam_v || (((uintptr_t)grads | (uintptr_t)params | (uintptr_t)adam_m | (uintptr_t)adam_v) & 15)))
         return fail(MV3D_E_INVAL, "mv3d_grad_finalize_commit: the optimiser needs the four flat buffers (16-byte aligned)");
-    return grad_finalize_launch(segs, need, table, table_bytes, grads, params, adam_m, adam_v, adam_state, adam ? OPT_ADAM : OPT_NONE, stream);
+    return grad_finalize_launch(segs, need, table, table_bytes, grads, params, adam_m, adam_v, adam_state, adam ? OPT_ADAM : OPT_NONE, keep_planes, stream);
 }
 
 int mv3d_grad_finalize_commit_sgd(void* table, size_t table_bytes, void* grads, void* params, void* accum, const void* sgd_state,
                                   void* stream) {
     if (!finalize_collecting()) return fail(MV3D_E_INVAL, "mv3d_grad_finalize_commit_sgd: no open collection");
     const size_t need = mv3d_grad_finalize_table_bytes();
+    int prc;
+    const bool keep_planes = fin_keep_planes(grads, params, true, &prc);
     std::vector<FinSegHost> segs;
     finalize_take(&segs);
     if (!grads || !params || !sgd_state || (((uintptr_t)grads | (uintptr_t)params | (uintptr_t)accum) & 15))
         return fail(MV3D_E_INVAL, "mv3d_grad_finalize_commit_sgd: the optimiser needs the flat gradient, parameter (and momentum) buffers, 16-byte aligned, and the state");
-    return grad_finalize_launch(segs, need, table, table_bytes, grads, params, accum, nullptr, sgd_state, accum ? OPT_MOMENTUM : OPT_GD, stream);
-}
-
-}
+    if (prc != MV3D_OK) return prc;
+    return grad_finalize_launch(segs, need, table, table_bytes, grads, params, accum, nullptr, sgd_state, accum ? OPT_MOMENTUM : OPT_GD, keep_planes, stream);
+}
+
+}
diff --git a/dynamic_multiview_3d_amd/csrc/reduce_common.h b/dynamic_multiview_3d_amd/csrc/reduce_common.h
--- a/dynamic_multiview_3d_amd/csrc/reduce_common.h
+++ b/dynamic_multiview_3d_amd/csrc/reduce_common.h
@@ -3,17 +3,15 @@
 
 namespace mv3d {
 
-template <int VEC, class FIN>
-__device__ __forceinline__ void reduce_slabs_body(const float* __restrict__ part, int nslab, int64_t count,
-                                                  int blk, float (*s_sum)[16][17], FIN fin) {
-    const int e = threadIdx.x & 15, sl = threadIdx.x >> 4;
-    const int64_t i = ((int64_t)blk * 16 + e) * VEC;
+template <int VEC>
+__device__ __forceinline__ void reduce_slabs_partial(const float* __restrict__ part, int nslab, int64_t count, int64_t i, bool valid,
+                                                     int e, int sl, float (*s_sum)[16][17]) {
     float acc[8][VEC];
 #pragma unroll
     for (int u = 0; u < 8; ++u)
 #pragma unroll
         for (int v = 0; v < VEC; ++v) acc[u][v] = 0.f;
-    if (i < count) {
+    if (valid) {
         const float* p = part + (int64_t)sl * count + i;
         const int64_t step = 16 * count;
         int k = sl;
@@ -40,13 +38,23 @@
 #pragma unroll
     for (int v = 0; v < VEC; ++v)
         s_sum[v][sl][e] = ((acc[0][v] + acc[1][v]) + (acc[2][v] + acc[3][v])) + ((acc[4][v] + acc[5][v]) + (acc[6][v] + acc[7][v]));
+}
+__device__ __forceinline__ float reduce_slabs_total(const float (*s_sum)[16][17], int v, int e) {
+    float t = 0.f;
+#pragma unroll
+    for (int j = 0; j < 16; ++j) t += s_sum[v][j][e];
+    return t;
+}
+
+template <int VEC, class FIN>
+__device__ __forceinline__ void reduce_slabs_body(const float* __restrict__ part, int nslab, int64_t count,
+                                                  int blk, float (*s_sum)[16][17], FIN fin) {
+    const int e = threadIdx.x & 15, sl = threadIdx.x >> 4;
+    const int64_t i = ((int64_t)blk * 16 + e) * VEC;
+    reduce_slabs_partial<VEC>(part, nslab, count, i, i < count, e, sl, s_sum);
     __syncthreads();
-    if (sl < VEC && i < count) {
-        float t = 0.f;
-#pragma unroll
-        for (int j = 0; j < 16; ++j) t += s_sum[sl][j][e];
-        fin(i + sl, t);
-    }
+    if (sl < VEC && i < count)
+        fin(i + sl, reduce_slabs_total(s_sum, sl, e));
 }
 
 }
diff --git a/dynamic_multiview_3d_amd/csrc/split_bf16.h b/dynamic_multiview_3d_amd/csrc/split_bf16.h
--- /dev/null
+++ b/dynamic_multiview_3d_amd/csrc/split_bf16.h
@@ -0,0 +1,24 @@
+#pragma once
+#include "common.h"
+
+namespace mv3d {
+
+typedef __bf16 bf16x4 __attribute__((ext_vector_type(4)));
+
+__device__ __forceinline__ void split4(const float4& v, uint2& hi, uint2& lo) {
+    bf16x4 h, l;
+    h[0] = (__bf16)v.x; h[1] = (__bf16)v.y; h[2] = (__bf16)v.z; h[3] = (__bf16)v.w;
+    l[0] = (__bf16)(v.x - (float)h[0]); l[1] = (__bf16)(v.y - (float)h[1]);
+    l[2] = (__bf16)(v.z - (float)h[2]); l[3] = (__bf16)(v.w - (float)h[3]);
+    hi = __builtin_bit_cast(uint2, h);
+    lo = __builtin_bit_cast(uint2, l);
+}
+
+struct PlaneJob {
+    void* Wf;
+    int ntaps, chunks, ntiles, Ka, Cc, w_tap_stride, w_ks, w_ns;
+    int16_t widx[36];
+};
+int bconv_cache_jobs_of(const float* Wt, PlaneJob* out, int max_out);
+
+}
diff --git a/dynamic_multiview_3d_amd/graph.py b/dynamic_multiview_3d_amd/graph.py
--- a/dynamic_multiview_3d_amd/graph.py
+++ b/dynamic_multiview_3d_amd/graph.py
@@ -106,6 +106,7 @@
     def set(self, array):
         t = torch.as_tensor(np.ascontiguousarray(array, dtype=np.float32)) if not torch.is_tensor(array) else array
         self.value().copy_(t.reshape(self.shape), non_blocking=True)
+        self.graph._planes_dirty = True
 
 
 class Variable:
@@ -512,6 +513,11 @@
         self._finalizing = False
         self._finalized_in_plan = False
         self._part_arena = self._fin_table = None
+        self.split_in_finalize = os.environ.get('MV3D_SPLIT_IN_FINALIZE', '0') != '0'
+        self._plan_fwd_full = self._plan_fwd_lean = None
+        self._n_fwd_full = self._n_fwd_lean = 0
+        self._planes_dirty = True
+        self._keep_planes = False
         self._fused_vars = []
         self.pipeline_fc = os.environ.get('MV3D_PIPELINE_FCADAM', '1') != '0'
         self.pipeline_dp = os.environ.get('MV3D_PIPELINE_DP', '1') != '0'
@@ -523,7 +529,7 @@
         self._pending_idx = 0
         self.plan_bwd_fused = None
         self.opt_state = None
-        self.plan_fwd = self.plan_bwd = None
+        self.plan_bwd = None
         self._smooth_deferred = []
         self.optimizer = 'adam'
         self.momentum, self.use_nesterov = 0.0, False
@@ -538,6 +544,17 @@
         self.bucket_elems = 16 * 1024 * 1024
 
     OPTIMIZERS = ('adam', 'momentum', 'sgd')
+
+    def _fwd_is_lean(self):
+        return self._plan_fwd_lean is not None and not self._planes_dirty
+
+    @property
+    def plan_fwd(self):
+        return self._plan_fwd_lean if self._fwd_is_lean() else self._plan_fwd_full
+
+    @property
+    def n_launch_fwd(self):
+        return self._n_fwd_lean if self._fwd_is_lean() else self._n_fwd_full
 
     @property
     def adam_state(self):
@@ -787,21 +804,15 @@
                     raise ValueError("flow_smoothness_loss: a flow of shape %s is outside what mv3d_flow_smoothness takes" % (term.a.shape,))
                 term.ws = torch.empty(nbytes, dtype=torch.uint8, device=self.device)
         self._find_fc_chains()
-        self.plan_fwd = lib.plan_create()
-        lib.plan_begin(self.plan_fwd)
-        try:
-            lib.filter_cache_refresh(None)
-            if self.loss_expr is not None and self.loss_expr.terms:
-                lib.loss_overwrite_next()
-            else:
-                lib.fill(self.loss_buf.data_ptr(), 1, 0.0, self.stream)
-            self._fwd_first_op = {}
-            for n in self.nodes:
-                self._fwd_first_op[id(n)] = lib.plan_size(self.plan_fwd)
-                n.forward(self)
-            self._emit_losses(with_grad=True)
-        finally:
-            lib.plan_end()
+        self._keep_planes = (self.split_in_finalize and self.fuse_finalize and self.fuse_fc_adam and self.lr is not None and
+                             bool(self._prepared_vars) and any(isinstance(n, LinearNode) for n in self.nodes) and
+                             all(v.shape[-1] % 4 == 0 for v in self._prepared_vars))
+        self._plan_fwd_lean, self._planes_dirty = None, True
+        if self._keep_planes:
+            self._plan_fwd_lean = self._record_forward(refresh=False)
+            for t in self.tensors:
+                t.grad_written = t.grad_masked = False
+        self._plan_fwd_full = self._record_forward(refresh=True)
         flags_after_forward = [(t.grad_written, t.grad_masked) for t in self.tensors]
         self.plan_bwd = lib.plan_create()
         lib.plan_begin(self.plan_bwd)
@@ -851,9 +862,11 @@
             i = next(j for j, b in enumerate(self.grad_buckets) if b[0] > self.adam_gate)
             hi = self.grad_buckets[i][2]
             self.grad_buckets.insert(i, (self.adam_gate, hi, hi))
-        self.n_launch_fwd = lib.plan_size(self.plan_fwd)
+        self._n_fwd_full = lib.plan_size(self._plan_fwd_full)
+        self._n_fwd_lean = lib.plan_size(self._plan_fwd_lean) if self._plan_fwd_lean is not None else 0
         self.n_launch_bwd = lib.plan_size(self.plan_bwd)
         self._bucket_first_use = [self._first_param_use(lo, hi) for _, lo, hi in self.grad_buckets]
+        kept = set()
         self.plan_bwd_fused = None
         self._fused_vars = []
         self._fused_nodes = []
@@ -869,7 +882,7 @@
                         n._part_off, n._part_bytes = off, n.wgrad_partial_bytes(self)
                         off += -(-n._part_bytes // 256) * 256
                 self._part_arena = torch.empty(max(off // 4, 4), dtype=torch.float32, device=self.device)
-                lib.grad_finalize_begin()
+                self._finalize_begin()
                 self._finalizing = True
                 self._fin_pending, self._fin_vars, self._fin_done, self._fin_tables = 0, [], set(), []
             lib.plan_begin(plan)
@@ -883,7 +896,7 @@
                         self._fin_vars += [n.w] + ([n.b] if n.b is not None else [])
                         if self._fin_pending >= self.finalize_chunk_bytes:
                             self._finalize_commit()
-                            lib.grad_finalize_begin()
+                            self._finalize_begin()
                 self._smooth_all_placed(pending)
                 for n in self._fused_nodes:
                     n.record_fused_update(self)
@@ -892,6 +905,8 @@
                     for v in self.variables.values():
                         if v.has_grad and id(v) not in fused and id(v) not in self._fin_done:
                             lib.grad_finalize_add(v.grad_ptr, -(-v.size // 4) * 4)
+                            kept.add(id(v))
+                    kept |= self._fin_done
                     self._finalize_commit()
                     self._finalizing = False
                     self._finalized_in_plan = True
@@ -926,8 +941,32 @@
                 self._fwd_wait_idx = self._first_fc_hazard()
             else:
                 lib.plan_destroy(plan)
+        if self._plan_fwd_lean is not None and not (self.plan_bwd_fused is not None and self._finalized_in_plan and
+                                                    all(id(v) in kept or not v.has_grad for v in self._prepared_vars)):
+            lib.plan_destroy(self._plan_fwd_lean)
+            self._plan_fwd_lean, self._n_fwd_lean, self._keep_planes = None, 0, False
         self.upload_optimizer_state()
         return self
+
+    def _record_forward(self, refresh):
+        lib = self.lib
+        plan = lib.plan_create()
+        lib.plan_begin(plan)
+        try:
+            if refresh:
+                lib.filter_cache_refresh(None)
+            if self.loss_expr is not None and self.loss_expr.terms:
+                lib.loss_overwrite_next()
+            else:
+                lib.fill(self.loss_buf.data_ptr(), 1, 0.0, self.stream)
+            self._fwd_first_op = {}
+            for n in self.nodes:
+                self._fwd_first_op[id(n)] = lib.plan_size(plan)
+                n.forward(self)
+            self._emit_losses(with_grad=True)
+        finally:
+            lib.plan_end()
+        return plan
 
     def _finalize_commit(self):
         lib = self.lib
@@ -950,10 +989,16 @@
         self._fin_done |= {id(v) for v in self._fin_vars}
         self._fin_pending, self._fin_vars = 0, []
 
+    def _finalize_begin(self):
+        self.lib.grad_finalize_begin()
+        if self._keep_planes:
+            self.lib.grad_finalize_keep_planes(self.grads.data_ptr(), self.params.data_ptr())
+
     def _bind_prepared_filters(self):
         lib = self.lib
         lib.filter_cache_clear()
         self._prepared = []
+        self._prepared_vars = []
         if torch.device(self.device).type != 'cuda':
             return
         for n in self.nodes:
@@ -969,6 +1014,8 @@
                     buf = torch.empty(nbytes, dtype=torch.uint8, device=self.device)
                     self._prepared.append(buf)
                     lib.filter_cache_bind(C.byref(geom), op, n.w.ptr, buf.data_ptr(), nbytes)
+                    if n.w not in self._prepared_vars:
+                        self._prepared_vars.append(n.w)
         tb = int(lib.filter_cache_table_bytes())
         self._prepared_table = torch.empty(max(tb, 16), dtype=torch.uint8, device=self.device)
         lib.filter_cache_commit(self._prepared_table.data_ptr(), tb, None)
@@ -977,7 +1024,7 @@
         return torch.cuda.current_stream(self.device).cuda_stream
 
     def _first_param_use(self, lo, hi):
-        first = self.n_launch_fwd
+        first = self._n_fwd_full
         for n in self.nodes:
             for name, val in vars(n).items():
                 if isinstance(val, Variable) and val.offset is not None and lo <= val.offset < hi:
@@ -997,7 +1044,7 @@
                     if isinstance(t, Tensor):
                         yield t
         fused = {id(n) for n in self._fused_nodes}
-        idx = self.n_launch_fwd
+        idx = self._n_fwd_full
         for n in self.nodes:
             if id(n) in fused or any(id(t._root()[0]) in roots for t in tensors_of(n)):
                 idx = min(idx, self._fwd_first_op[id(n)])
@@ -1012,13 +1059,17 @@
 
     def run_forward(self):
         st = self._stream_ptr()
-        if self._fc_pending and 0 < self._pending_idx < self.n_launch_fwd:
-            self.lib.plan_run_range(self.plan_fwd, 0, self._pending_idx, st)
+        lean = self._fwd_is_lean()
+        plan, n = (self._plan_fwd_lean, self._n_fwd_lean) if lean else (self._plan_fwd_full, self._n_fwd_full)
+        idx = self._pending_idx - (self._n_fwd_full - n)
+        self._planes_dirty = False
+        if self._fc_pending and 0 < idx < n:
+            self.lib.plan_run_range(plan, 0, idx, st)
             self._settle()
-            self.lib.plan_run_range(self.plan_fwd, self._pending_idx, self.n_launch_fwd, st)
+            self.lib.plan_run_range(plan, idx, n, st)
             return
         self._settle()
-        self.lib.plan_run(self.plan_fwd, st)
+        self.lib.plan_run(plan, st)
 
     def begin_side(self, cls=1):
         if self.n_side == 0:
@@ -1087,6 +1138,7 @@
 
     def apply_optimizer(self):
         self._settle()
+        self._planes_dirty = True
         self._opt_range(0, self.flat_size, self._stream_ptr())
         self._adam_advance()
 
@@ -1117,12 +1169,15 @@
             self._fc_event.record(fcq)
             self._fc_pending = True
             self._pending_idx = self._fwd_wait_idx
+        if not self._keep_planes:
+            self._planes_dirty = True
         if not self._finalized_in_plan:
             self._opt_range(0, self.flat_size, st, (len(self._skip_lo), self._skip_lo, self._skip_hi))
         self._adam_advance(st, both=False)
 
     def run_backward_with_adam(self):
         self._settle()
+        self._planes_dirty = True
         main = torch.cuda.current_stream(self.device)
         sides, ns = self._side_ptrs()
         if self.adam_stream is None:
@@ -1156,6 +1211,7 @@
 
     def run_backward_overlapped(self, with_adam=False):
         self._settle()
+        self._planes_dirty = self._planes_dirty or with_adam
         main = self._stream_ptr()
         sides, ns = self._side_ptrs()
         on_gpu = torch.device(self.device).type == 'cuda'
@@ -1235,6 +1291,7 @@
 
     def set_variables(self, values):
         self._settle()
+        self._planes_dirty = True
         for k, a in values.items():
             self.variables[k].value().copy_(torch.as_tensor(np.asarray(a, dtype=np.float32)).reshape(self.variables[k].shape))
 
@@ -1286,6 +1343,7 @@
 
     def load_state_dict(self, sd):
         self._settle()
+        self._planes_dirty = True
         slots = self._slots()
         names = {n for n, _ in slots}
         missing = [k for k in self.variables if k not in sd]
diff --git a/include/mv3d_hip.h b/include/mv3d_hip.h
--- a/include/mv3d_hip.h
+++ b/include/mv3d_hip.h
@@ -169,6 +169,7 @@
 int mv3d_grad_finalize_commit_sgd(void* table, size_t table_bytes, void* grads, void* params, void* accum, const void* sgd_state,
                                   void* stream);
 int mv3d_grad_finalize_abort(void);
+int mv3d_grad_finalize_keep_planes(const void* grads, const void* params);
 
 typedef struct mv3d_comm mv3d_comm;
 int mv3d_comm_available(void);
```

After: 38270 images/sec, median of 3. No clear change (+0.2%).
